# ashawkey/torch-ngp

Measured on AMD Instinct MI355X. Metric: training samples/s (rays x steps), lego-shaped synthetic, fp16 autocast, full step incl. Adam, higher is better.
Workload: dtype f16

## Files before the change

include/ngp_hip.h:

```cpp
#ifndef NGP_HIP_H
#define NGP_HIP_H

#include <stddef.h>
#include <stdint.h>

#ifdef __cplusplus
extern "C" {
#endif

typedef void* ngp_stream_t;

enum {
    NGP_OK = 0,
    NGP_ERR_INVALID = 1,
    NGP_ERR_LAUNCH = 2,
    NGP_ERR_DEVICE = 3
};

enum { NGP_F32 = 0, NGP_F16 = 1, NGP_F64 = 2 };

#define NGP_MAX_LEVELS 32

const char* ngp_last_error(void);
int ngp_abi_version(void);
// ... 133 lines not shown
    float lr, beta1, beta2, eps;
} ngp_table_adam_t;
uint32_t ngp_grid_table_adam_prefix(const int32_t* offsets_host, uint32_t B, uint32_t D, uint32_t C, uint32_t L, float S, uint32_t H,
                                    uint32_t gridtype, int align_corners, int dtype);
typedef struct ngp_slab_sets {
    const void* slabs_a; uint32_t n_slabs_a, n_params_a; void* grad_weights_a;
    const void* slabs_b; uint32_t n_slabs_b, n_params_b; void* grad_weights_b;
    const float* ray_err; uint32_t n_rays; float* loss;
    uint32_t overwrite_table;
    const ngp_table_adam_t* table_adam;
} ngp_slab_sets_t;
int ngp_grid_encode_backward_checked_slabs(const void* grad, const float* inputs, const void* embeddings, const int32_t* offsets,
                                           void* grad_embeddings, uint32_t B, uint32_t D, uint32_t C, uint32_t L, float S, uint32_t H,
                                           const void* dy_dx, void* grad_inputs, uint32_t gridtype, int align_corners, uint32_t interp,
                                           int dtype, float bound, const int32_t* offsets_host, void* workspace, size_t workspace_bytes,
                                           float* found_inf, const ngp_slab_sets_t* slab_sets, ngp_stream_t stream);
int ngp_grid_encode_backward_ws(const void* grad, const float* inputs, const void* embeddings, const int32_t* offsets,
                                void* grad_embeddings, uint32_t B, uint32_t D, uint32_t C, uint32_t L, float S, uint32_t H,
                                const void* dy_dx, void* grad_inputs, uint32_t gridtype, int align_corners, uint32_t interp,
                                int dtype, float bound, const int32_t* offsets_host, void* workspace, size_t workspace_bytes,
                                ngp_stream_t stream);

size_t ngp_density_grid_update_workspace_bytes(uint32_t n_cells);
int ngp_density_grid_update(const float* sigmas, const int64_t* cells, uint32_t n, float density_scale, float decay, float* density_grid,
                            uint32_t n_cells, float* scratch, float density_thresh, float* mean_out, uint8_t* bitfield, void* workspace,
                            ngp_stream_t stream);

#define NGP_FF_INPUT_PLANAR 1u
#define NGP_FF_DX_PLANAR 2u
#define NGP_FF_LAYERED 4u
#define NGP_FF_SINGLE_WAVE 8u
#define NGP_FF_DEFER_REDUCE 16u
#define NGP_FF_RECOMPUTE 32u
int ngp_ffmlp_forward_ex(const void* inputs, const void* weights, uint32_t B, uint32_t input_dim, uint32_t output_dim,
                         uint32_t hidden_dim, uint32_t num_layers, uint32_t activation, uint32_t output_activation,
                         void* forward_buffer, void* outputs, uint32_t flags, ngp_stream_t stream);
int ngp_ffmlp_inference_ex(const void* inputs, const void* weights, uint32_t B, uint32_t input_dim,
                           uint32_t output_dim, uint32_t hidden_dim, uint32_t num_layers, uint32_t activation,
                           uint32_t output_activation, void* inference_buffer, void* outputs, uint32_t flags,
                           ngp_stream_t stream);
int ngp_ffmlp_backward_ex(const void* grad, const void* inputs, const void* weights, const void* forward_buffer,
                          uint32_t B, uint32_t input_dim, uint32_t output_dim, uint32_t hidden_dim, uint32_t num_layers,
                          uint32_t activation, uint32_t output_activation, int calc_grad_inputs, void* backward_buffer,
                          void* grad_inputs, void* grad_weights, uint32_t flags, ngp_stream_t stream);

size_t ngp_ffmlp_backward_workspace_bytes(uint32_t B, uint32_t input_dim, uint32_t hidden_dim, uint32_t num_layers);
int ngp_ffmlp_backward_ws(const void* grad, const void* inputs, const void* weights, const void* forward_buffer, uint32_t B,
                          uint32_t input_dim, uint32_t output_dim, uint32_t hidden_dim, uint32_t num_layers, uint32_t activation,
                          uint32_t output_activation, int calc_grad_inputs, void* backward_buffer, void* grad_inputs, void* grad_weights,
                          uint32_t flags, void* workspace, size_t workspace_bytes, ngp_stream_t stream);

int ngp_network_forward(const void* enc, const float* dirs, uint32_t M, uint32_t M_valid, const void* w_sigma, const void* w_color,
                        uint32_t num_layers_sigma, uint32_t num_layers_color, float density_scale, int training,
                        void* forward_buffer_sigma, void* h16, float* sigma, void* color_in, void* forward_buffer_color, float* rgb,
                        uint32_t flags, ngp_stream_t stream);

int ngp_network_forward_rows(const void* enc, const float* dirs, uint32_t M, uint32_t M_valid, const void* w_sigma, const void* w_color,
                             uint32_t num_layers_sigma, uint32_t num_layers_color, float density_scale, int training,
                             void* forward_buffer_sigma, void* h16, float* sigma, void* color_in, void* forward_buffer_color, float* rgb,
                             uint32_t flags, const uint32_t* rows_dev, ngp_stream_t stream);

int ngp_network_backward_color(const void* grad_out16, const void* color_in, const void* w_color, const void* forward_buffer_color, uint32_t M,
                               uint32_t num_layers_color, void* backward_buffer, const float* grad_sigma, const void* h16,
                               float density_scale, void* grad_h16, void* grad_w_color, uint32_t flags, ngp_stream_t stream);
uint32_t ngp_ffmlp_backward_slab_count(uint32_t B, uint32_t input_dim, uint32_t hidden_dim, uint32_t num_layers);
int ngp_ffmlp_reduce_slabs_pair(const void* slabs_a, uint32_t n_slabs_a, uint32_t n_params_a, void* grad_weights_a, const void* slabs_b,
                                uint32_t n_slabs_b, uint32_t n_params_b, void* grad_weights_b, float* found_inf, ngp_stream_t stream);

int ngp_pipeline_mid_forward(const void* h16, const float* dirs, float* sigma, void* color_in, uint32_t M, uint32_t M_valid,
                             float density_scale, ngp_stream_t stream);
int ngp_pipeline_rgb_forward(const void* out16, float* rgb, uint32_t M, ngp_stream_t stream);
int ngp_pipeline_rgb_backward(const float* grad_rgb, const float* rgb, void* grad_out16, uint32_t M, ngp_stream_t stream);
int ngp_pipeline_mid_backward(const float* grad_sigma, const void* h16, const void* grad_color_in, void* grad_h16, uint32_t M,
                              float density_scale, ngp_stream_t stream);

int ngp_pipeline_mse_loss(const float* image, const float* target, uint32_t n, const float* loss_scale, float* loss,
                          float* grad_image, ngp_stream_t stream);
// ... 73 lines not shown
                                         float T_thresh, float* grad_sigmas, float* grad_rgbs, int bg_mode, float bg_scalar,
                                         const float* bg, const uint32_t* rows_used, ngp_stream_t stream);

int ngp_composite_train_loss_backward(const float* sigmas, const float* rgbs, const float* deltas, const int32_t* rays, uint32_t M,
                                      uint32_t N, float T_thresh, int bg_mode, float bg_scalar, const float* bg, const float* nears,
                                      const float* fars, const float* target, const float* loss_scale, float* weights_sum,
                                      float* image_out, float* depth_out, float* loss, float* ray_err, float* grad_sigmas,
                                      void* grad_out16, void* march_workspace, size_t march_workspace_bytes, ngp_stream_t stream);

int ngp_freq_encode_forward(const float* inputs, uint32_t B, uint32_t D, uint32_t deg, uint32_t C, float* outputs,
                            ngp_stream_t stream);
int ngp_freq_encode_backward(const float* grad, const float* outputs, uint32_t B, uint32_t D, uint32_t deg, uint32_t C,
                             float* grad_inputs, ngp_stream_t stream);

int ngp_optim_adam_step(int count, const uint64_t* n, float* const* params, float* const* exp_avg, float* const* exp_avg_sq,
                        void* const* grads, void* const* params_fp16, const int* grad_is_half, const float* lr, float beta1,
                        float beta2, float eps, float grad_mult, float growth_factor, float backoff_factor, float growth_interval,
                        float* state, ngp_stream_t stream);

#define NGP_OPT_PHASE_CHECK 1u
#define NGP_OPT_PHASE_UPDATE 2u
#define NGP_OPT_PHASE_COMMIT 4u
#define NGP_OPT_PHASE_FLIP 8u
int ngp_optim_adam_step_ex(int count, const uint64_t* n, float* const* params, float* const* exp_avg, float* const* exp_avg_sq,
                           void* const* grads, void* const* params_fp16, const int* grad_is_half, const float* lr, float beta1,
                           float beta2, float eps, float grad_mult, float growth_factor, float backoff_factor, float growth_interval,
                           float* state, float* const* ema, float ema_one_minus_decay, uint32_t phases, ngp_stream_t stream);
struct ngp_table_adam;
int ngp_optim_adam_small_commit(int count, const uint64_t* n, float* const* params, float* const* exp_avg, float* const* exp_avg_sq,
                                void* const* grads, void* const* params_fp16, const int* grad_is_half, const float* lr, float beta1,
                                float beta2, float eps, float grad_mult, float growth_factor, float backoff_factor, float growth_interval,
                                float* state, int flip_parity, const struct ngp_table_adam* table, const void* table_grad_fp16,
                                uint64_t table_prefix_params, ngp_stream_t stream);
int ngp_optim_poison_shards(void* flat_grad_fp16, uint32_t shards, uint64_t payload, const float* state, ngp_stream_t stream);
int ngp_optim_shard_verdict(const void* shard_grad_fp16, float* state, void* flat_grad_fp16, uint32_t shards, uint64_t payload,
                            ngp_stream_t stream);
int ngp_optim_ema_update(int count, const uint64_t* n, float* const* params, float* const* ema, float one_minus_decay, ngp_stream_t stream);

#ifdef __cplusplus
}
#endif
#endif
```

torch-ngp_amd/_ngp_capi.py:

```python
import ctypes
import os

import torch

_HERE = os.path.dirname(os.path.abspath(__file__))
LIB_PATH = os.environ.get('NGP_HIP_LIBRARY') or os.path.join(_HERE, 'libngp_hip.so')

NGP_F32, NGP_F16, NGP_F64 = 0, 1, 2
NGP_FF_INPUT_PLANAR, NGP_FF_DX_PLANAR, NGP_FF_LAYERED, NGP_FF_SINGLE_WAVE, NGP_FF_DEFER_REDUCE, NGP_FF_RECOMPUTE = 1, 2, 4, 8, 16, 32
NGP_MARCH_RESET_COUNTER, NGP_MARCH_ZERO_TAIL, NGP_MARCH_NOISE_FROM_SEED, NGP_MARCH_SCAN_LAUNCH = 1, 2, 4, 8
NGP_OPT_PHASE_CHECK, NGP_OPT_PHASE_UPDATE, NGP_OPT_PHASE_COMMIT, NGP_OPT_PHASE_FLIP = 1, 2, 4, 8
ABI_VERSION = 11

if not os.path.exists(LIB_PATH):
    raise ImportError(
        f"{LIB_PATH} is missing: build the HIP extension first (python __graft_entry__.py, or "
        f"make -C {os.path.join(_HERE, 'csrc')}).  There is no CPU fallback for these operators.")

lib = ctypes.CDLL(LIB_PATH)

_vp, _u32, _f32, _i32, _sz = ctypes.c_void_p, ctypes.c_uint32, ctypes.c_float, ctypes.c_int, ctypes.c_size_t

_SIGNATURES = {
    'ngp_grid_encode_forward': [_vp, _vp, _vp, _vp, _u32, _u32, _u32, _u32, _f32, _u32, _vp, _u32, _i32, _u32, _i32, _vp],
    'ngp_grid_encode_backward': [_vp, _vp, _vp, _vp, _vp, _u32, _u32, _u32, _u32, _f32, _u32, _vp, _vp, _u32, _i32, _u32, _i32, _vp],
    'ngp_grad_total_variation': [_vp, _vp, _vp, _vp, _f32, _u32, _u32, _u32, _u32, _f32, _u32, _u32, _i32, _i32, _vp],
    'ngp_grid_corner_indices': [_vp, _vp, _vp, _u32, _u32, _u32, _f32, _u32, _u32, _i32, _vp],
    'ngp_grid_level_table': [_u32, _f32, _u32, _vp, _vp],
    'ngp_grid_encode_backward_backward': [_vp, _vp, _vp, _vp, _vp, _vp, _vp, _vp, _u32, _u32, _u32, _u32, _f32, _u32, _u32, _i32, _u32, _i32, _vp,
                                          _sz, _vp],
    'ngp_sh_encode_forward': [_vp, _vp, _u32, _u32, _u32, _vp, _i32, _vp],
    'ngp_sh_encode_backward': [_vp, _vp, _u32, _u32, _u32, _vp, _vp, _i32, _vp],
    'ngp_freq_encode_forward': [_vp, _u32, _u32, _u32, _u32, _vp, _vp],
    'ngp_freq_encode_backward': [_vp, _vp, _u32, _u32, _u32, _u32, _vp, _vp],
    'ngp_near_far_from_aabb': [_vp, _vp, _vp, _u32, _f32, _vp, _vp, _vp],
    'ngp_sph_from_ray': [_vp, _vp, _f32, _u32, _vp, _vp],
    'ngp_morton3D': [_vp, _u32, _vp, _vp],
    'ngp_morton3D_invert': [_vp, _u32, _vp, _vp],
    'ngp_packbits': [_vp, _u32, _f32, _vp, _vp],
    'ngp_packbits_ex': [_vp, _u32, _f32, _vp, _vp, _vp],
    'ngp_march_rays_train': [_vp, _vp, _vp, _f32, _f32, _u32, _u32, _u32, _u32, _u32, _vp, _vp, _vp, _vp, _vp, _vp, _vp, _vp, _vp, _vp],
    'ngp_composite_rays_train_forward': [_vp, _vp, _vp, _vp, _u32, _u32, _f32, _vp, _vp, _vp, _vp],
# ... 24 lines not shown
    'ngp_grid_encode_backward_ws': [_vp, _vp, _vp, _vp, _vp, _u32, _u32, _u32, _u32, _f32, _u32, _vp, _vp, _u32, _i32, _u32, _i32, _f32, _vp, _vp,
                                    _sz, _vp],
    'ngp_grid_encode_backward_checked': [_vp, _vp, _vp, _vp, _vp, _u32, _u32, _u32, _u32, _f32, _u32, _vp, _vp, _u32, _i32, _u32, _i32, _f32, _vp,
                                         _vp, _sz, _vp, _vp],
    'ngp_grid_encode_backward_checked_slabs': [_vp, _vp, _vp, _vp, _vp, _u32, _u32, _u32, _u32, _f32, _u32, _vp, _vp, _u32, _i32, _u32, _i32, _f32,
                                               _vp, _vp, _sz, _vp, _vp, _vp],
    'ngp_density_grid_update': [_vp, _vp, _u32, _f32, _f32, _vp, _u32, _vp, _f32, _vp, _vp, _vp, _vp],
    'ngp_ffmlp_forward_ex': [_vp, _vp, _u32, _u32, _u32, _u32, _u32, _u32, _u32, _vp, _vp, _u32, _vp],
    'ngp_ffmlp_inference_ex': [_vp, _vp, _u32, _u32, _u32, _u32, _u32, _u32, _u32, _vp, _vp, _u32, _vp],
    'ngp_ffmlp_backward_ex': [_vp, _vp, _vp, _vp, _u32, _u32, _u32, _u32, _u32, _u32, _u32, _i32, _vp, _vp, _vp, _u32, _vp],
    'ngp_ffmlp_backward_ws': [_vp, _vp, _vp, _vp, _u32, _u32, _u32, _u32, _u32, _u32, _u32, _i32, _vp, _vp, _vp, _u32, _vp, _sz, _vp],
    'ngp_network_forward': [_vp, _vp, _u32, _u32, _vp, _vp, _u32, _u32, _f32, _i32, _vp, _vp, _vp, _vp, _vp, _vp, _u32, _vp],
    'ngp_network_forward_rows': [_vp, _vp, _u32, _u32, _vp, _vp, _u32, _u32, _f32, _i32, _vp, _vp, _vp, _vp, _vp, _vp, _u32, _vp, _vp],
    'ngp_march_rays_dev_rows': [_vp, _u32, _u32, _u32, _vp, _vp, _vp, _vp, _f32, _f32, _u32, _u32, _u32, _vp, _vp, _vp, _vp, _vp, _vp, _vp, _u32, _vp, _vp],
    'ngp_pipeline_mid_forward': [_vp, _vp, _vp, _vp, _u32, _u32, _f32, _vp],
    'ngp_pipeline_rgb_forward': [_vp, _vp, _u32, _vp],
    'ngp_pipeline_rgb_backward': [_vp, _vp, _vp, _u32, _vp],
    'ngp_pipeline_mid_backward': [_vp, _vp, _vp, _vp, _u32, _f32, _vp],
    'ngp_pipeline_mse_loss': [_vp, _vp, _u32, _vp, _vp, _vp, _vp],
    'ngp_rays_from_pixels': [_vp, _u32, _f32, _f32, _f32, _f32, _u32, _vp, _u32, _u32, _vp, _vp, _vp],
    'ngp_march_rays_train_ex': [_vp, _vp, _vp, _f32, _f32, _u32, _u32, _u32, _u32, _u32, _vp, _vp, _vp, _vp, _vp, _vp, _vp, _vp, _vp, _u32, _vp],
    'ngp_march_rays_train_aabb': [_vp, _vp, _vp, _f32, _f32, _u32, _u32, _u32, _u32, _u32, _vp, _f32, _vp, _vp, _vp, _vp, _vp, _vp, _vp, _vp, _vp, _u32,
                                  _vp],
    'ngp_composite_rays_train_forward_ex': [_vp, _vp, _vp, _vp, _u32, _u32, _f32, _vp, _vp, _vp, _i32, _f32, _vp, _vp, _vp, _vp, _vp, _vp],
    'ngp_composite_rays_train_backward_ex': [_vp, _vp, _vp, _vp, _vp, _vp, _vp, _vp, _u32, _u32, _f32, _vp, _vp, _i32, _f32, _vp, _vp, _vp],
    'ngp_composite_train_loss_backward': [_vp, _vp, _vp, _vp, _u32, _u32, _f32, _i32, _f32, _vp, _vp, _vp, _vp, _vp, _vp, _vp, _vp, _vp, _vp, _vp,
                                          _vp, _vp, _sz, _vp],
    'ngp_network_backward_color': [_vp, _vp, _vp, _vp, _u32, _u32, _vp, _vp, _vp, _f32, _vp, _vp, _u32, _vp],
    'ngp_ffmlp_reduce_slabs_pair': [_vp, _u32, _u32, _vp, _vp, _u32, _u32, _vp, _vp, _vp],
    'ngp_optim_adam_step': [_i32, _vp, _vp, _vp, _vp, _vp, _vp, _vp, _vp, _f32, _f32, _f32, _f32, _f32, _f32, _f32, _vp, _vp],
    'ngp_optim_adam_step_ex': [_i32, _vp, _vp, _vp, _vp, _vp, _vp, _vp, _vp, _f32, _f32, _f32, _f32, _f32, _f32, _f32, _vp, _vp, _f32, _u32, _vp],
    'ngp_optim_adam_small_commit': [_i32, _vp, _vp, _vp, _vp, _vp, _vp, _vp, _vp, _f32, _f32, _f32, _f32, _f32, _f32, _f32, _vp, _i32, _vp, _vp,
                                    ctypes.c_uint64, _vp],
    'ngp_optim_ema_update': [_i32, _vp, _vp, _vp, _f32, _vp],
    'ngp_optim_poison_shards': [_vp, _u32, ctypes.c_uint64, _vp, _vp],
    'ngp_optim_shard_verdict': [_vp, _vp, _vp, _u32, ctypes.c_uint64, _vp],
    'ngp_linear_stack_pack': [_vp, _u32, _u32, _u32, _u32, _i32, _vp, _vp],
    'ngp_linear_stack_unpack_grad': [_vp, _u32, _u32, _u32, _u32, _i32, _vp, _vp],
    'ngp_pad_2d_fp16': [_vp, _u32, _u32, _u32, _vp, _u32, _u32, _vp],
    'ngp_allocate_splitk': [_sz],
    'ngp_free_splitk': [],
}
for _name, _args in _SIGNATURES.items():
    _fn = getattr(lib, _name)
    _fn.argtypes = _args
    _fn.restype = ctypes.c_int
lib.ngp_last_error.restype = ctypes.c_char_p
lib.ngp_target_arch.restype = ctypes.c_char_p
lib.ngp_abi_version.restype = ctypes.c_int
lib.ngp_ffmlp_backward_slab_count.argtypes = [_u32, _u32, _u32, _u32]
lib.ngp_ffmlp_backward_slab_count.restype = _u32
lib.ngp_march_rays_train_workspace_bytes.argtypes = [_u32]
lib.ngp_march_rays_train_workspace_bytes.restype = _sz
lib.ngp_compact_rays_workspace_bytes.argtypes = [_u32]
lib.ngp_ffmlp_backward_workspace_bytes.argtypes = [_u32, _u32, _u32, _u32]
lib.ngp_ffmlp_backward_workspace_bytes.restype = _sz
lib.ngp_grid_backward_workspace_bytes.argtypes = [_vp, _u32, _u32, _u32, _u32, _f32, _u32, _u32, _i32, _i32]
lib.ngp_grid_backward_workspace_bytes.restype = _sz
lib.ngp_grid_backward_backward_workspace_bytes.argtypes = [_vp, _u32, _u32, _u32, _u32, _i32]
lib.ngp_grid_backward_backward_workspace_bytes.restype = _sz
lib.ngp_compact_rays_workspace_bytes.restype = _sz
lib.ngp_grid_table_adam_prefix.argtypes = [_vp, _u32, _u32, _u32, _u32, _f32, _u32, _u32, _i32, _i32]
lib.ngp_grid_table_adam_prefix.restype = _u32
lib.ngp_coarse_occupancy_bytes.argtypes = [_u32, _u32]
lib.ngp_coarse_occupancy_bytes.restype = _sz
lib.ngp_grid_forward_work_lists.argtypes = [_u32, _u32, _vp, _vp, _vp, _vp]
lib.ngp_grid_forward_work_lists.restype = _u32
lib.ngp_density_grid_update_workspace_bytes.argtypes = [_u32]
lib.ngp_linear_stack_flat_size.argtypes = [_u32, _u32, _u32, _u32, _i32]
lib.ngp_linear_stack_flat_size.restype = _u32
lib.ngp_density_grid_update_workspace_bytes.restype = _sz

if lib.ngp_abi_version() != ABI_VERSION:
    raise ImportError(f"{LIB_PATH}: ABI version {lib.ngp_abi_version()} != expected {ABI_VERSION}; rebuild the extension")

EXPORTED = sorted(list(_SIGNATURES) + ['ngp_last_error', 'ngp_target_arch', 'ngp_abi_version',
                                       'ngp_march_rays_train_workspace_bytes', 'ngp_compact_rays_workspace_bytes',
                                       'ngp_grid_backward_workspace_bytes', 'ngp_ffmlp_backward_workspace_bytes',
                                       'ngp_ffmlp_backward_slab_count', 'ngp_density_grid_update_workspace_bytes', 'ngp_grid_forward_work_lists', 'ngp_coarse_occupancy_bytes',
                                       'ngp_grid_table_adam_prefix', 'ngp_linear_stack_flat_size',
                                       'ngp_grid_backward_backward_workspace_bytes'])


def check(rc):
    if rc != 0:
        raise RuntimeError(lib.ngp_last_error().decode('utf-8', 'replace'))


class SlabSets(ctypes.Structure):
    _fields_ = [('slabs_a', ctypes.c_void_p), ('n_slabs_a', ctypes.c_uint32), ('n_params_a', ctypes.c_uint32), ('grad_weights_a', ctypes.c_void_p),
                ('slabs_b', ctypes.c_void_p), ('n_slabs_b', ctypes.c_uint32), ('n_params_b', ctypes.c_uint32), ('grad_weights_b', ctypes.c_void_p),
                ('ray_err', ctypes.c_void_p), ('n_rays', ctypes.c_uint32), ('loss', ctypes.c_void_p), ('overwrite_table', ctypes.c_uint32),
                ('table_adam', ctypes.c_void_p)]


class RenderLoop(ctypes.Structure):
    _fields_ = ([('state', ctypes.c_void_p), ('alive', ctypes.c_void_p * 2)] +
                [(n, ctypes.c_void_p) for n in ('rays_t', 'rays_o', 'rays_d', 'nears', 'fars', 'grid', 'noises', 'xyzs', 'dirs', 'deltas', 'enc', 'sigmas',
                                                'rgbs', 'embeddings', 'offsets', 'level_cost_host', 'w_sigma', 'w_color', 'weights_sum', 'depth', 'image',
                                                'compact_workspace', 'rows_used')] +
                [(n, ctypes.c_uint32) for n in ('lanes', 'rows', 'n_total', 'n_step_cap', 'max_steps', 'cascade', 'grid_size', 'L', 'H', 'gridtype',
                                                'interp', 'num_layers_sigma', 'num_layers_color')] +
                [('align_corners', ctypes.c_int32)] + [(n, ctypes.c_float) for n in ('bound', 'dt_gamma', 'T_thresh', 'S', 'density_scale')])


class TableAdam(ctypes.Structure):
    _fields_ = [('param', ctypes.c_void_p * 2), ('exp_avg', ctypes.c_void_p * 2), ('exp_avg_sq', ctypes.c_void_p * 2), ('param_fp16', ctypes.c_void_p * 2),
                ('state', ctypes.c_void_p), ('lr', ctypes.c_float), ('beta1', ctypes.c_float), ('beta2', ctypes.c_float), ('eps', ctypes.c_float)]


def ptr(t):
    return None if t is None else t.data_ptr()


def stream():
    return torch.cuda.current_stream().cuda_stream


def require_device(t, name):
    if not t.is_cuda:
        raise RuntimeError(f"{name} must be a CUDA tensor")


def require_contiguous(t, name):
    if not t.is_contiguous():
        raise RuntimeError(f"{name} must be a contiguous tensor")


def require_int32(t, name):
    if t.dtype != torch.int32:
        raise RuntimeError(f"{name} must be an int tensor")


def float_code(t, name):
    if t.dtype == torch.float16:
        return NGP_F16
    if t.dtype == torch.float32:
        return NGP_F32
    if t.dtype == torch.float64:
        return NGP_F64
    raise RuntimeError(f"{name} must be a floating tensor")
# ... 60 lines not shown
```

torch-ngp_amd/csrc/ffmlp.hip:

```cpp
#include "common.h"
#include "sh_poly.inc"

namespace ngp {

constexpr int FF_WAVES = 4;
constexpr int FF_THREADS = FF_WAVES * 64;
constexpr int FF_TILE = 32;

enum Act : uint32_t { ACT_RELU = 0, ACT_EXP = 1, ACT_SINE = 2, ACT_SIGMOID = 3, ACT_SQUAREPLUS = 4, ACT_SOFTPLUS = 5, ACT_NONE = 6 };
constexpr float K_ACT = 10.0f;

__device__ __forceinline__ float act_forward(uint32_t a, float x) {
    switch (a) {
        case ACT_RELU: return x > 0.0f ? x : 0.0f;
        case ACT_EXP: return __expf(x);
        case ACT_SINE: return __sinf(x);
        case ACT_SIGMOID: return 1.0f / (1.0f + __expf(-x));
        case ACT_SQUAREPLUS: { const float s = x * K_ACT; return 0.5f * (s + sqrtf(s * s + 4.0f)) / K_ACT; }
        case ACT_SOFTPLUS: return __logf(__expf(x * K_ACT) + 1.0f) / K_ACT;
        default: return x;
    }
}
__device__ __forceinline__ float act_backward_factor(uint32_t a, float y) {
    switch (a) {
        case ACT_RELU: return y > 0.0f ? 1.0f : 0.0f;
        case ACT_EXP: return y;
        case ACT_SIGMOID: return y * (1.0f - y);
        case ACT_SQUAREPLUS: { const float s = y * K_ACT; return s * s / (s * s + 1.0f); }
        case ACT_SOFTPLUS: return 1.0f - __expf(-y * K_ACT);
        default: return 1.0f;
    }
}

// ... 115 lines not shown
__device__ void build_forward_image(half8_t* img, const half_t* __restrict__ w, uint32_t in_dim, uint32_t num_layers, uint32_t first_frag = 0,
                                    uint32_t n_frags = 0xFFFFFFFFu) {
    if (first_frag == 0u && n_frags == 0xFFFFFFFFu && (in_dim & 15u) == 0u) {
        build_forward_image_coalesced<WIDTH>(img, w, in_dim, num_layers);
        return;
    }
    const uint32_t all = fwd_frag_count<WIDTH>(in_dim, num_layers);
    const uint32_t total = (n_frags == 0xFFFFFFFFu ? all : n_frags) * 64;
    const uint32_t shift = first_frag * 64;
    for (uint32_t e0 = threadIdx.x; e0 < total; e0 += IMG_BATCH * blockDim.x) {
        half4_t lo[IMG_BATCH], hi[IMG_BATCH];
        bool real[IMG_BATCH];
#pragma unroll
        for (int b = 0; b < IMG_BATCH; b++) {
            const uint32_t e = e0 + b * blockDim.x;
            const half_t *pl = nullptr, *ph = nullptr;
            if (e < total) forward_fragment_source<WIDTH>(e + shift, w, in_dim, num_layers, pl, ph);
            real[b] = pl != nullptr;
            lo[b] = *reinterpret_cast<const half4_t*>(pl ? pl : w);
            hi[b] = *reinterpret_cast<const half4_t*>(ph ? ph : w);
        }
#pragma unroll
        for (int b = 0; b < IMG_BATCH; b++) {
            const uint32_t e = e0 + b * blockDim.x;
            if (e < total) {
                const half4_t z = {(half_t)0.0f, (half_t)0.0f, (half_t)0.0f, (half_t)0.0f};
                const half4_t l4 = real[b] ? lo[b] : z, h4 = real[b] ? hi[b] : z;
                img[e] = half8_t{l4.x, l4.y, l4.z, l4.w, h4.x, h4.y, h4.z, h4.w};
            }
        }
    }
}

template <int WIDTH>
__device__ __forceinline__ void pack_hidden(const float16_t (&acc)[Shape<WIDTH>::NIB], half8_t (&frag)[Shape<WIDTH>::NKB]) {
#pragma unroll
    for (int kb = 0; kb < Shape<WIDTH>::NKB; kb++) {
#pragma unroll
        for (int j = 0; j < 8; j++) frag[kb][j] = (half_t)acc[kb >> 1][(kb & 1) * 8 + j];
    }
}

__device__ __forceinline__ uint32_t relu_pack2(float a, float b) {
    typedef float f32x2 __attribute__((ext_vector_type(2)));
    typedef short i16x2 __attribute__((ext_vector_type(2)));
    const half2_t hv = __builtin_convertvector(f32x2{a, b}, half2_t);
    return __builtin_bit_cast(uint32_t, __builtin_elementwise_max(__builtin_bit_cast(i16x2, hv), i16x2{0, 0}));
}
template <int WIDTH>
__device__ __forceinline__ void pack_hidden_relu(const float16_t (&acc)[Shape<WIDTH>::NIB], half8_t (&frag)[Shape<WIDTH>::NKB]) {
    typedef uint32_t u32x4 __attribute__((ext_vector_type(4)));
#pragma unroll
    for (int kb = 0; kb < Shape<WIDTH>::NKB; kb++) {
        u32x4 w;
#pragma unroll
        for (int q = 0; q < 4; q++) w[q] = relu_pack2(acc[kb >> 1][(kb & 1) * 8 + 2 * q], acc[kb >> 1][(kb & 1) * 8 + 2 * q + 1]);
        frag[kb] = __builtin_bit_cast(half8_t, w);
    }
}


__device__ __forceinline__ half8_t load_features8(const half_t* __restrict__ inputs, bool planar, size_t rows, size_t s, uint32_t in_dim,
                                                  uint32_t f0) {
    if (!planar) return *reinterpret_cast<const half8_t*>(inputs + s * in_dim + f0);
    half8_t v;
#pragma unroll
    for (int q = 0; q < 4; q++) {
        const half2_t t = *reinterpret_cast<const half2_t*>(inputs + ((size_t)(f0 / 2 + q) * rows + s) * 2);
        v[2 * q] = t.x;
        v[2 * q + 1] = t.y;
    }
    return v;
}

template <typename V>
__device__ __forceinline__ void stream_store(V* dst, V v) {
    __builtin_nontemporal_store(v, dst);
}

template <int WIDTH, bool TRAIN, bool PLAIN >
__device__ __forceinline__ void ffmlp_forward_body(const half_t* __restrict__ inputs, const half_t* __restrict__ weights,
                                                   half_t* __restrict__ forward_buffer, half_t* __restrict__ outputs, uint32_t n_tiles,
                                                   uint32_t in_dim, uint32_t num_layers, uint32_t act, uint32_t out_act, bool in_planar) {
    constexpr int NIB = Shape<WIDTH>::NIB, NKB = Shape<WIDTH>::NKB;
    extern __shared__ __attribute__((aligned(16))) unsigned char smem[];
    half8_t* img = reinterpret_cast<half8_t*>(smem);
    build_forward_image<WIDTH>(img, weights, in_dim, num_layers);
    const size_t rows = (size_t)n_tiles * FF_TILE;
    __syncthreads();

    const int lane = threadIdx.x & 63, wid = threadIdx.x >> 6;
    const int n = lane & 31, h = lane >> 5;
    const uint32_t in_kb = in_dim / 16;
    const half8_t* img_l0 = img + lane;
    const half8_t* img_hid = img_l0 + (size_t)NIB * in_kb * 64;
    const half8_t* img_out = img_hid + (size_t)(num_layers - 1) * NIB * NKB * 64;
    const size_t layer_stride = (size_t)n_tiles * NKB * 64;

    for (uint32_t tile = blockIdx.x * FF_WAVES + wid; tile < n_tiles; tile += gridDim.x * FF_WAVES) {
        const size_t srow = (size_t)tile * FF_TILE + n;
        float16_t acc[NIB];
#pragma unroll
        for (int ib = 0; ib < NIB; ib++) acc[ib] = zero16();
        for (uint32_t kb = 0; kb < in_kb; kb++) {
            const half8_t x = load_features8(inputs, in_planar, rows, srow, in_dim, 16 * kb + 8 * h);
#pragma unroll
            for (int ib = 0; ib < NIB; ib++) acc[ib] = mfma(img_l0[(ib * in_kb + kb) * 64], x, acc[ib]);
        }
        half8_t hid[NKB];
        for (uint32_t l = 0;; l++) {
            if (PLAIN || act == ACT_RELU) {
                pack_hidden_relu<WIDTH>(acc, hid);
            } else {
                if (act != ACT_NONE) {
#pragma unroll
                    for (int ib = 0; ib < NIB; ib++)
#pragma unroll
                        for (int r = 0; r < 16; r++) acc[ib][r] = act_forward(act, acc[ib][r]);
                }
                pack_hidden<WIDTH>(acc, hid);
            }
            if (TRAIN) {
                half8_t* dst = reinterpret_cast<half8_t*>(forward_buffer) + l * layer_stride + (size_t)tile * NKB * 64 + lane;
#pragma unroll
                for (int kb = 0; kb < NKB; kb++) stream_store(dst + kb * 64, hid[kb]);
            }
            if (l + 1 == num_layers) break;
            const half8_t* wl = img_hid + (size_t)l * NIB * NKB * 64;
#pragma unroll
            for (int ib = 0; ib < NIB; ib++) {
                acc[ib] = zero16();
#pragma unroll
                for (int kb = 0; kb < NKB; kb++) acc[ib] = mfma(wl[(ib * NKB + kb) * 64], hid[kb], acc[ib]);
            }
        }
        float16_t o = zero16();
#pragma unroll
        for (int kb = 0; kb < NKB; kb++) o = mfma(img_out[kb * 64], hid[kb], o);
        half4_t lo, hi;
#pragma unroll
        for (int c = 0; c < 4; c++) {
            lo[c] = (half_t)(PLAIN ? o[c] : act_forward(out_act, o[c]));
            hi[c] = (half_t)(PLAIN ? o[4 + c] : act_forward(out_act, o[4 + c]));
        }
        half_t* orow = outputs + ((size_t)tile * FF_TILE + n) * 16 + 4 * h;
        *reinterpret_cast<half4_t*>(orow) = lo;
        *reinterpret_cast<half4_t*>(orow + 8) = hi;
    }
}

template <int WIDTH, bool TRAIN, bool PLAIN>
__global__ __launch_bounds__(FF_THREADS) __attribute__((amdgpu_waves_per_eu(4, 4))) void k_ffmlp_forward(
    const half_t* __restrict__ inputs, const half_t* __restrict__ weights, half_t* __restrict__ forward_buffer, half_t* __restrict__ outputs,
    uint32_t n_tiles, uint32_t in_dim, uint32_t num_layers, uint32_t act, uint32_t out_act, bool in_planar) {
    ffmlp_forward_body<WIDTH, TRAIN, PLAIN>(inputs, weights, forward_buffer, outputs, n_tiles, in_dim, num_layers, act, out_act, in_planar);
}
template <int WIDTH, bool TRAIN, bool PLAIN>
__global__ __launch_bounds__(FF_THREADS) __attribute__((amdgpu_waves_per_eu(2, 2))) void k_ffmlp_forward_wide(
    const half_t* __restrict__ inputs, const half_t* __restrict__ weights, half_t* __restrict__ forward_buffer, half_t* __restrict__ outputs,
    uint32_t n_tiles, uint32_t in_dim, uint32_t num_layers, uint32_t act, uint32_t out_act, bool in_planar) {
    ffmlp_forward_body<WIDTH, TRAIN, PLAIN>(inputs, weights, forward_buffer, outputs, n_tiles, in_dim, num_layers, act, out_act, in_planar);
}


template <bool TRAIN, int NT>
__device__ __forceinline__ void relu_network_tail(float16_t (&acc)[NT][2], float16_t (&o)[NT], const half8_t* __restrict__ hid_img,
                                                  const half8_t* __restrict__ out_img, uint32_t nl, half_t* __restrict__ fb, size_t layer_stride,
                                                  const uint32_t (&tile)[NT], const bool (&live)[NT], int lane) {
    constexpr int WIDTH = 64, NIB = 2, NKB = 4;
    half8_t hid[NT][NKB];
    for (uint32_t l = 0;; l++) {
#pragma unroll
        for (int t = 0; t < NT; t++) {
            pack_hidden_relu<WIDTH>(acc[t], hid[t]);
            if (TRAIN && fb && live[t]) {
                half8_t* dst = reinterpret_cast<half8_t*>(fb) + l * layer_stride + (size_t)tile[t] * NKB * 64 + lane;
#pragma unroll
                for (int kb = 0; kb < NKB; kb++) stream_store(dst + kb * 64, hid[t][kb]);
            }
        }
        if (l + 1 == nl) break;
        const half8_t* wl = hid_img + (size_t)l * NIB * NKB * 64;
#pragma unroll
        for (int ib = 0; ib < NIB; ib++) {
#pragma unroll
            for (int t = 0; t < NT; t++) acc[t][ib] = zero16();
#pragma unroll
            for (int kb = 0; kb < NKB; kb++) {
                const half8_t a = wl[(ib * NKB + kb) * 64];
#pragma unroll
                for (int t = 0; t < NT; t++) acc[t][ib] = mfma(a, hid[t][kb], acc[t][ib]);
            }
        }
    }
#pragma unroll
    for (int t = 0; t < NT; t++) o[t] = zero16();
#pragma unroll
    for (int kb = 0; kb < NKB; kb++) {
        const half8_t a = out_img[kb * 64];
#pragma unroll
        for (int t = 0; t < NT; t++) o[t] = mfma(a, hid[t][kb], o[t]);
    }
}

template <bool TRAIN, int WAVES , int NT >
__global__ __launch_bounds__(WAVES * 64) __attribute__((amdgpu_waves_per_eu(NT == 1 ? 4 : 2, NT == 1 ? 4 : 3))) void k_network_forward(
    const half_t* __restrict__ enc, bool enc_planar, const float* __restrict__ dirs, uint32_t M_valid, const half_t* __restrict__ w_sigma,
    const half_t* __restrict__ w_color, half_t* __restrict__ fb_s, half_t* __restrict__ h16, float* __restrict__ sigma,
    half_t* __restrict__ color_in, half_t* __restrict__ fb_c, float* __restrict__ rgb, uint32_t n_tiles_cap, uint32_t nl_s, uint32_t nl_c,
    float density_scale, const uint32_t* __restrict__ rows_dev) {
    constexpr int WIDTH = 64, NIB = 2, NKB = 4;
    constexpr uint32_t in_kb = 2;
    const uint32_t n_tiles = rows_dev ? min(n_tiles_cap, (rows_dev[0] + (uint32_t)FF_TILE - 1u) / (uint32_t)FF_TILE) : n_tiles_cap;
    extern __shared__ __attribute__((aligned(16))) unsigned char smem[];
    half8_t* img_s = reinterpret_cast<half8_t*>(smem);
    const uint32_t frags_s = NIB * in_kb + (nl_s - 1) * NIB * NKB + NKB;
    half8_t* img_c = img_s + (size_t)frags_s * 64;
    const size_t rows = (size_t)n_tiles_cap * FF_TILE;
    const int lane = threadIdx.x & 63, wid = threadIdx.x >> 6;
    const int n = lane & 31, h = lane >> 5;
    const uint32_t n_groups = (n_tiles + NT - 1) / NT;
    half8_t x_next[NT][in_kb];
    float dir_next[NT][3];
#pragma unroll
    for (int t = 0; t < NT; t++) dir_next[t][0] = dir_next[t][1] = dir_next[t][2] = 0.0f;
    auto request = [&](uint32_t group) {
        if (group < n_groups) {
#pragma unroll
            for (int t = 0; t < NT; t++) {
                const uint32_t tl = group * NT + t < n_tiles ? group * NT + t : n_tiles - 1;
                const size_t srow = (size_t)tl * FF_TILE + n;
#pragma unroll
                for (uint32_t kb = 0; kb < in_kb; kb++) x_next[t][kb] = load_features8(enc, enc_planar, rows, srow, 32, 16 * kb + 8 * h);
                dir_next[t][0] = dir_next[t][1] = dir_next[t][2] = 0.0f;
                if (srow < M_valid) { dir_next[t][0] = dirs[srow * 3]; dir_next[t][1] = dirs[srow * 3 + 1]; dir_next[t][2] = dirs[srow * 3 + 2]; }
            }
        }
    };
    request(blockIdx.x * WAVES + wid);
    build_forward_image<WIDTH>(img_s, w_sigma, 32, nl_s);
    build_forward_image<WIDTH>(img_c, w_color, 32, nl_c);
    __syncthreads();

    const size_t layer_stride = (size_t)n_tiles_cap * NKB * 64;
    const half8_t* s_l0 = img_s + lane;
    const half8_t* s_hid = s_l0 + (size_t)NIB * in_kb * 64;
    const half8_t* s_out = s_hid + (size_t)(nl_s - 1) * NIB * NKB * 64;
    const half8_t* c_l0 = img_c + lane;
    const half8_t* c_hid = c_l0 + (size_t)NIB * in_kb * 64;
    const half8_t* c_out = c_hid + (size_t)(nl_c - 1) * NIB * NKB * 64;

    for (uint32_t group = blockIdx.x * WAVES + wid; group < n_groups; group += gridDim.x * WAVES) {
        uint32_t tile[NT];
        bool live[NT];
        size_t srow[NT];
        half8_t x_cur[NT][in_kb];
        float dir_x[NT], dir_y[NT], dir_z[NT];
#pragma unroll
        for (int t = 0; t < NT; t++) {
            live[t] = NT == 1 || group * NT + t < n_tiles;
            tile[t] = live[t] ? group * NT + t : n_tiles - 1;
            srow[t] = (size_t)tile[t] * FF_TILE + n;
#pragma unroll
            for (uint32_t kb = 0; kb < in_kb; kb++) x_cur[t][kb] = x_next[t][kb];
            dir_x[t] = dir_next[t][0]; dir_y[t] = dir_next[t][1]; dir_z[t] = dir_next[t][2];
        }
        request(group + gridDim.x * WAVES);
        float16_t acc[NT][NIB], o[NT];
#pragma unroll
        for (int t = 0; t < NT; t++)
#pragma unroll
            for (int ib = 0; ib < NIB; ib++) acc[t][ib] = zero16();
#pragma unroll
        for (uint32_t kb = 0; kb < in_kb; kb++)
// ... 254 lines not shown
        for (int kb = 0; kb < NKB; kb++) { dma16(frag + l * layer_stride + kb * 64, buf + (size_t)(1 + l * NKB + kb) * 1024); issued++; }
    unsigned char* xb = buf + (size_t)(1 + num_layers * NKB) * 1024;
    const uint32_t in_kb = in_dim / 16;
    if (!in_planar) {
        for (uint32_t kb = 0; kb < in_kb; kb++) { dma16(inputs + srow * in_dim + 16 * kb + 8 * h, xb + (size_t)kb * 1024); issued++; }
    } else {
        for (uint32_t kb = 0; kb < in_kb; kb++)
#pragma unroll
            for (int q = 0; q < 4; q++) {
                dma4(inputs + ((size_t)((16 * kb + 8 * h) / 2 + q) * rows + srow) * 2, xb + (size_t)kb * 1024 + q * 256);
                issued++;
            }
    }
    return issued;
}

__device__ __forceinline__ half8_t tile_x(const unsigned char* xb, uint32_t kb, bool in_planar, int lane) {
    if (!in_planar) return *reinterpret_cast<const half8_t*>(xb + (size_t)kb * 1024 + lane * 16);
    half8_t v;
#pragma unroll
    for (int q = 0; q < 4; q++) {
        const half2_t t = *reinterpret_cast<const half2_t*>(xb + (size_t)kb * 1024 + q * 256 + lane * 4);
        v[2 * q] = t.x;
        v[2 * q + 1] = t.y;
    }
    return v;
}

template <int WIDTH, int IN_JB , int NHM , bool RELU >
__global__ __launch_bounds__(FF_THREADS) void k_ffmlp_backward(const half_t* __restrict__ grad, const half_t* __restrict__ inputs,
                                                               const half_t* __restrict__ weights, const half_t* __restrict__ forward_buffer,
                                                               uint32_t n_tiles, uint32_t in_dim, uint32_t num_layers, uint32_t act,
                                                               bool with_dx, half_t* __restrict__ grad_inputs, float* __restrict__ slabs,
                                                               half_t* __restrict__ grad_weights_direct, bool in_planar, bool dx_planar, uint32_t pf_depth) {
    constexpr int NIB = Shape<WIDTH>::NIB, NKB = Shape<WIDTH>::NKB;
    extern __shared__ __attribute__((aligned(16))) unsigned char smem[];
    half8_t* img = reinterpret_cast<half8_t*>(smem);
    const uint32_t nfrag = bwd_frag_count<WIDTH>(in_dim, num_layers, with_dx);
    build_backward_image<WIDTH>(img, weights, in_dim, num_layers, with_dx);
    const int lane = threadIdx.x & 63, wid = threadIdx.x >> 6;
    const int n = lane & 31, h = lane >> 5;
    (void)nfrag;
    const Selectors sel = make_selectors(n, h);
    __syncthreads();

    const uint32_t in_kb = in_dim / 16;
    const half8_t* img_out = img + lane;
    const half8_t* img_hid = img_out + (size_t)NIB * 64;
    const half8_t* img_in = img_hid + (size_t)(num_layers - 1) * NIB * NKB * 64;
    const size_t layer_stride = (size_t)n_tiles * NKB * 64;
    const half8_t* fb = reinterpret_cast<const half8_t*>(forward_buffer);
    const size_t rows = (size_t)n_tiles * FF_TILE;

    float16_t gw_out[NIB];
    float16_t gw_in[NIB][IN_JB];
#pragma unroll
    for (int jb = 0; jb < NIB; jb++) gw_out[jb] = zero16();
#pragma unroll
    for (int ib = 0; ib < NIB; ib++)
#pragma unroll
        for (int jb = 0; jb < IN_JB; jb++) gw_in[ib][jb] = zero16();
    float16_t gw_hid[NHM][NIB][NIB];
#pragma unroll
    for (int l = 0; l < NHM; l++)
#pragma unroll
        for (int ib = 0; ib < NIB; ib++)
#pragma unroll
            for (int jb = 0; jb < NIB; jb++) gw_hid[l][ib][jb] = zero16();

    const uint32_t tile_frags = 1 + num_layers * NKB + in_dim / 16;
    unsigned char* pf_base = smem + (size_t)nfrag * 1024 + (size_t)wid * pf_depth * tile_frags * 1024;
    const uint32_t tile_step = gridDim.x * FF_WAVES;
// ... 169 lines not shown
    for (int ib = 0; ib < NIB; ib++) acc[ib] = zero16();
    for (uint32_t kb = 0; kb < in_kb; kb++) {
        const half8_t x = tile_x(xb, kb, in_planar, lane);
#pragma unroll
        for (int ib = 0; ib < NIB; ib++) acc[ib] = mfma(fimg_lane[(ib * in_kb + kb) * 64], x, acc[ib]);
    }
    const half8_t* fhid = fimg_lane + (size_t)NIB * in_kb * 64;
    half8_t hid[NKB];
#pragma unroll
    for (int l = 0; l <= NHM; l++) {
        pack_hidden_relu<WIDTH>(acc, hid);
        sink(l, hid);
        if (l == NHM) break;
        const half8_t* wl = fhid + (size_t)l * NIB * NKB * 64;
#pragma unroll
        for (int ib = 0; ib < NIB; ib++) {
            acc[ib] = zero16();
#pragma unroll
            for (int kb = 0; kb < NKB; kb++) acc[ib] = mfma(wl[(ib * NKB + kb) * 64], hid[kb], acc[ib]);
        }
    }
}

template <int N>
__device__ __forceinline__ void wait_vmcnt() {
    asm volatile("s_waitcnt vmcnt(%0)" ::"n"(N) : "memory");
}

template <int WIDTH, int IN_JB, int NHM , bool RELU, bool RECOMP = false>
__global__ __launch_bounds__(FP_THREADS) __attribute__((amdgpu_waves_per_eu(2, 2)))
void k_ffmlp_backward_paired(const half_t* __restrict__ grad, const half_t* __restrict__ inputs, const half_t* __restrict__ weights,
                             const half_t* __restrict__ forward_buffer, uint32_t n_tiles, uint32_t in_dim, uint32_t num_layers, uint32_t act,
                             bool with_dx, half_t* __restrict__ grad_inputs, float* __restrict__ slabs,
                             half_t* __restrict__ grad_weights_direct, bool in_planar, bool dx_planar, uint32_t pf_depth, MidEpilogue mid) {
    static_assert(NHM == 1 || NHM == 2, "the paired backward covers 2- and 3-layer networks");
    constexpr int NIB = Shape<WIDTH>::NIB, NKB = Shape<WIDTH>::NKB;
    extern __shared__ __attribute__((aligned(16))) unsigned char smem[];
    half8_t* img = reinterpret_cast<half8_t*>(smem);
    const uint32_t nfrag = bwd_frag_count<WIDTH>(in_dim, num_layers, with_dx);
    const uint32_t in_kb = in_dim / 16;
    const uint32_t ffrag = RECOMP ? NIB * in_kb + (num_layers - 1) * NIB * NKB : 0u;
    const int lane = threadIdx.x & 63, wid = threadIdx.x >> 6;
    const int n = lane & 31, h = lane >> 5;
    const int pair = wid & (FP_PAIRS - 1), role = wid / FP_PAIRS;
    const size_t layer_stride = (size_t)n_tiles * NKB * 64;
    const half8_t* fb = reinterpret_cast<const half8_t*>(forward_buffer);
    const size_t rows = (size_t)n_tiles * FF_TILE;
    const uint32_t act_layers = RECOMP ? 0u : num_layers;
    const uint32_t tile_frags = 1 + act_layers * NKB + in_kb;
    unsigned char* pf_base = smem + (size_t)(nfrag + ffrag) * 1024 + (size_t)pair * pf_depth * tile_frags * 1024;
    half8_t* scratch = reinterpret_cast<half8_t*>(smem + (size_t)(nfrag + ffrag) * 1024 + (size_t)FP_PAIRS * pf_depth * tile_frags * 1024 +
                                                  (size_t)pair * NHM * NKB * 1024) + lane;
    const uint32_t base_step = gridDim.x * FP_PAIRS;
    uint32_t cur = 0;
    const uint32_t tile_loads = tile_dma_count<WIDTH>(act_layers, in_dim, in_planar);
    auto prefetch = [&](uint32_t buffer, uint32_t tile) {
        const uint32_t issued = prefetch_tile<WIDTH>(pf_base + (size_t)buffer * tile_frags * 1024, tile, grad, fb, inputs, act_layers, layer_stride,
                                                     rows, in_dim, in_planar, lane, n, h);
        NGP_BOUNDS(issued == tile_loads);
        (void)issued;
    };
    if (role == 0) {
        for (uint32_t d = 0; d + 1 < (pf_depth > 1 ? pf_depth : 2u); d++)
            if (blockIdx.x * FP_PAIRS + d * base_step + pair < n_tiles) prefetch(d, blockIdx.x * FP_PAIRS + d * base_step + pair);
    }
    build_backward_image<WIDTH>(img, weights, in_dim, num_layers, with_dx);
    if (RECOMP) build_forward_image<WIDTH>(img + (size_t)nfrag * 64, weights, in_dim, num_layers, 0, ffrag);
    const Selectors sel = make_selectors(n, h);
    __syncthreads();

    const half8_t* img_out = img + lane;
    const half8_t* img_hid = img_out + (size_t)NIB * 64;
    const half8_t* img_in = img_hid + (size_t)(num_layers - 1) * NIB * NKB * 64;
    const half8_t* fimg = img + (size_t)nfrag * 64 + lane;
    static_assert(tile_dma_count<64>(0, 32, false) == 3u && tile_dma_count<64>(0, 32, true) == 9u && tile_dma_count<64>(2, 32, false) == 11u &&
                  tile_dma_count<64>(2, 32, true) == 17u, "the enumerated vmcnt immediates below are the DMA counts of the three-deep shapes");
    const bool deep = pf_depth == 3 && (tile_loads == 3u || tile_loads == 9u || tile_loads == 11u || tile_loads == 17u);
    auto next_tile_buffer = [&](uint32_t base) -> const unsigned char* {
        if (role == 0) {
            if (deep && base + base_step + pair < n_tiles) {
                switch (tile_loads) {
                    case 3u: wait_vmcnt<3>(); break;
                    case 9u: wait_vmcnt<9>(); break;
                    case 11u: wait_vmcnt<11>(); break;
                    default: wait_vmcnt<17>(); break;
                }
            } else {
                wait_vmcnt<0>();
            }
        }
        __syncthreads();
        const unsigned char* tb = pf_base + (size_t)cur * tile_frags * 1024;
        if (pf_depth > 1) {
            const uint32_t ahead = pf_depth - 1;
            const uint32_t fill = cur == 0 ? pf_depth - 1 : cur - 1;
            cur = cur + 1 == pf_depth ? 0u : cur + 1;
            if (role == 0 && base + ahead * base_step + pair < n_tiles) prefetch(fill, base + ahead * base_step + pair);
        }
        return tb;
    };
// ... 542 lines not shown
    slab_reduce_block(sets, blockIdx.x, part, found_inf);
}

struct DeviceInfo {
    int cus = 0;
    bool ok = false;
};
static DeviceInfo device_info() {
    static thread_local DeviceInfo info;
    if (!info.ok) {
        int dev = 0;
        if (hipGetDevice(&dev) == hipSuccess) {
            hipDeviceProp_t p;
            if (hipGetDeviceProperties(&p, dev) == hipSuccess) {
                info.cus = p.multiProcessorCount;
                info.ok = true;
            }
        }
        if (!info.ok) info.cus = 256;
    }
    return info;
}

static int check_ff_args(const char* fn, uint32_t B, uint32_t in_dim, uint32_t out_dim, uint32_t hidden, uint32_t num_layers) {
    NGP_REQUIRE(hidden == 16 || hidden == 32 || hidden == 64 || hidden == 128 || hidden == 256, NGP_ERR_INVALID,
                "%s: hidden_dim should in [16, 32, 64, 128, 256], but got %u", fn, hidden);
    NGP_REQUIRE(in_dim > 0 && in_dim % 16 == 0, NGP_ERR_INVALID, "%s: input_dim should be 16 * m (m > 0), but got %u", fn, in_dim);
    NGP_REQUIRE(out_dim == 16, NGP_ERR_INVALID, "%s: output_dim must be padded to 16 by the caller (got %u)", fn, out_dim);
    NGP_REQUIRE(num_layers >= 2, NGP_ERR_INVALID, "%s: num_layers should be larger than 2 (3 matmuls), but got %u", fn, num_layers);
    NGP_REQUIRE(B % 128 == 0, NGP_ERR_INVALID, "%s: batch size must be 128 * m, but got %u", fn, B);
    return NGP_OK;
}

static int raise_lds(const void* kern, size_t lds, const char* what) {
    if (lds > 64 * 1024) {
        hipError_t e = hipFuncSetAttribute(kern, hipFuncAttributeMaxDynamicSharedMemorySize, (int)lds);
        NGP_REQUIRE(e == hipSuccess, NGP_ERR_LAUNCH, "%s: cannot raise the dynamic LDS limit: %s", what, hipGetErrorString(e));
    }
    return NGP_OK;
}

template <int WIDTH>
static size_t forward_image_bytes(uint32_t in_dim, uint32_t num_layers) {
    constexpr int NIB = Shape<WIDTH>::NIB, NKB = Shape<WIDTH>::NKB;
    return (size_t)(NIB * (in_dim / 16) + (num_layers - 1) * NIB * NKB + NKB) * 1024;
}

template <int WIDTH, bool TRAIN>
static int launch_forward_layered(const void* inputs, const void* weights, uint32_t B, uint32_t in_dim, uint32_t num_layers, uint32_t act,
                                  uint32_t out_act, void* buffer, void* outputs, uint32_t flags, hipStream_t st) {
    constexpr int NIB = Shape<WIDTH>::NIB, NKB = Shape<WIDTH>::NKB;
    const uint32_t n_tiles = B / FF_TILE;
    uint32_t frags = NIB * (in_dim / 16);
    if (frags < (uint32_t)(NIB * NKB)) frags = NIB * NKB;
    const size_t lds = (size_t)frags * 1024;
    NGP_REQUIRE(lds <= 152 * 1024, NGP_ERR_INVALID, "ffmlp: one %u x %u layer (%zu B) exceeds the LDS of a CU", (unsigned)WIDTH, in_dim, lds);
    NGP_REQUIRE(buffer, NGP_ERR_INVALID, "ffmlp: this network shape needs the %s the reference passes", TRAIN ? "forward_buffer" : "inference_buffer [B, hidden]");
    auto kern = k_ffmlp_forward_layered<WIDTH, TRAIN>;
    int rc = raise_lds(reinterpret_cast<const void*>(kern), lds, "ffmlp");
    if (rc) return rc;
    const uint32_t per_cu = (uint32_t)((160 * 1024) / (lds + 1024));
    uint32_t blocks = (uint32_t)device_info().cus * (per_cu < 1 ? 1 : (per_cu > 2 ? 2 : per_cu));
    const uint32_t need = cdiv(n_tiles, FF_WAVES);
    if (blocks > need) blocks = need;
    hipLaunchKernelGGL(kern, dim3(blocks), dim3(FF_THREADS), lds, st, (const half_t*)inputs, (const half_t*)weights, (half_t*)buffer,
                       (half_t*)outputs, n_tiles, in_dim, num_layers, act, out_act, (flags & NGP_FF_INPUT_PLANAR) != 0);
    return check_launch(TRAIN ? "ffmlp_forward(layered)" : "ffmlp_inference(layered)");
}

template <int WIDTH, bool TRAIN>
static int launch_forward(const void* inputs, const void* weights, uint32_t B, uint32_t in_dim, uint32_t num_layers, uint32_t act,
                          uint32_t out_act, void* fwd, void* outputs, uint32_t flags, hipStream_t st) {
    const uint32_t n_tiles = B / FF_TILE;
    const size_t lds = forward_image_bytes<WIDTH>(in_dim, num_layers);
    if (WIDTH > 128 || lds > 152 * 1024 || (flags & NGP_FF_LAYERED))
        return launch_forward_layered<WIDTH, TRAIN>(inputs, weights, B, in_dim, num_layers, act, out_act, fwd, outputs, flags, st);
    if constexpr (WIDTH > 128) {
        return NGP_ERR_INVALID;
    } else {
    const bool plain = act == ACT_RELU && out_act == ACT_NONE;
    const void* kern;
    if constexpr (WIDTH > 64) kern = plain ? reinterpret_cast<const void*>(k_ffmlp_forward_wide<WIDTH, TRAIN, true>)
                                           : reinterpret_cast<const void*>(k_ffmlp_forward_wide<WIDTH, TRAIN, false>);
    else kern = plain ? reinterpret_cast<const void*>(k_ffmlp_forward<WIDTH, TRAIN, true>) : reinterpret_cast<const void*>(k_ffmlp_forward<WIDTH, TRAIN, false>);
    int rc = raise_lds(kern, lds, "ffmlp");
    if (rc) return rc;
    const uint32_t per_cu = (uint32_t)((160 * 1024) / (lds + 1024));
    uint32_t blocks = (uint32_t)device_info().cus * (per_cu < 1 ? 1 : (per_cu > 4 ? 4 : per_cu));
    const uint32_t need = cdiv(n_tiles, FF_WAVES);
    if (blocks > need) blocks = need;
    const half_t* a0 = (const half_t*)inputs;
    const half_t* a1 = (const half_t*)weights;
    half_t* a2 = (half_t*)fwd;
    half_t* a3 = (half_t*)outputs;
    uint32_t a4 = n_tiles, a5 = in_dim, a6 = num_layers, a7 = act, a8 = out_act;
    bool a9 = (flags & NGP_FF_INPUT_PLANAR) != 0;
    void* args[] = {&a0, &a1, &a2, &a3, &a4, &a5, &a6, &a7, &a8, &a9};
    hipError_t e = hipLaunchKernel(kern, dim3(blocks), dim3(FF_THREADS), args, lds, st);
    NGP_REQUIRE(e == hipSuccess, NGP_ERR_LAUNCH, "ffmlp: kernel launch failed: %s", hipGetErrorString(e));
    return check_launch(TRAIN ? "ffmlp_forward" : "ffmlp_inference");
    }
}

constexpr uint32_t WG_MAX_CHUNKS = 64;

template <int WIDTH>
static int launch_backward_layered(const void* grad, const void* inputs, const void* weights, const void* fwd, uint32_t B, uint32_t in_dim,
                                   uint32_t num_layers, uint32_t act, bool with_dx, void* backward_buffer, void* grad_inputs,
                                   void* grad_weights, uint32_t flags, void* workspace, size_t workspace_bytes, hipStream_t st) {
    constexpr int NIB = Shape<WIDTH>::NIB, NKB = Shape<WIDTH>::NKB;
    const bool in_planar = (flags & NGP_FF_INPUT_PLANAR) != 0, dx_planar = (flags & NGP_FF_DX_PLANAR) != 0;
    const uint32_t n_tiles = B / FF_TILE;
    const uint32_t in_jb = (in_dim + 31) / 32;
    uint32_t frags = NIB * NKB;
    if (with_dx && frags < in_jb * NKB) frags = in_jb * NKB;
    const size_t lds = (size_t)frags * 1024;
    NGP_REQUIRE(lds <= 152 * 1024, NGP_ERR_INVALID, "ffmlp_backward: one %u x %u layer (%zu B) exceeds the LDS of a CU", (unsigned)WIDTH, in_dim, lds);
    const void* dk = act == ACT_RELU ? reinterpret_cast<const void*>(k_ffmlp_dgrad_layered<WIDTH, true>)
                                     : reinterpret_cast<const void*>(k_ffmlp_dgrad_layered<WIDTH, false>);
    int rc = raise_lds(dk, lds, "ffmlp_backward");
    if (rc) return rc;
    const uint32_t per_cu = (uint32_t)((160 * 1024) / (lds + 1024));
    uint32_t blocks = (uint32_t)device_info().cus * (per_cu < 1 ? 1 : (per_cu > 2 ? 2 : per_cu));
    const uint32_t need = cdiv(n_tiles, FF_WAVES);
    if (blocks > need) blocks = need;
    if (act == ACT_RELU)
        hipLaunchKernelGGL((k_ffmlp_dgrad_layered<WIDTH, true>), dim3(blocks), dim3(FF_THREADS), lds, st, (const half_t*)grad, (const half_t*)weights,
                           (const half_t*)fwd, (half_t*)backward_buffer, n_tiles, in_dim, num_layers, act, with_dx, (half_t*)grad_inputs, dx_planar);
    else
        hipLaunchKernelGGL((k_ffmlp_dgrad_layered<WIDTH, false>), dim3(blocks), dim3(FF_THREADS), lds, st, (const half_t*)grad, (const half_t*)weights,
// ... 12 lines not shown
        if (chunks > by_tiles) chunks = by_tiles;
        if (chunks < 1) chunks = 1;
    }
    const uint32_t tiles_per_chunk = cdiv(n_tiles, chunks);
    chunks = cdiv(n_tiles, tiles_per_chunk);
    const bool direct = chunks == 1;
    hipLaunchKernelGGL(k_ffmlp_wgrad<WIDTH>, dim3(chunks, jobs), dim3(FF_THREADS), 0, st, (const half_t*)grad, (const half_t*)inputs, (const half_t*)fwd,
                       (const half_t*)backward_buffer, n_tiles, in_dim, num_layers, in_planar, tiles_per_chunk, direct ? (float*)nullptr : (float*)workspace,
                       direct ? (half_t*)grad_weights : (half_t*)nullptr);
    rc = check_launch("ffmlp_backward(wgrad)");
    if (rc || direct) return rc;
    hipLaunchKernelGGL(k_ffmlp_reduce_slabs, dim3(cdiv(n_params, RS_PARAMS)), dim3(RS_PARAMS * RS_GROUPS), 0, st, (const float*)workspace, chunks,
                       n_params, (half_t*)grad_weights);
    return check_launch("ffmlp_backward(reduce)");
}

template <int WIDTH>
static uint32_t backward_slab_count(uint32_t B, uint32_t in_dim, uint32_t num_layers) {
    const uint32_t n_params = ff_param_count(in_dim, WIDTH, num_layers);
    const size_t buf_bytes = (size_t)num_layers * B * WIDTH * sizeof(half_t);
    uint32_t blocks = (uint32_t)device_info().cus;
    const uint32_t need = cdiv(B / FF_TILE, FF_WAVES);
    if (blocks > need) blocks = need;
    const size_t fit = buf_bytes / ((size_t)n_params * 4);
    if (blocks > fit) blocks = (uint32_t)fit;
    return blocks;
}

template <int WIDTH, int IN_JB, int NHM, bool RELU>
static int launch_backward_t(const void* grad, const void* inputs, const void* weights, const void* fwd, uint32_t B, uint32_t in_dim,
                           uint32_t num_layers, uint32_t act, bool with_dx, void* backward_buffer, void* grad_inputs,
                           void* grad_weights, uint32_t flags, hipStream_t st, const MidEpilogue* mid_in) {
    const bool in_planar = (flags & NGP_FF_INPUT_PLANAR) != 0, dx_planar = (flags & NGP_FF_DX_PLANAR) != 0;
    const bool defer = (flags & NGP_FF_DEFER_REDUCE) != 0;
    const MidEpilogue mid = mid_in ? *mid_in : MidEpilogue{nullptr, nullptr, nullptr, 0.0f};
    constexpr int NIB = Shape<WIDTH>::NIB, NKB = Shape<WIDTH>::NKB;
    const uint32_t n_tiles = B / FF_TILE;
    const uint32_t nfrag = NIB + (num_layers - 1) * NIB * NKB + (with_dx ? ((in_dim + 31) / 32) * NKB : 0);
    const uint32_t n_params = ff_param_count(in_dim, WIDTH, num_layers);
    const size_t tile_bytes = (size_t)(1 + num_layers * NKB + in_dim / 16) * 1024;
    uint32_t pf_depth = 2;
    if ((size_t)nfrag * 1024 + 2 * FF_WAVES * tile_bytes > 160 * 1024) pf_depth = 1;
    size_t lds = (size_t)nfrag * 1024 + (size_t)pf_depth * FF_WAVES * tile_bytes;
    if (lds < (size_t)n_params * 4) lds = (size_t)n_params * 4;
    NGP_REQUIRE(lds <= 160 * 1024, NGP_ERR_INVALID, "ffmlp_backward: LDS need (%zu B) exceeds 160 KiB", lds);
    const uint32_t blocks = backward_slab_count<WIDTH>(B, in_dim, num_layers);
    if (flags & NGP_FF_RECOMPUTE) {
        if constexpr (WIDTH == 64 && IN_JB == 1 && RELU && (NHM == 1 || NHM == 2)) {
            NGP_REQUIRE(in_dim == 32 && !(flags & NGP_FF_SINGLE_WAVE), NGP_ERR_INVALID, "ffmlp_backward: NGP_FF_RECOMPUTE needs input_dim 32 and the paired kernel");
            const uint32_t ffrag = NIB * (in_dim / 16) + (num_layers - 1) * NIB * NKB;
            const size_t tile_b = (size_t)(1 + in_dim / 16) * 1024;
            const uint32_t depth = 3;
            size_t lds_r = (size_t)(nfrag + ffrag) * 1024 + (size_t)depth * FP_PAIRS * tile_b + (size_t)FP_PAIRS * NHM * NKB * 1024;
            if (lds_r < (size_t)n_params * 4) lds_r = (size_t)n_params * 4;
            auto pk = k_ffmlp_backward_paired<WIDTH, IN_JB, NHM, RELU, true>;
            if (lds_r > 64 * 1024) {
                hipError_t e = hipFuncSetAttribute(reinterpret_cast<const void*>(pk), hipFuncAttributeMaxDynamicSharedMemorySize, (int)lds_r);
                NGP_REQUIRE(e == hipSuccess, NGP_ERR_LAUNCH, "ffmlp_backward: cannot raise the dynamic LDS limit: %s", hipGetErrorString(e));
            }
            const bool direct = blocks <= 1;
            hipLaunchKernelGGL(pk, dim3(direct ? 1 : blocks), dim3(FP_THREADS), lds_r, st, (const half_t*)grad, (const half_t*)inputs,
                               (const half_t*)weights, (const half_t*)nullptr, n_tiles, in_dim, num_layers, act, with_dx, (half_t*)grad_inputs,
                               direct ? (float*)nullptr : (float*)backward_buffer, direct ? (half_t*)grad_weights : (half_t*)nullptr, in_planar,
                               dx_planar, depth, mid);
            int rc = check_launch("ffmlp_backward");
            if (rc || direct || defer) return rc;
            hipLaunchKernelGGL(k_ffmlp_reduce_slabs, dim3(cdiv(n_params, RS_PARAMS)), dim3(RS_PARAMS * RS_GROUPS), 0, st,
                               (const float*)backward_buffer, blocks, n_params, (half_t*)grad_weights);
            return check_launch("ffmlp_backward(reduce)");
        } else {
            NGP_REQUIRE(false, NGP_ERR_INVALID, "ffmlp_backward: NGP_FF_RECOMPUTE serves 64-wide ReLU networks with 32 inputs and 2 or 3 layers");
        }
    }
    if constexpr (NHM == 1 || NHM == 2) {
        if (!(flags & NGP_FF_SINGLE_WAVE)) {
            auto pk = k_ffmlp_backward_paired<WIDTH, IN_JB, NHM, RELU>;
            if (lds > 64 * 1024) {
                hipError_t e = hipFuncSetAttribute(reinterpret_cast<const void*>(pk), hipFuncAttributeMaxDynamicSharedMemorySize, (int)lds);
                NGP_REQUIRE(e == hipSuccess, NGP_ERR_LAUNCH, "ffmlp_backward: cannot raise the dynamic LDS limit: %s", hipGetErrorString(e));
            }
            const bool direct = blocks <= 1;
            hipLaunchKernelGGL(pk, dim3(direct ? 1 : blocks), dim3(FP_THREADS), lds, st, (const half_t*)grad, (const half_t*)inputs,
                               (const half_t*)weights, (const half_t*)fwd, n_tiles, in_dim, num_layers, act, with_dx, (half_t*)grad_inputs,
                               direct ? (float*)nullptr : (float*)backward_buffer, direct ? (half_t*)grad_weights : (half_t*)nullptr, in_planar,
                               dx_planar, pf_depth, mid);
            int rc = check_launch("ffmlp_backward");
            if (rc || direct || defer) return rc;
            hipLaunchKernelGGL(k_ffmlp_reduce_slabs, dim3(cdiv(n_params, RS_PARAMS)), dim3(RS_PARAMS * RS_GROUPS), 0, st,
                               (const float*)backward_buffer, blocks, n_params, (half_t*)grad_weights);
            return check_launch("ffmlp_backward(reduce)");
        }
    }
    NGP_REQUIRE(!mid.grad_sigma && !defer, NGP_ERR_INVALID, "ffmlp_backward: this extension needs the paired kernel (2 or 3 layers)");
    auto kern = k_ffmlp_backward<WIDTH, IN_JB, NHM, RELU>;
    if (lds > 64 * 1024) {
        hipError_t e = hipFuncSetAttribute(reinterpret_cast<const void*>(kern), hipFuncAttributeMaxDynamicSharedMemorySize, (int)lds);
        NGP_REQUIRE(e == hipSuccess, NGP_ERR_LAUNCH, "ffmlp_backward: cannot raise the dynamic LDS limit: %s", hipGetErrorString(e));
    }
    if (blocks <= 1) {
        hipLaunchKernelGGL(kern, dim3(1), dim3(FF_THREADS), lds, st, (const half_t*)grad, (const half_t*)inputs, (const half_t*)weights,
                           (const half_t*)fwd, n_tiles, in_dim, num_layers, act, with_dx, (half_t*)grad_inputs, (float*)nullptr,
                           (half_t*)grad_weights, in_planar, dx_planar, pf_depth);
        return check_launch("ffmlp_backward");
    }
    hipLaunchKernelGGL(kern, dim3(blocks), dim3(FF_THREADS), lds, st, (const half_t*)grad, (const half_t*)inputs, (const half_t*)weights,
                       (const half_t*)fwd, n_tiles, in_dim, num_layers, act, with_dx, (half_t*)grad_inputs, (float*)backward_buffer,
                       (half_t*)nullptr, in_planar, dx_planar, pf_depth);
    int rc = check_launch("ffmlp_backward");
    if (rc) return rc;
    hipLaunchKernelGGL(k_ffmlp_reduce_slabs, dim3(cdiv(n_params, RS_PARAMS)), dim3(RS_PARAMS * RS_GROUPS), 0, st, (const float*)backward_buffer, blocks, n_params,
                       (half_t*)grad_weights);
    return check_launch("ffmlp_backward(reduce)");
}

template <int WIDTH, int IN_JB, int NHM>
static int launch_backward(const void* grad, const void* inputs, const void* weights, const void* fwd, uint32_t B, uint32_t in_dim,
                           uint32_t num_layers, uint32_t act, bool with_dx, void* backward_buffer, void* grad_inputs,
                           void* grad_weights, uint32_t flags, hipStream_t st, const MidEpilogue* mid = nullptr) {
    if (act == ACT_RELU)
        return launch_backward_t<WIDTH, IN_JB, NHM, true>(grad, inputs, weights, fwd, B, in_dim, num_layers, act, with_dx, backward_buffer,
                                                          grad_inputs, grad_weights, flags, st, mid);
    return launch_backward_t<WIDTH, IN_JB, NHM, false>(grad, inputs, weights, fwd, B, in_dim, num_layers, act, with_dx, backward_buffer,
                                                       grad_inputs, grad_weights, flags, st, mid);
}

}

using namespace ngp;

#define FF_WIDTHS(CALL)                  \
    switch (hidden_dim) {                \
        case 16: return CALL(16);        \
        case 32: return CALL(32);        \
        case 64: return CALL(64);        \
        case 128: return CALL(128);      \
        default: return CALL(256);       \
    }

extern "C" int ngp_ffmlp_forward_ex(const void* inputs, const void* weights, uint32_t B, uint32_t input_dim, uint32_t output_dim,
                                    uint32_t hidden_dim, uint32_t num_layers, uint32_t activation, uint32_t output_activation,
                                    void* forward_buffer, void* outputs, uint32_t flags, ngp_stream_t stream) {
    int rc = check_ff_args("ffmlp_forward", B, input_dim, output_dim, hidden_dim, num_layers);
    if (rc) return rc;
    if (B == 0) return NGP_OK;
    NGP_REQUIRE(inputs && weights && forward_buffer && outputs, NGP_ERR_INVALID, "ffmlp_forward: NULL tensor");
    hipStream_t st = as_stream(stream);
#define FF_FWD(W) launch_forward<W, true>(inputs, weights, B, input_dim, num_layers, activation, output_activation, forward_buffer, outputs, flags, st)
    FF_WIDTHS(FF_FWD)
#undef FF_FWD
}

extern "C" int ngp_ffmlp_inference_ex(const void* inputs, const void* weights, uint32_t B, uint32_t input_dim, uint32_t output_dim,
                                      uint32_t hidden_dim, uint32_t num_layers, uint32_t activation, uint32_t output_activation,
                                      void* inference_buffer, void* outputs, uint32_t flags, ngp_stream_t stream) {
    int rc = check_ff_args("ffmlp_inference", B, input_dim, output_dim, hidden_dim, num_layers);
    if (rc) return rc;
    if (B == 0) return NGP_OK;
    NGP_REQUIRE(inputs && weights && outputs, NGP_ERR_INVALID, "ffmlp_inference: NULL tensor");
    hipStream_t st = as_stream(stream);
#define FF_INF(W) launch_forward<W, false>(inputs, weights, B, input_dim, num_layers, activation, output_activation, inference_buffer, outputs, flags, st)
    FF_WIDTHS(FF_INF)
#undef FF_INF
}

extern "C" size_t ngp_ffmlp_backward_workspace_bytes(uint32_t B, uint32_t input_dim, uint32_t hidden_dim, uint32_t num_layers) {
    const bool fast = (hidden_dim == 32 || hidden_dim == 64) && num_layers <= 4 && input_dim <= 64;
    if (fast || B == 0) return 0;
    return (size_t)WG_MAX_CHUNKS * ff_param_count(input_dim, hidden_dim, num_layers) * sizeof(float);
}

extern "C" int ngp_ffmlp_backward_ws(const void* grad, const void* inputs, const void* weights, const void* forward_buffer, uint32_t B,
                                     uint32_t input_dim, uint32_t output_dim, uint32_t hidden_dim, uint32_t num_layers, uint32_t activation,
                                     uint32_t output_activation, int calc_grad_inputs, void* backward_buffer, void* grad_inputs,
                                     void* grad_weights, uint32_t flags, void* workspace, size_t workspace_bytes, ngp_stream_t stream) {
    (void)output_activation;
    int rc = check_ff_args("ffmlp_backward", B, input_dim, output_dim, hidden_dim, num_layers);
    if (rc) return rc;
    if (B == 0) {
        if (grad_weights && !(flags & NGP_FF_DEFER_REDUCE)) {
            const size_t n_w = (size_t)hidden_dim * ((size_t)input_dim + (size_t)hidden_dim * (num_layers - 1) + (size_t)output_dim);
            hipError_t e = hipMemsetAsync(grad_weights, 0, n_w * sizeof(half_t), as_stream(stream));
            NGP_REQUIRE(e == hipSuccess, NGP_ERR_LAUNCH, "ffmlp_backward: hipMemsetAsync failed: %s", hipGetErrorString(e));
        }
        return NGP_OK;
    }
    NGP_REQUIRE(grad && inputs && weights && (forward_buffer || (flags & NGP_FF_RECOMPUTE)) && backward_buffer && grad_weights, NGP_ERR_INVALID,
                "ffmlp_backward: NULL tensor");
    NGP_REQUIRE(!calc_grad_inputs || grad_inputs, NGP_ERR_INVALID, "ffmlp_backward: grad_inputs is NULL but calc_grad_inputs is set");
    hipStream_t st = as_stream(stream);
    const bool dx = calc_grad_inputs != 0;
    const bool fast = (hidden_dim == 32 || hidden_dim == 64) && num_layers <= 4 && input_dim <= 64 && !(flags & NGP_FF_LAYERED);
    NGP_REQUIRE(fast || !(flags & NGP_FF_RECOMPUTE), NGP_ERR_INVALID, "ffmlp_backward: NGP_FF_RECOMPUTE serves 64-wide ReLU networks with 32 inputs and 2 or 3 layers");
    NGP_REQUIRE(fast || !(flags & NGP_FF_DEFER_REDUCE), NGP_ERR_INVALID, "ffmlp_backward: NGP_FF_DEFER_REDUCE needs a 2- or 3-layer network of width 32 / 64");
    if (!fast) {
#define FF_LAY(W) launch_backward_layered<W>(grad, inputs, weights, forward_buffer, B, input_dim, num_layers, activation, dx, backward_buffer, grad_inputs, grad_weights, flags, workspace, workspace_bytes, st)
        FF_WIDTHS(FF_LAY)
#undef FF_LAY
    }
    const uint32_t in_jb = (input_dim + 31) / 32;
#define FF_BWD(W, J, N) \
    return launch_backward<W, J, N>(grad, inputs, weights, forward_buffer, B, input_dim, num_layers, activation, dx, backward_buffer, grad_inputs, grad_weights, flags, st)
#define FF_BWD_N(W, J)                      \
    switch (num_layers - 1) {               \
        case 1: FF_BWD(W, J, 1);            \
        case 2: FF_BWD(W, J, 2);            \
        default: FF_BWD(W, J, 3);           \
    }
    if (hidden_dim == 64) {
        if (in_jb == 1) { FF_BWD_N(64, 1) }
        FF_BWD_N(64, 2)
    }
    if (in_jb == 1) { FF_BWD_N(32, 1) }
    FF_BWD_N(32, 2)
#undef FF_BWD_N
#undef FF_BWD
}

extern "C" int ngp_ffmlp_backward_ex(const void* grad, const void* inputs, const void* weights, const void* forward_buffer, uint32_t B,
                                     uint32_t input_dim, uint32_t output_dim, uint32_t hidden_dim, uint32_t num_layers, uint32_t activation,
                                     uint32_t output_activation, int calc_grad_inputs, void* backward_buffer, void* grad_inputs,
                                     void* grad_weights, uint32_t flags, ngp_stream_t stream) {
    return ngp_ffmlp_backward_ws(grad, inputs, weights, forward_buffer, B, input_dim, output_dim, hidden_dim, num_layers, activation,
                                 output_activation, calc_grad_inputs, backward_buffer, grad_inputs, grad_weights, flags, nullptr, 0, stream);
}


extern "C" uint32_t ngp_ffmlp_backward_slab_count(uint32_t B, uint32_t input_dim, uint32_t hidden_dim, uint32_t num_layers) {
    if ((hidden_dim != 32 && hidden_dim != 64) || num_layers < 2 || num_layers > 3 || input_dim > 64 || B == 0) return 0;
    const uint32_t blocks = hidden_dim == 64 ? backward_slab_count<64>(B, input_dim, num_layers) : backward_slab_count<32>(B, input_dim, num_layers);
    return blocks <= 1 ? 0u : blocks;
}

extern "C" int ngp_ffmlp_reduce_slabs_pair(const void* slabs_a, uint32_t n_slabs_a, uint32_t n_params_a, void* grad_weights_a,
                                           const void* slabs_b, uint32_t n_slabs_b, uint32_t n_params_b, void* grad_weights_b,
                                           float* found_inf, ngp_stream_t stream) {
    const uint32_t blocks_a = (n_slabs_a || found_inf) && n_params_a ? cdiv(n_params_a, RS_PARAMS) : 0u;
    const uint32_t blocks_b = (n_slabs_b || found_inf) && n_params_b ? cdiv(n_params_b, RS_PARAMS) : 0u;
    if (blocks_a + blocks_b == 0) return NGP_OK;
    NGP_REQUIRE((!blocks_a || ((slabs_a || !n_slabs_a) && grad_weights_a)) && (!blocks_b || ((slabs_b || !n_slabs_b) && grad_weights_b)),
                NGP_ERR_INVALID, "ffmlp_reduce_slabs_pair: NULL tensor");
    SlabSets sets;
    sets.slabs[0] = (const float*)slabs_a; sets.n_slabs[0] = n_slabs_a; sets.n_params[0] = n_params_a; sets.grad_weights[0] = (half_t*)grad_weights_a;
    sets.slabs[1] = (const float*)slabs_b; sets.n_slabs[1] = n_slabs_b; sets.n_params[1] = n_params_b; sets.grad_weights[1] = (half_t*)grad_weights_b;
    sets.blocks[0] = blocks_a; sets.blocks[1] = blocks_b;
    hipLaunchKernelGGL(k_ffmlp_reduce_slabs_pair, dim3(blocks_a + blocks_b), dim3(RS_PARAMS * RS_GROUPS), 0, as_stream(stream), sets, found_inf);
    return check_launch("ffmlp_reduce_slabs_pair");
}

extern "C" int ngp_network_backward_color(const void* grad_out16, const void* color_in, const void* w_color, const void* forward_buffer_color,
                                          uint32_t M, uint32_t num_layers_color, void* backward_buffer, const float* grad_sigma,
                                          const void* h16, float density_scale, void* grad_h16, void* grad_w_color, uint32_t flags,
                                          ngp_stream_t stream) {
    NGP_REQUIRE(num_layers_color == 2 || num_layers_color == 3, NGP_ERR_INVALID,
                "network_backward_color: 2 or 3 layers (got %u); use ngp_ffmlp_backward_ex + ngp_pipeline_mid_backward", num_layers_color);
    NGP_REQUIRE(!(flags & ~(NGP_FF_DEFER_REDUCE | NGP_FF_RECOMPUTE)), NGP_ERR_INVALID,
                "network_backward_color: only NGP_FF_DEFER_REDUCE and NGP_FF_RECOMPUTE are accepted");
    int rc = check_ff_args("network_backward_color", M, 32, 16, 64, num_layers_color);
    if (rc) return rc;
    if (M == 0) return NGP_OK;
    NGP_REQUIRE(grad_out16 && color_in && w_color && (forward_buffer_color || (flags & NGP_FF_RECOMPUTE)) && backward_buffer && grad_sigma && h16 &&
                    grad_h16 && grad_w_color,
                NGP_ERR_INVALID, "network_backward_color: NULL tensor");
    const MidEpilogue mid{grad_sigma, (const half_t*)h16, (half_t*)grad_h16, density_scale};
    if (num_layers_color == 2)
        return launch_backward<64, 1, 1>(grad_out16, color_in, w_color, forward_buffer_color, M, 32, 2, ACT_RELU, true, backward_buffer, nullptr,
                                         grad_w_color, flags, as_stream(stream), &mid);
    return launch_backward<64, 1, 2>(grad_out16, color_in, w_color, forward_buffer_color, M, 32, 3, ACT_RELU, true, backward_buffer, nullptr,
                                     grad_w_color, flags, as_stream(stream), &mid);
}

extern "C" int ngp_network_forward(const void* enc, const float* dirs, uint32_t M, uint32_t M_valid, const void* w_sigma, const void* w_color,
                                   uint32_t num_layers_sigma, uint32_t num_layers_color, float density_scale, int training,
                                   void* forward_buffer_sigma, void* h16, float* sigma, void* color_in, void* forward_buffer_color,
                                   float* rgb, uint32_t flags, ngp_stream_t stream) {
    return ngp_network_forward_rows(enc, dirs, M, M_valid, w_sigma, w_color, num_layers_sigma, num_layers_color, density_scale, training,
                                    forward_buffer_sigma, h16, sigma, color_in, forward_buffer_color, rgb, flags, nullptr, stream);
}

extern "C" int ngp_network_forward_rows(const void* enc, const float* dirs, uint32_t M, uint32_t M_valid, const void* w_sigma, const void* w_color,
                                        uint32_t num_layers_sigma, uint32_t num_layers_color, float density_scale, int training,
                                        void* forward_buffer_sigma, void* h16, float* sigma, void* color_in, void* forward_buffer_color,
                                        float* rgb, uint32_t flags, const uint32_t* rows_dev, ngp_stream_t stream) {
    NGP_REQUIRE(M % 128 == 0, NGP_ERR_INVALID, "network_forward: sample count must be 128 * m, but got %u", M);
    NGP_REQUIRE(num_layers_sigma >= 2 && num_layers_color >= 2, NGP_ERR_INVALID, "network_forward: num_layers should be larger than 2");
    if (M == 0) return NGP_OK;
    NGP_REQUIRE(enc && dirs && w_sigma && w_color && sigma && rgb, NGP_ERR_INVALID, "network_forward: NULL tensor");
    NGP_REQUIRE(!training || (h16 && color_in && (forward_buffer_sigma != nullptr) == (forward_buffer_color != nullptr)), NGP_ERR_INVALID,
                "network_forward: the training variant needs h16 and color_in, and both forward buffers or (NGP_FF_RECOMPUTE backward) neither");
    const size_t lds = forward_image_bytes<64>(32, num_layers_sigma) + forward_image_bytes<64>(32, num_layers_color);
    NGP_REQUIRE(lds <= 152 * 1024, NGP_ERR_INVALID, "network_forward: weights (%zu B) exceed the LDS of a CU", lds);
#ifndef NGP_NETFWD_TRAIN_WAVES
#define NGP_NETFWD_TRAIN_WAVES 4
#endif
#ifndef NGP_NETFWD_INFER_WAVES
#define NGP_NETFWD_INFER_WAVES 4
#endif
#ifndef NGP_NETFWD_TRAIN_TILES
#define NGP_NETFWD_TRAIN_TILES 1
#endif
#ifndef NGP_NETFWD_INFER_TILES
#define NGP_NETFWD_INFER_TILES 1
#endif
    constexpr int TW = NGP_NETFWD_TRAIN_WAVES, IW = NGP_NETFWD_INFER_WAVES, TT = NGP_NETFWD_TRAIN_TILES, IT = NGP_NETFWD_INFER_TILES;
    const void* kern = training ? reinterpret_cast<const void*>(k_network_forward<true, TW, TT>) : reinterpret_cast<const void*>(k_network_forward<false, IW, IT>);
    int rc = raise_lds(kern, lds, "network_forward");
    if (rc) return rc;
    const uint32_t n_tiles = M / FF_TILE;
    const uint32_t waves = training ? TW : IW, nt = training ? TT : IT;
    const uint32_t by_lds = (uint32_t)((160 * 1024) / (lds + 1024)), by_waves = (nt == 1 ? 16u : 12u) / waves;
#ifndef NGP_NETFWD_PER_CU
#define NGP_NETFWD_PER_CU 4u
#endif
    uint32_t per_cu = by_lds < by_waves ? by_lds : by_waves;
    per_cu = per_cu < 1 ? 1 : (per_cu > NGP_NETFWD_PER_CU ? NGP_NETFWD_PER_CU : per_cu);
    uint32_t blocks = (uint32_t)device_info().cus * per_cu;
    const uint32_t need = cdiv(cdiv(n_tiles, nt), waves);
    if (blocks > need) blocks = need;
    hipStream_t st = as_stream(stream);
    const bool planar = (flags & NGP_FF_INPUT_PLANAR) != 0;
    if (training)
        hipLaunchKernelGGL((k_network_forward<true, TW, TT>), dim3(blocks), dim3(TW * 64), lds, st, (const half_t*)enc, planar, dirs, M_valid, (const half_t*)w_sigma,
                           (const half_t*)w_color, (half_t*)forward_buffer_sigma, (half_t*)h16, sigma, (half_t*)color_in, (half_t*)forward_buffer_color, rgb,
                           n_tiles, num_layers_sigma, num_layers_color, density_scale, rows_dev);
    else
        hipLaunchKernelGGL((k_network_forward<false, IW, IT>), dim3(blocks), dim3(IW * 64), lds, st, (const half_t*)enc, planar, dirs, M_valid, (const half_t*)w_sigma,
                           (const half_t*)w_color, (half_t*)nullptr, (half_t*)nullptr, sigma, (half_t*)nullptr, (half_t*)nullptr, rgb, n_tiles,
                           num_layers_sigma, num_layers_color, density_scale, rows_dev);
    return check_launch("network_forward");
}

extern "C" int ngp_ffmlp_forward(const void* inputs, const void* weights, uint32_t B, uint32_t input_dim, uint32_t output_dim,
                                 uint32_t hidden_dim, uint32_t num_layers, uint32_t activation, uint32_t output_activation,
                                 void* forward_buffer, void* outputs, ngp_stream_t stream) {
    return ngp_ffmlp_forward_ex(inputs, weights, B, input_dim, output_dim, hidden_dim, num_layers, activation, output_activation,
                                forward_buffer, outputs, 0u, stream);
}
extern "C" int ngp_ffmlp_inference(const void* inputs, const void* weights, uint32_t B, uint32_t input_dim, uint32_t output_dim,
                                   uint32_t hidden_dim, uint32_t num_layers, uint32_t activation, uint32_t output_activation,
                                   void* inference_buffer, void* outputs, ngp_stream_t stream) {
    return ngp_ffmlp_inference_ex(inputs, weights, B, input_dim, output_dim, hidden_dim, num_layers, activation, output_activation,
                                  inference_buffer, outputs, 0u, stream);
}
extern "C" int ngp_ffmlp_backward(const void* grad, const void* inputs, const void* weights, const void* forward_buffer, uint32_t B,
                                  uint32_t input_dim, uint32_t output_dim, uint32_t hidden_dim, uint32_t num_layers, uint32_t activation,
                                  uint32_t output_activation, int calc_grad_inputs, void* backward_buffer, void* grad_inputs,
                                  void* grad_weights, ngp_stream_t stream) {
    return ngp_ffmlp_backward_ex(grad, inputs, weights, forward_buffer, B, input_dim, output_dim, hidden_dim, num_layers, activation,
                                 output_activation, calc_grad_inputs, backward_buffer, grad_inputs, grad_weights, 0u, stream);
}

static size_t g_splitk_request = 0;
extern "C" int ngp_allocate_splitk(size_t size) {
    g_splitk_request = size;
    return NGP_OK;
}
extern "C" int ngp_free_splitk(void) {
    g_splitk_request = 0;
    return NGP_OK;
}
```

torch-ngp_amd/csrc/optim.hip:

```cpp
#include "common.h"
#include <math.h>
#include <stdlib.h>

namespace ngp {

#define NGP_ADAM_EL(G, M, V, P)                                                    \
    {                                                                              \
        float m_ = (M), v_ = (V), p_ = (P);                                        \
        adam_element((G), m_, v_, p_, beta1, beta2, eps, step_size, bc2_sqrt);     \
        (M) = m_; (V) = v_; (P) = p_;                                              \
    }

constexpr int OPT_THREADS = 256;
constexpr int OPT_MAX_TENSORS = 8;

struct OptTensors {
    int count;
    uint64_t n[OPT_MAX_TENSORS];
    float* p[OPT_MAX_TENSORS];
    float* m[OPT_MAX_TENSORS];
    float* v[OPT_MAX_TENSORS];
    void* g[OPT_MAX_TENSORS];
    half_t* p16[OPT_MAX_TENSORS];
    int g_is_half[OPT_MAX_TENSORS];
    float lr[OPT_MAX_TENSORS];
    float* ema[OPT_MAX_TENSORS];
};

__global__ __launch_bounds__(OPT_THREADS) void k_check_finite(OptTensors ts, float* __restrict__ state) {
    bool bad = false;
    for (int k = 0; k < ts.count; k++) {
        const uint64_t n = ts.n[k];
        if (ts.g_is_half[k] & 1) {
// ... 152 lines not shown
    }
}

__device__ __forceinline__ void update_scale(float* state, float growth, float backoff, float growth_interval, bool flip_parity = false) {
    float4_t a = *reinterpret_cast<const float4_t*>(state), b = *reinterpret_cast<const float4_t*>(state + 4);
    float scale = a.x, tracker = a.y, t = a.w, parity = b.y, dead = b.w;
    const bool scale_dead = !__builtin_isfinite(1.0f / scale);
    if (a.z != 0.0f || scale_dead) {
        if (scale_dead) dead = 1.0f;
        scale *= backoff;
        tracker = 0.0f;
    } else {
        t += 1.0f;
        const float tr = tracker + 1.0f;
        if (tr >= growth_interval) {
            const float grown = scale * growth;
            if (__builtin_isfinite(grown)) scale = grown;
            tracker = 0.0f;
        } else {
            tracker = tr;
        }
        if (flip_parity) parity = parity != 0.0f ? 0.0f : 1.0f;
    }
    *reinterpret_cast<float4_t*>(state) = float4_t{scale, tracker, 0.0f, t};
    state[5] = parity;
    state[7] = dead;
}
__global__ void k_update_scale(float* __restrict__ state, float growth, float backoff, float growth_interval, int flip_parity) {
    if (threadIdx.x != 0 || blockIdx.x != 0) return;
    update_scale(state, growth, backoff, growth_interval, flip_parity != 0);
}

constexpr int OPT_SMALL_THREADS = 1024;
__global__ __launch_bounds__(OPT_SMALL_THREADS) void k_adam_small_commit(OptTensors ts, float* __restrict__ state, float beta1, float beta2, float eps,
                                                                        float grad_mult, float growth, float backoff, float growth_interval,
                                                                        int flip_parity, TableAdam ta, const half_t* __restrict__ tgrad,
                                                                        uint64_t tprefix, uint32_t prefix_blocks) {
    const AdamConsts ac = adam_consts(state, beta1, beta2, grad_mult);
    const float bc2_sqrt = ac.bc2_sqrt;
    const float beta1_s = beta1, beta2_s = beta2, eps_s = eps;
    const bool prefix_role = blockIdx.x < prefix_blocks;
    const uint32_t role_blocks = prefix_role ? prefix_blocks : gridDim.x - prefix_blocks;
    const uint64_t gtid = (uint64_t)(prefix_role ? blockIdx.x : blockIdx.x - prefix_blocks) * OPT_SMALL_THREADS + threadIdx.x;
    const uint64_t gstride = (uint64_t)role_blocks * OPT_SMALL_THREADS;
    if (prefix_role && tprefix && !ac.skip) {
        const uint32_t src = state[5] != 0.0f ? 1u : 0u, dst = src ^ 1u;
        const float step_size = ta.lr * ac.lr_mult / ac.bc1;
        beta1 = ta.beta1; beta2 = ta.beta2; eps = ta.eps;
        const float4_t* __restrict__ p_in = reinterpret_cast<const float4_t*>(ta.p[src]);
        const float4_t* __restrict__ m_in = reinterpret_cast<const float4_t*>(ta.m[src]);
        const float4_t* __restrict__ v_in = reinterpret_cast<const float4_t*>(ta.v[src]);
        float4_t* __restrict__ p_out = reinterpret_cast<float4_t*>(ta.p[dst]);
        float4_t* __restrict__ m_out = reinterpret_cast<float4_t*>(ta.m[dst]);
        float4_t* __restrict__ v_out = reinterpret_cast<float4_t*>(ta.v[dst]);
        half4_t* __restrict__ h_out = reinterpret_cast<half4_t*>(ta.p16[dst]);
        const half4_t* __restrict__ g4 = reinterpret_cast<const half4_t*>(tgrad);
        const uint64_t n4 = tprefix / 4;
        for (uint64_t i = gtid; i < n4; i += 2 * gstride) {
            const uint64_t j = i + gstride;
            const bool two = j < n4;
            const uint64_t jj = two ? j : i;
            const half4_t x0 = g4[i], x1 = g4[jj];
            float4_t pm0 = m_in[i], pv0 = v_in[i], pp0 = p_in[i];
            float4_t pm1 = m_in[jj], pv1 = v_in[jj], pp1 = p_in[jj];
            half4_t ph0, ph1;
#pragma unroll
            for (int c = 0; c < 4; c++) {
                const float g0 = (float)x0[c] * ac.inv_scale, g1 = (float)x1[c] * ac.inv_scale;
                NGP_ADAM_EL(g0, pm0[c], pv0[c], pp0[c]);
                ph0[c] = (half_t)pp0[c];
                NGP_ADAM_EL(g1, pm1[c], pv1[c], pp1[c]);
                ph1[c] = (half_t)pp1[c];
            }
            m_out[i] = pm0; v_out[i] = pv0; p_out[i] = pp0; h_out[i] = ph0;
            if (two) { m_out[j] = pm1; v_out[j] = pv1; p_out[j] = pp1; h_out[j] = ph1; }
        }
    }
    for (int k = 0; !prefix_role && k < ts.count; k++) {
        const uint64_t n = ts.n[k];
        const float step_size = ts.lr[k] * ac.lr_mult / ac.bc1;
        float* __restrict__ p = ts.p[k];
        float* __restrict__ m = ts.m[k];
        float* __restrict__ v = ts.v[k];
        half_t* __restrict__ p16 = ts.p16[k];
        const bool gh = (ts.g_is_half[k] & 1) != 0, keep = (ts.g_is_half[k] & 2) != 0;
        half_t* g16 = reinterpret_cast<half_t*>(ts.g[k]);
        float* g32 = reinterpret_cast<float*>(ts.g[k]);
        for (uint64_t i = gtid; i < n; i += gstride) {
            float g = gh ? (float)g16[i] : g32[i];
            if (!keep) { if (gh) g16[i] = (half_t)0.0f; else g32[i] = 0.0f; }
            if (ac.skip) continue;
            g *= ac.inv_scale;
            float nm = m[i], nv = v[i], np_ = p[i];
            adam_element(g, nm, nv, np_, beta1_s, beta2_s, eps_s, step_size, bc2_sqrt);
            m[i] = nm; v[i] = nv; p[i] = np_;
            if (p16) p16[i] = (half_t)np_;
        }
    }
    __syncthreads();
    if (threadIdx.x == 0) {
        const float old = __hip_atomic_fetch_add(&state[6], 1.0f, __ATOMIC_RELAXED, __HIP_MEMORY_SCOPE_AGENT);
        if (old == (float)(gridDim.x - 1u)) {
            update_scale(state, growth, backoff, growth_interval, flip_parity != 0);
            __hip_atomic_store(&state[6], 0.0f, __ATOMIC_RELAXED, __HIP_MEMORY_SCOPE_AGENT);
        }
    }
}

__global__ void k_poison_shards(half_t* __restrict__ grad, uint32_t shards, uint64_t payload, const float* __restrict__ state) {
    if (state[2] == 0.0f) return;
    for (uint32_t r = threadIdx.x; r < shards; r += blockDim.x) grad[(uint64_t)r * payload] = (half_t)__builtin_nanf("");
}
__global__ void k_shard_verdict(const half_t* __restrict__ shard, float* __restrict__ state, half_t* __restrict__ flat, uint32_t shards,
                                uint64_t payload) {
    if (threadIdx.x == 0 && !__builtin_isfinite((float)shard[0])) state[2] = 1.0f;
    if (flat)
        for (uint32_t r = threadIdx.x; r < shards; r += blockDim.x)
            if (!__builtin_isfinite((float)flat[(uint64_t)r * payload])) flat[(uint64_t)r * payload] = (half_t)0.0f;
}

__global__ __launch_bounds__(OPT_THREADS) void k_ema(OptTensors ts, float omd) {
    for (int k = 0; k < ts.count; k++) {
        const uint64_t n = ts.n[k];
        const float* __restrict__ p = ts.p[k];
        float* __restrict__ e = ts.ema[k];
        for (uint64_t i = (uint64_t)blockIdx.x * OPT_THREADS + threadIdx.x; i < n; i += (uint64_t)gridDim.x * OPT_THREADS) e[i] -= omd * (e[i] - p[i]);
    }
}

}

using namespace ngp;

static uint32_t opt_blocks(uint64_t total) {
    uint32_t blocks = (uint32_t)cdiv64(total / 2 + 1, OPT_THREADS * 4);
#ifndef NGP_ADAM_MAX_BLOCKS
#define NGP_ADAM_MAX_BLOCKS 768u
#endif
    if (blocks > NGP_ADAM_MAX_BLOCKS) blocks = NGP_ADAM_MAX_BLOCKS;
// ... 38 lines not shown
            hipLaunchKernelGGL(k_check_finite, dim3(blocks), dim3(OPT_THREADS), 0, st, ts, state);
            const int rc = check_launch("optim_adam_step(check)");
            if (rc) return rc;
        }
        if (phases & NGP_OPT_PHASE_UPDATE) {
            hipLaunchKernelGGL(k_adam, dim3(blocks), dim3(OPT_THREADS), 0, st, ts, (const float*)state, beta1, beta2, eps, grad_mult,
                               ema_one_minus_decay > 0.0f ? ema_one_minus_decay : 0.0f);
            const int rc = check_launch("optim_adam_step(adam)");
            if (rc) return rc;
        }
    }
    if (phases & NGP_OPT_PHASE_COMMIT) {
        hipLaunchKernelGGL(k_update_scale, dim3(1), dim3(64), 0, st, state, growth_factor, backoff_factor, growth_interval,
                           (phases & NGP_OPT_PHASE_FLIP) ? 1 : 0);
        return check_launch("optim_adam_step(scale)");
    }
    return NGP_OK;
}

extern "C" int ngp_optim_adam_step(int count, const uint64_t* n, float* const* params, float* const* exp_avg, float* const* exp_avg_sq,
                                   void* const* grads, void* const* params_fp16, const int* grad_is_half, const float* lr, float beta1,
                                   float beta2, float eps, float grad_mult, float growth_factor, float backoff_factor, float growth_interval,
                                   float* state, ngp_stream_t stream) {
    const uint32_t phases = NGP_OPT_PHASE_CHECK | NGP_OPT_PHASE_UPDATE | (growth_interval < 0.0f ? 0u : NGP_OPT_PHASE_COMMIT);
    return ngp_optim_adam_step_ex(count, n, params, exp_avg, exp_avg_sq, grads, params_fp16, grad_is_half, lr, beta1, beta2, eps, grad_mult,
                                  growth_factor, backoff_factor, growth_interval, state, nullptr, 0.0f, phases, stream);
}

extern "C" int ngp_optim_adam_small_commit(int count, const uint64_t* n, float* const* params, float* const* exp_avg, float* const* exp_avg_sq,
                                           void* const* grads, void* const* params_fp16, const int* grad_is_half, const float* lr, float beta1,
                                           float beta2, float eps, float grad_mult, float growth_factor, float backoff_factor,
                                           float growth_interval, float* state, int flip_parity, const ngp_table_adam_t* table,
                                           const void* table_grad_fp16, uint64_t table_prefix_params, ngp_stream_t stream) {
    NGP_REQUIRE(state, NGP_ERR_INVALID, "optim_adam_small_commit: NULL state");
    NGP_REQUIRE((reinterpret_cast<uintptr_t>(state) & 15u) == 0, NGP_ERR_INVALID, "optim_adam_small_commit: state (8 floats) must be 16-byte aligned");
    NGP_REQUIRE(count >= 0 && count <= OPT_MAX_TENSORS, NGP_ERR_INVALID, "optim_adam_small_commit: at most %d tensors per call (got %d)", OPT_MAX_TENSORS,
                count);
    NGP_REQUIRE(count == 0 || (n && params && exp_avg && exp_avg_sq && grads && grad_is_half && lr), NGP_ERR_INVALID,
                "optim_adam_small_commit: NULL argument");
    OptTensors ts = {};
    ts.count = count;
    uint64_t total = 0;
    for (int k = 0; k < count; k++) {
        NGP_REQUIRE(grads[k] && params[k] && exp_avg[k] && exp_avg_sq[k], NGP_ERR_INVALID, "optim_adam_small_commit: NULL tensor %d", k);
        ts.n[k] = n[k];
        ts.p[k] = params[k];
        ts.m[k] = exp_avg[k];
        ts.v[k] = exp_avg_sq[k];
        ts.g[k] = grads[k];
        ts.p16[k] = params_fp16 ? reinterpret_cast<half_t*>(params_fp16[k]) : nullptr;
        ts.g_is_half[k] = grad_is_half[k];
        ts.lr[k] = lr[k];
        total += n[k];
    }
    TableAdam ta = {};
    if (table_prefix_params) {
        NGP_REQUIRE(table && table_grad_fp16 && table->state == state, NGP_ERR_INVALID,
                    "optim_adam_small_commit: a table prefix needs the table's buffer sets (on the same state) and its stored fp16 gradient");
        NGP_REQUIRE((table_prefix_params & 3u) == 0, NGP_ERR_INVALID, "optim_adam_small_commit: table_prefix_params must be a multiple of 4");
        for (int k = 0; k < 2; k++) {
            NGP_REQUIRE(table->param[k] && table->exp_avg[k] && table->exp_avg_sq[k] && table->param_fp16[k], NGP_ERR_INVALID,
                        "optim_adam_small_commit: NULL buffer in table set %d", k);
            ta.p[k] = table->param[k]; ta.m[k] = table->exp_avg[k]; ta.v[k] = table->exp_avg_sq[k];
            ta.p16[k] = reinterpret_cast<_Float16*>(table->param_fp16[k]);
        }
        ta.state = state;
        ta.lr = table->lr; ta.beta1 = table->beta1; ta.beta2 = table->beta2; ta.eps = table->eps;
        total += table_prefix_params;
    }
    NGP_REQUIRE(total <= (1u << 22), NGP_ERR_INVALID, "optim_adam_small_commit: %llu parameters -- this entry serves small tensors (<= 4 M); use "
                "ngp_optim_adam_step_ex", (unsigned long long)total);
    uint32_t prefix_blocks = (uint32_t)cdiv64(table_prefix_params, (uint64_t)OPT_SMALL_THREADS * 8);
    if (prefix_blocks > 192u) prefix_blocks = 192u;
    uint32_t small_blocks = (uint32_t)cdiv64(total - table_prefix_params, (uint64_t)OPT_SMALL_THREADS);
    small_blocks = small_blocks < 1u ? 1u : (small_blocks > 32u ? 32u : small_blocks);
    hipLaunchKernelGGL(k_adam_small_commit, dim3(prefix_blocks + small_blocks), dim3(OPT_SMALL_THREADS), 0, as_stream(stream), ts, state, beta1, beta2, eps,
                       grad_mult, growth_factor, backoff_factor, growth_interval, flip_parity, ta, reinterpret_cast<const half_t*>(table_grad_fp16),
                       table_prefix_params, prefix_blocks);
    return check_launch("optim_adam_small_commit");
}

extern "C" int ngp_optim_poison_shards(void* flat_grad_fp16, uint32_t shards, uint64_t payload, const float* state, ngp_stream_t stream) {
    NGP_REQUIRE(flat_grad_fp16 && state && shards >= 1 && payload >= 1, NGP_ERR_INVALID, "optim_poison_shards: NULL / empty argument");
    hipLaunchKernelGGL(k_poison_shards, dim3(1), dim3(64), 0, as_stream(stream), reinterpret_cast<half_t*>(flat_grad_fp16), shards, payload, state);
    return check_launch("optim_poison_shards");
}

extern "C" int ngp_optim_shard_verdict(const void* shard_grad_fp16, float* state, void* flat_grad_fp16, uint32_t shards, uint64_t payload,
                                       ngp_stream_t stream) {
    NGP_REQUIRE(shard_grad_fp16 && state, NGP_ERR_INVALID, "optim_shard_verdict: NULL argument");
    NGP_REQUIRE(!flat_grad_fp16 || (shards >= 1 && payload >= 1), NGP_ERR_INVALID, "optim_shard_verdict: empty shard layout");
    hipLaunchKernelGGL(k_shard_verdict, dim3(1), dim3(64), 0, as_stream(stream), reinterpret_cast<const half_t*>(shard_grad_fp16), state,
                       reinterpret_cast<half_t*>(flat_grad_fp16), shards, payload);
    return check_launch("optim_shard_verdict");
}

extern "C" int ngp_optim_ema_update(int count, const uint64_t* n, float* const* params, float* const* ema, float one_minus_decay,
                                    ngp_stream_t stream) {
    NGP_REQUIRE(count >= 1 && count <= OPT_MAX_TENSORS, NGP_ERR_INVALID, "optim_ema_update: between 1 and %d tensors per call (got %d)",
                OPT_MAX_TENSORS, count);
    NGP_REQUIRE(n && params && ema, NGP_ERR_INVALID, "optim_ema_update: NULL argument");
    OptTensors ts = {};
    ts.count = count;
    uint64_t total = 0;
    for (int k = 0; k < count; k++) {
        NGP_REQUIRE(params[k] && ema[k], NGP_ERR_INVALID, "optim_ema_update: NULL tensor %d", k);
        ts.n[k] = n[k];
        ts.p[k] = params[k];
        ts.ema[k] = ema[k];
        total += n[k];
    }
// ... 4 lines not shown
```

torch-ngp_amd/ffmlp/ffmlp.py:

```python
import math

import torch
import torch.nn as nn
from torch.autograd import Function
from torch.amp import custom_bwd, custom_fwd

try:
    import os as _os
    if _os.environ.get('NGP_HIP_LIBRARY'):
        raise ImportError('NGP_HIP_LIBRARY is set')
    import _ffmlp as _backend
except ImportError:
    from .backend import _backend

ACTIVATION_IDS = {'relu': 0, 'exponential': 1, 'sine': 2, 'sigmoid': 3, 'squareplus': 4, 'softplus': 5}


def convert_activation(act):
    return ACTIVATION_IDS.get(act, 6)


class _ffmlp_forward(Function):
    @staticmethod
    @custom_fwd(device_type='cuda', cast_inputs=torch.half)
# ... 21 lines not shown
        input_dim, output_dim, hidden_dim, num_layers, activation, output_activation, calc_grad_inputs = ctx.net
        grad = grad.contiguous()
        batch = grad.shape[0]
        grad_inputs = torch.empty_like(inputs) if calc_grad_inputs else torch.empty(1, device=grad.device, dtype=grad.dtype)
        grad_weights = torch.empty_like(weights)
        backward_buffer = torch.empty(num_layers, batch, hidden_dim, device=grad.device, dtype=grad.dtype)
        _backend.ffmlp_backward(grad, inputs, weights, forward_buffer, batch, input_dim, output_dim, hidden_dim, num_layers,
                                activation, output_activation, calc_grad_inputs, backward_buffer, grad_inputs, grad_weights)
        return (grad_inputs if calc_grad_inputs else None), grad_weights, None, None, None, None, None, None, None, None


ffmlp_forward = _ffmlp_forward.apply


class FFMLP(nn.Module):
    def __init__(self, input_dim, output_dim, hidden_dim, num_layers, activation='relu'):
        super().__init__()
        assert hidden_dim in [16, 32, 64, 128, 256], f"FFMLP only support hidden_dim in [16, 32, 64, 128, 256], but got {hidden_dim}"
        assert input_dim > 0 and input_dim % 16 == 0, f"FFMLP input_dim should be 16 * m (m  > 0), but got {input_dim}"
        assert output_dim <= 16, f"FFMLP current only supports output dim <= 16, but got {output_dim}"
        assert num_layers >= 2, f"FFMLP num_layers should be larger than 2 (3 matmuls), but got {num_layers}"

        self.input_dim = input_dim
        self.output_dim = output_dim
        self.hidden_dim = hidden_dim
        self.num_layers = num_layers
        self.activation = convert_activation(activation)
        self.output_activation = convert_activation('none')
        self.tensorcore_width = 16
        self.padded_output_dim = int(math.ceil(output_dim / 16)) * 16

        self.num_parameters = hidden_dim * (input_dim + hidden_dim * (num_layers - 1) + self.padded_output_dim)
        self.weights = nn.Parameter(torch.zeros(self.num_parameters))
        self.reset_parameters()
        _backend.allocate_splitk(self.num_layers + 1)

    def cleanup(self):
        _backend.free_splitk()

    def __repr__(self):
        return (f"FFMLP: input_dim={self.input_dim} output_dim={self.output_dim} hidden_dim={self.hidden_dim} "
                f"num_layers={self.num_layers} activation={self.activation}")

    def reset_parameters(self):
        torch.manual_seed(42)
        bound = math.sqrt(3 / self.hidden_dim)
        self.weights.data.uniform_(-bound, bound)

    def forward(self, inputs):
        batch, width = inputs.shape
        pad = 128 - (batch % 128)
        padded = torch.cat([inputs, torch.zeros(pad, width, dtype=inputs.dtype, device=inputs.device)], dim=0)
        out = ffmlp_forward(padded, self.weights, self.input_dim, self.padded_output_dim, self.hidden_dim, self.num_layers,
                            self.activation, self.output_activation, not self.training, padded.requires_grad)
        return out[:batch, :self.output_dim]
```

torch-ngp_amd/fused.py:

```python
import ctypes
import os
from collections import namedtuple

import numpy as np
import torch
from torch.autograd import Function

import _ngp_capi as capi
from optim import announce_overwrite, clean_deposits, resync_stale_shadows

_PLANAR_IN = capi.NGP_FF_INPUT_PLANAR
_PLANAR_DX = capi.NGP_FF_DX_PLANAR

NetCfg = namedtuple('NetCfg', 'bound L S H gridtype align interp nl_sigma nl_color training')
RenderCfg = namedtuple('RenderCfg', 'cascade grid_size min_near capacity perturb dt_gamma max_steps T_thresh density_scale bg_scalar')
Marched = namedtuple('Marched', 'xyzs dirs deltas rays nears fars ws')
Saved = namedtuple('Saved', 'xyzs offsets enc ws16 wc16 fb_s fb_c h16 color_in rgb sigma deltas rays weights_sum image_raw bg march_ws')
Bufs = namedtuple('Bufs', 'emb16 ws16 wc16 g_emb g_ws g_wc')


def _grid_forward(x, emb16, offsets, enc, M, L, S, H, gridtype, align, interp, bound, costs, st):
    sel = getattr(emb16, '_ngp_sel', None)
    if sel is not None:
        capi.check(capi.lib.ngp_grid_encode_forward_sel(x.data_ptr(), emb16.data_ptr(), sel[0].data_ptr(), sel[1].data_ptr(), None, offsets.data_ptr(),
                                                         enc.data_ptr(), M, 3, 2, L, S, H, gridtype, align, interp, capi.NGP_F16, float(bound), costs, st))
    else:
        capi.check(capi.lib.ngp_grid_encode_forward_sched(x.data_ptr(), emb16.data_ptr(), offsets.data_ptr(), enc.data_ptr(), M, 3, 2, L, S, H,
                                                           None, gridtype, align, interp, capi.NGP_F16, float(bound), costs, st))


class _fused_ngp(Function):
    @staticmethod
    def forward(ctx, x, d, embeddings, w_sigma, w_color, offsets, cfg, bufs, density_scale=1.0):
        M = x.shape[0]
        dev = x.device
        st = capi.stream()
        x = x.contiguous()
        d = d.contiguous()
        half = dict(device=dev, dtype=torch.half)

        enc = torch.empty(cfg.L, M, 2, **half)
        costs = capi.ray_level_costs(cfg.L, cfg.S, cfg.H, 3.0 ** 0.5 / (1024.0 * max(float(cfg.bound), 1e-6))) if USE_BALANCED_FORWARD else None
        _grid_forward(x, bufs.emb16, offsets, enc, M, cfg.L, cfg.S, cfg.H, cfg.gridtype, cfg.align, cfg.interp, cfg.bound, costs, st)
        h16 = torch.empty(M, 16, **half)
        color_in = torch.empty(M, 32, **half)
        out16 = torch.empty(M, 16, **half)
        sigma = torch.empty(M, device=dev, dtype=torch.float32)
        rgb = torch.empty(M, 3, device=dev, dtype=torch.float32)
        d_valid = d.shape[0]
        if cfg.training:
            fb_s = torch.empty(cfg.nl_sigma, M, 64, **half)
            fb_c = torch.empty(cfg.nl_color, M, 64, **half)
        else:
            fb_s = fb_c = None
        assert not cfg.training or density_scale == 1.0, 'the backward of _fused_ngp knows no density scale (the fused training render folds it itself)'
        _network_forward(enc, d, d_valid, bufs.ws16, bufs.wc16, cfg.nl_sigma, cfg.nl_color, float(density_scale), cfg.training, fb_s, h16, sigma,
                         color_in, fb_c, out16, rgb, M, st)
        if cfg.training:
            ctx.save_for_backward(x, offsets, enc, bufs.ws16, bufs.wc16, fb_s, fb_c, h16, color_in, rgb)
            ctx.cfg = cfg
            ctx.n_emb = embeddings.shape[0]
            ctx.bufs = bufs
        return sigma, rgb

    @staticmethod
    def backward(ctx, grad_sigma, grad_rgb):
        x, offsets, enc, ws16, wc16, fb_s, fb_c, h16, color_in, rgb = ctx.saved_tensors
        cfg = ctx.cfg
        nl_sigma, nl_color = cfg.nl_sigma, cfg.nl_color
        M = x.shape[0]
        dev = x.device
        st = capi.stream()
        half = dict(device=dev, dtype=torch.half)
        grad_sigma = torch.zeros(M, device=dev) if grad_sigma is None else grad_sigma.contiguous().float()
        grad_rgb = torch.zeros(M, 3, device=dev) if grad_rgb is None else grad_rgb.contiguous().float()

        g_out16 = torch.empty(M, 16, **half)
        capi.check(capi.lib.ngp_pipeline_rgb_backward(grad_rgb.data_ptr(), rgb.data_ptr(), g_out16.data_ptr(), M, st))
        g_color_in = torch.empty(M, 32, **half)
        g_emb, g_ws, g_wc, deposited = _grad_targets(ctx.bufs, ctx.n_emb, dev)
        scratch_c = torch.empty(nl_color, M, 64, **half)
        capi.check(capi.lib.ngp_ffmlp_backward_ex(g_out16.data_ptr(), color_in.data_ptr(), wc16.data_ptr(), fb_c.data_ptr(), M, 32, 16, 64,
                                                   nl_color, 0, 6, 1, scratch_c.data_ptr(), g_color_in.data_ptr(), g_wc.data_ptr(), 0, st))
        g_h16 = g_out16
        capi.check(capi.lib.ngp_pipeline_mid_backward(grad_sigma.data_ptr(), h16.data_ptr(), g_color_in.data_ptr(), g_h16.data_ptr(), M, 1.0, st))
        g_enc = torch.empty(cfg.L, M, 2, **half)
        scratch_s = scratch_c[:nl_sigma]
        capi.check(capi.lib.ngp_ffmlp_backward_ex(g_h16.data_ptr(), enc.data_ptr(), ws16.data_ptr(), fb_s.data_ptr(), M, 32, 16, 64, nl_sigma,
                                                   0, 6, 1, scratch_s.data_ptr(), g_enc.data_ptr(), g_ws.data_ptr(), _PLANAR_IN | _PLANAR_DX, st))
        _grid_backward(g_enc, x, offsets, g_emb, M, cfg.L, cfg.S, cfg.H, cfg.gridtype, cfg.align, cfg.interp, cfg.bound, st)
        if deposited:
            return None, None, None, None, None, None, None, None, None
        return None, None, g_emb, g_ws, g_wc, None, None, None, None


USE_FUSED_NETWORK = True


def _network_forward(enc, dirs, d_valid, ws16, wc16, nl_sigma, nl_color, density_scale, training, fb_s, h16, sigma, color_in, fb_c, out16, rgb, M, st):
    if USE_FUSED_NETWORK:
        capi.check(capi.lib.ngp_network_forward(enc.data_ptr(), dirs.data_ptr(), M, d_valid, ws16.data_ptr(), wc16.data_ptr(), nl_sigma, nl_color,
                                                 float(density_scale), 1 if training else 0, capi.ptr(fb_s), capi.ptr(h16) if training else None,
                                                 sigma.data_ptr(), capi.ptr(color_in) if training else None, capi.ptr(fb_c), rgb.data_ptr(), _PLANAR_IN, st))
        return
    if training:
        capi.check(capi.lib.ngp_ffmlp_forward_ex(enc.data_ptr(), ws16.data_ptr(), M, 32, 16, 64, nl_sigma, 0, 6, fb_s.data_ptr(), h16.data_ptr(),
                                                  _PLANAR_IN, st))
    else:
        capi.check(capi.lib.ngp_ffmlp_inference_ex(enc.data_ptr(), ws16.data_ptr(), M, 32, 16, 64, nl_sigma, 0, 6, None, h16.data_ptr(), _PLANAR_IN, st))
    capi.check(capi.lib.ngp_pipeline_mid_forward(h16.data_ptr(), dirs.data_ptr(), sigma.data_ptr(), color_in.data_ptr(), M, d_valid, float(density_scale), st))
    if training:
        capi.check(capi.lib.ngp_ffmlp_forward_ex(color_in.data_ptr(), wc16.data_ptr(), M, 32, 16, 64, nl_color, 0, 6, fb_c.data_ptr(), out16.data_ptr(), 0, st))
    else:
        capi.check(capi.lib.ngp_ffmlp_inference_ex(color_in.data_ptr(), wc16.data_ptr(), M, 32, 16, 64, nl_color, 0, 6, None, out16.data_ptr(), 0, st))
    capi.check(capi.lib.ngp_pipeline_rgb_forward(out16.data_ptr(), rgb.data_ptr(), M, st))


def _grid_backward(g_enc, x, offsets, g_emb, M, L, S, H, gridtype, align, interp, bound, st, found_inf=None, slabs=None, overwrite=False,
                   table_adam=None):
    arr, ws, nbytes = capi.grid_backward_workspace(offsets, M, 3, 2, L, S, H, gridtype, align, capi.NGP_F16)
    if overwrite:
        slabs = slabs if slabs is not None else capi.SlabSets()
        slabs.overwrite_table = 1
    if table_adam is not None:
        if not overwrite:
            raise RuntimeError('fused: table_adam needs overwrite_table')
        slabs.table_adam = ctypes.cast(ctypes.pointer(table_adam), ctypes.c_void_p)
    if found_inf is not None and arr is None:
        raise RuntimeError('fused: the in-kernel non-finite sweep needs the host copy of the encoder offsets (call iteration_checks_gradients '
                           'outside stream capture first)')
    capi.check(capi.lib.ngp_grid_encode_backward_checked_slabs(g_enc.data_ptr(), x.data_ptr(), None, offsets.data_ptr(), capi.ptr(g_emb), M, 3, 2, L, S,
                                                                 H, None, None, gridtype, align, interp, capi.NGP_F16, float(bound),
                                                                 None if arr is None else ctypes.cast(arr, ctypes.c_void_p), capi.ptr(ws), nbytes,
                                                                 capi.ptr(found_inf), None if slabs is None else ctypes.cast(ctypes.pointer(slabs), ctypes.c_void_p),
                                                                 st))

# ... 28 lines not shown
    cfg = network_cfg(encoder, sigma_net, color_net, bound, training)
    params = (encoder.embeddings, sigma_net.weights, color_net.weights)
    return _fused_ngp.apply(x, d, *params, encoder.offsets, cfg, _operands(params, deposit=training), density_scale)


def _render_train_march(rays_o, rays_d, bitfield, aabb, counter, cfg, rcfg, noise_seed=None, into=None):
    N = rays_o.shape[0]
    M = rcfg.capacity
    dev = rays_o.device
    st = capi.stream()
    f32 = dict(device=dev, dtype=torch.float32)
    if into is not None:
        (xyzs, dirs, deltas, rays, nears, fars, ws) = into
    else:
        nears = torch.empty(N, **f32)
        fars = torch.empty(N, **f32)
        xyzs = torch.empty(M, 3, **f32)
        dirs = torch.empty(M, 3, **f32)
        deltas = torch.empty(M, 2, **f32)
        rays = torch.empty(N, 3, device=dev, dtype=torch.int32)
        ws = torch.empty(capi.lib.ngp_march_rays_train_workspace_bytes(N), dtype=torch.uint8, device=dev)
    march_flags = capi.NGP_MARCH_RESET_COUNTER | capi.NGP_MARCH_ZERO_TAIL | (0 if USE_FUSED_SCAN else capi.NGP_MARCH_SCAN_LAUNCH)
    if rcfg.perturb and noise_seed is not None:
        noises, march_flags = noise_seed, march_flags | capi.NGP_MARCH_NOISE_FROM_SEED
    else:
        noises = torch.rand(N, **f32) if rcfg.perturb else torch.zeros(N, **f32)
    capi.check(capi.lib.ngp_march_rays_train_aabb(rays_o.data_ptr(), rays_d.data_ptr(), bitfield.data_ptr(), float(cfg.bound), float(rcfg.dt_gamma),
                                                   rcfg.max_steps, N, rcfg.cascade, rcfg.grid_size, M, aabb.data_ptr(), float(rcfg.min_near),
                                                   nears.data_ptr(), fars.data_ptr(), xyzs.data_ptr(), dirs.data_ptr(), deltas.data_ptr(),
                                                   rays.data_ptr(), counter.data_ptr(), noises.data_ptr(), ws.data_ptr(), march_flags, st))
    return Marched(xyzs, dirs, deltas, rays, nears, fars, ws)


def _render_train_network(marched, bufs, bg, offsets, cfg, rcfg, composite=True):
    xyzs, rays = marched.xyzs, marched.rays
    nl_sigma, nl_color = cfg.nl_sigma, cfg.nl_color
    N, M = rays.shape[0], rcfg.capacity
    dev = xyzs.device
    st = capi.stream()
    f32 = dict(device=dev, dtype=torch.float32)
    half = dict(device=dev, dtype=torch.half)
    enc = torch.empty(cfg.L, M, 2, **half)
    costs = capi.ray_level_costs(cfg.L, cfg.S, cfg.H, 3.0 ** 0.5 / (rcfg.max_steps * max(float(cfg.bound), 1e-6))) if USE_BALANCED_FORWARD else None
    _grid_forward(xyzs, bufs.emb16, offsets, enc, M, cfg.L, cfg.S, cfg.H, cfg.gridtype, cfg.align, cfg.interp, cfg.bound, costs, st)
    h16 = torch.empty(M, 16, **half)
    color_in = torch.empty(M, 32, **half)
    out16 = torch.empty(M, 16, **half)
    sigma = torch.empty(M, **f32)
    rgb = torch.empty(M, 3, **f32)
    if _recompute(nl_sigma, nl_color):
        fb_s = fb_c = None
    else:
        fb_s = torch.empty(nl_sigma, M, 64, **half)
        fb_c = torch.empty(nl_color, M, 64, **half)
    _network_forward(enc, marched.dirs, M, bufs.ws16, bufs.wc16, nl_sigma, nl_color, float(rcfg.density_scale), True, fb_s, h16, sigma, color_in, fb_c,
                     out16, rgb, M, st)
    saved = Saved(xyzs, offsets, enc, bufs.ws16, bufs.wc16, fb_s, fb_c, h16, color_in, rgb, sigma, marched.deltas, rays, weights_sum=None,
                  image_raw=None, bg=bg, march_ws=marched.ws)
    if not composite:
        return saved
    weights_sum = torch.empty(N, **f32)
    depth_raw = torch.empty(N, **f32)
    image_raw = torch.empty(N, 3, **f32)
    image = torch.empty(N, 3, **f32)
    depth = torch.empty(N, **f32)
    bg_mode = 2 if bg is not None else 1
    capi.check(capi.lib.ngp_composite_rays_train_forward_ex(sigma.data_ptr(), rgb.data_ptr(), marched.deltas.data_ptr(), rays.data_ptr(), M, N,
                                                             float(rcfg.T_thresh), weights_sum.data_ptr(), depth_raw.data_ptr(), image_raw.data_ptr(),
                                                             bg_mode, float(rcfg.bg_scalar), capi.ptr(bg), marched.nears.data_ptr(),
                                                             marched.fars.data_ptr(), image.data_ptr(), depth.data_ptr(), st))
    return image, depth, weights_sum, saved._replace(weights_sum=weights_sum, image_raw=image_raw)


def _render_train_backward(saved, cfg, rcfg, grad_image, grad_ws, g_emb, g_ws, g_wc, found_inf=None, overwrite=False):
    s = saved
    M, N = s.xyzs.shape[0], s.rays.shape[0]
    dev = s.xyzs.device
    st = capi.stream()
    g_sigma = torch.empty(M, device=dev)
    g_rgb = torch.empty(M, 3, device=dev)
    bg_mode = 2 if s.bg is not None else 1
    capi.check(capi.lib.ngp_composite_rays_train_backward_ex(capi.ptr(grad_ws), grad_image.data_ptr(), s.sigma.data_ptr(), s.rgb.data_ptr(),
                                                              s.deltas.data_ptr(), s.rays.data_ptr(), s.weights_sum.data_ptr(),
                                                              s.image_raw.data_ptr(), M, N, float(rcfg.T_thresh), g_sigma.data_ptr(),
                                                              g_rgb.data_ptr(), bg_mode, float(rcfg.bg_scalar), capi.ptr(s.bg),
                                                              s.march_ws.data_ptr(), st))
    g_out16 = torch.empty(M, 16, device=dev, dtype=torch.half)
    capi.check(capi.lib.ngp_pipeline_rgb_backward(g_rgb.data_ptr(), s.rgb.data_ptr(), g_out16.data_ptr(), M, st))
    _network_backward(saved, cfg, rcfg, g_sigma, g_out16, g_emb, g_ws, g_wc, found_inf, None, overwrite)


def _network_backward(saved, cfg, rcfg, g_sigma, g_out16, g_emb, g_ws, g_wc, found_inf=None, loss_job=None, overwrite=False, table_adam=None):
    s = saved
    nl_sigma, nl_color, density_scale = cfg.nl_sigma, cfg.nl_color, rcfg.density_scale
    grid = (cfg.L, cfg.S, cfg.H, cfg.gridtype, cfg.align, cfg.interp, cfg.bound)
    M = s.xyzs.shape[0]
    st = capi.stream()
    half = dict(device=s.xyzs.device, dtype=torch.half)
    g_enc = torch.empty(cfg.L, M, 2, **half)
    if USE_FUSED_MID and nl_color in (2, 3) and nl_sigma in (2, 3):
        scratch_c = torch.empty(nl_color, M, 64, **half)
        scratch_s = torch.empty(nl_sigma, M, 64, **half)
        g_h16 = torch.empty(M, 16, **half)
        rc = capi.NGP_FF_RECOMPUTE if s.fb_c is None else 0
        capi.check(capi.lib.ngp_network_backward_color(g_out16.data_ptr(), s.color_in.data_ptr(), s.wc16.data_ptr(), capi.ptr(s.fb_c), M, nl_color,
                                                        scratch_c.data_ptr(), g_sigma.data_ptr(), s.h16.data_ptr(), float(density_scale),
                                                        g_h16.data_ptr(), g_wc.data_ptr(), capi.NGP_FF_DEFER_REDUCE | rc, st))
        capi.check(capi.lib.ngp_ffmlp_backward_ex(g_h16.data_ptr(), s.enc.data_ptr(), s.ws16.data_ptr(), capi.ptr(s.fb_s), M, 32, 16, 64, nl_sigma,
                                                   0, 6, 1, scratch_s.data_ptr(), g_enc.data_ptr(), g_ws.data_ptr(),
                                                   _PLANAR_IN | _PLANAR_DX | capi.NGP_FF_DEFER_REDUCE | rc, st))
        n_c, n_s = capi.lib.ngp_ffmlp_backward_slab_count(M, 32, 64, nl_color), capi.lib.ngp_ffmlp_backward_slab_count(M, 32, 64, nl_sigma)
        if USE_SLABS_IN_ACCUMULATE:
            err, loss = loss_job if loss_job is not None else (None, None)
            slabs = capi.SlabSets(scratch_c.data_ptr(), n_c, g_wc.numel(), g_wc.data_ptr(), scratch_s.data_ptr(), n_s, g_ws.numel(), g_ws.data_ptr(),
                                  capi.ptr(err), 0 if err is None else err.numel(), capi.ptr(loss))
            _grid_backward(g_enc, s.xyzs, s.offsets, g_emb, M, *grid, st, found_inf, slabs, overwrite, table_adam)
            return
        if loss_job is not None:
            raise RuntimeError('fused: a deferred loss sum needs the carried reductions (_carries_reductions)')
        capi.check(capi.lib.ngp_ffmlp_reduce_slabs_pair(scratch_c.data_ptr(), n_c, g_wc.numel(), g_wc.data_ptr(), scratch_s.data_ptr(), n_s, g_ws.numel(),
                                                         g_ws.data_ptr(), capi.ptr(found_inf), st))
    else:
        if found_inf is not None:
            raise RuntimeError('fused: found_inf needs the fused colour-head / slab-reduction path (see iteration_checks_gradients)')
        if loss_job is not None:
            raise RuntimeError('fused: a deferred loss sum needs the carried reductions (_carries_reductions)')
        g_color_in = torch.empty(M, 32, **half)
        scratch = torch.empty(max(nl_color, nl_sigma), M, 64, **half)
        capi.check(capi.lib.ngp_ffmlp_backward_ex(g_out16.data_ptr(), s.color_in.data_ptr(), s.wc16.data_ptr(), s.fb_c.data_ptr(), M, 32, 16, 64,
                                                   nl_color, 0, 6, 1, scratch.data_ptr(), g_color_in.data_ptr(), g_wc.data_ptr(), 0, st))
        g_h16 = g_out16
        capi.check(capi.lib.ngp_pipeline_mid_backward(g_sigma.data_ptr(), s.h16.data_ptr(), g_color_in.data_ptr(), g_h16.data_ptr(), M,
                                                       float(density_scale), st))
        capi.check(capi.lib.ngp_ffmlp_backward_ex(g_h16.data_ptr(), s.enc.data_ptr(), s.ws16.data_ptr(), s.fb_s.data_ptr(), M, 32, 16, 64, nl_sigma,
                                                   0, 6, 1, scratch[:nl_sigma].data_ptr(), g_enc.data_ptr(), g_ws.data_ptr(),
                                                   _PLANAR_IN | _PLANAR_DX, st))
    _grid_backward(g_enc, s.xyzs, s.offsets, g_emb, M, *grid, st, found_inf, None, overwrite, table_adam)


class _fused_render_train(Function):
    @staticmethod
    def forward(ctx, rays_o, rays_d, embeddings, w_sigma, w_color, bg, offsets, bitfield, aabb, counter, cfg, rcfg, bufs):
        marched = _render_train_march(rays_o, rays_d, bitfield, aabb, counter, cfg, rcfg)
        image, depth, weights_sum, saved = _render_train_network(marched, bufs, bg, offsets, cfg, rcfg)
        ctx.save_for_backward(*saved)
        ctx.cfg, ctx.rcfg, ctx.n_emb, ctx.bufs = cfg, rcfg, embeddings.shape[0], bufs
        ctx.mark_non_differentiable(depth)
        return image, depth, weights_sum

    @staticmethod
    def backward(ctx, grad_image, grad_depth, grad_ws):
        saved = Saved(*ctx.saved_tensors)
        dev = saved.xyzs.device
        N = saved.rays.shape[0]
        grad_image = torch.zeros(N, 3, device=dev) if grad_image is None else grad_image.contiguous().float()
        grad_ws = None if grad_ws is None else grad_ws.contiguous().float()
        g_emb, g_ws, g_wc, deposited = _grad_targets(ctx.bufs, ctx.n_emb, dev)
        _render_train_backward(saved, ctx.cfg, ctx.rcfg, grad_image, grad_ws, g_emb, g_ws, g_wc)
        if deposited:
            return (None,) * 13
        return None, None, g_emb, g_ws, g_wc, None, None, None, None, None, None, None, None


def network_cfg(encoder, sigma_net, color_net, bound, training):
    return NetCfg(float(bound), int(encoder.num_levels), float(np.log2(encoder.per_level_scale)), int(encoder.base_resolution),
                  int(encoder.gridtype_id), int(bool(encoder.align_corners)), int(encoder.interp_id), int(sigma_net.num_layers),
                  int(color_net.num_layers), bool(training))


# ... 16 lines not shown
def fused_train_iteration(model, rays_o, rays_d, target, box, counter, capacity, loss_scale, bg_color=1, perturb=False, dt_gamma=0,
                          max_steps=1024, T_thresh=1e-4, noise_seed=None, found_inf=None, overwrite_table=False, table_adam=None):
    march, rest = fused_train_iteration_split(model, rays_o, rays_d, target, box, counter, capacity, loss_scale, bg_color, perturb, dt_gamma,
                                              max_steps, T_thresh, noise_seed, found_inf, overwrite_table, table_adam)
    march()
    return rest()


def _table_adam_prefix(model, cfg, M):
    arr = capi.host_offsets(model.encoder.offsets)
    prefix = int(capi.lib.ngp_grid_table_adam_prefix(ctypes.cast(arr, ctypes.c_void_p), int(M), 3, 2, cfg.L, cfg.S, cfg.H, cfg.gridtype, cfg.align,
                                                     capi.NGP_F16))
    if prefix == 0xffffffff:
        raise RuntimeError('fused: table_adam: this batch / table shape cannot carry the sweep (ngp_grid_table_adam_prefix)')
    return prefix


def _table_adam_of(optimizer, model):
    if optimizer is None:
        return None
    if getattr(optimizer, 'fused_table', None) is not model.encoder.embeddings:
        raise RuntimeError('fused: table_adam: call optimizer.enable_table_fusion(model.encoder.embeddings) first')
    return optimizer.table_adam()


USE_BALANCED_FORWARD = True
USE_FUSED_CHECK = True
USE_FUSED_SCAN = True
USE_FUSED_MID = True
USE_FUSED_COMPOSITE = True
USE_OVERWRITE_TABLE = os.environ.get('NGP_FUSED_OVERWRITE_TABLE', '1') != '0'
USE_SLABS_IN_ACCUMULATE = os.environ.get('NGP_FUSED_SLABS_IN_ACCUMULATE', '1') != '0'
USE_RECOMPUTE = os.environ.get('NGP_FUSED_RECOMPUTE', '0') == '1'


def _carries_reductions(nl_sigma, nl_color):
    return bool(USE_SLABS_IN_ACCUMULATE and USE_FUSED_MID and nl_color in (2, 3) and nl_sigma in (2, 3))


def _recompute(nl_sigma, nl_color):
    return bool(USE_RECOMPUTE and USE_FUSED_NETWORK and USE_FUSED_MID and nl_color in (2, 3) and nl_sigma in (2, 3))


def iteration_checks_gradients(model):
    nl = (int(model.sigma_net.num_layers), int(model.color_net.num_layers))
    return bool(USE_FUSED_CHECK and USE_FUSED_MID and all(n in (2, 3) for n in nl) and capi.host_offsets(model.encoder.offsets) is not None)


def _train_iteration_rest(marched, bufs, bg_t, offsets, target, loss_scale, cfg, rcfg, found_inf=None, overwrite=False, table_adam=None):
    if table_adam is not None and not (USE_FUSED_COMPOSITE and found_inf is not None and overwrite):
        raise RuntimeError('fused: table_adam needs the fused compositor, the in-kernel non-finite sweep (found_inf) and overwrite_table')
    g_emb, g_ws, g_wc = bufs.g_emb, bufs.g_ws.view(-1), bufs.g_wc.view(-1)
    if not USE_FUSED_COMPOSITE:
        image, depth, weights_sum, saved = _render_train_network(marched, bufs, bg_t, offsets, cfg, rcfg)
        loss = torch.empty(1, device=image.device, dtype=torch.float32)
        grad_image = torch.empty_like(image)
        capi.check(capi.lib.ngp_pipeline_mse_loss(image.data_ptr(), target.data_ptr(), image.numel(), capi.ptr(loss_scale), loss.data_ptr(),
                                                   grad_image.data_ptr(), capi.stream()))
        _render_train_backward(saved, cfg, rcfg, grad_image, None, g_emb, g_ws, g_wc, found_inf, overwrite)
        return loss, image, depth, weights_sum
    s = _render_train_network(marched, bufs, bg_t, offsets, cfg, rcfg, composite=False)
    N, M, dev = s.rays.shape[0], s.xyzs.shape[0], s.xyzs.device
    f32 = dict(device=dev, dtype=torch.float32)
    weights_sum, image, depth = torch.empty(N, **f32), torch.empty(N, 3, **f32), torch.empty(N, **f32)
    loss, ray_err = torch.empty(1, **f32), torch.empty(N, **f32)
    g_sigma = torch.empty(M, **f32)
    g_out16 = torch.empty(M, 16, device=dev, dtype=torch.half)
    defer = _carries_reductions(cfg.nl_sigma, cfg.nl_color)
    capi.check(capi.lib.ngp_composite_train_loss_backward(s.sigma.data_ptr(), s.rgb.data_ptr(), s.deltas.data_ptr(), s.rays.data_ptr(), M, N,
                                                           float(rcfg.T_thresh), 2 if s.bg is not None else 1, float(rcfg.bg_scalar), capi.ptr(s.bg),
                                                           marched.nears.data_ptr(), marched.fars.data_ptr(), target.data_ptr(),
                                                           capi.ptr(loss_scale), weights_sum.data_ptr(), image.data_ptr(), depth.data_ptr(),
                                                           None if defer else loss.data_ptr(), ray_err.data_ptr(), g_sigma.data_ptr(),
                                                           g_out16.data_ptr(), s.march_ws.data_ptr(),
                                                           s.march_ws.numel() * s.march_ws.element_size(), capi.stream()))
    _network_backward(s, cfg, rcfg, g_sigma, g_out16, g_emb, g_ws, g_wc, found_inf, loss_job=(ray_err, loss) if defer else None,
                      overwrite=overwrite, table_adam=table_adam)
    return loss, image, depth, weights_sum


@torch.no_grad()
def fused_train_iteration_split(model, rays_o, rays_d, target, box, counter, capacity, loss_scale, bg_color=1, perturb=False, dt_gamma=0,
                                max_steps=1024, T_thresh=1e-4, noise_seed=None, found_inf=None, overwrite_table=False, table_adam=None):
    cfg = network_cfg(model.encoder, model.sigma_net, model.color_net, model.bound, True)
    bg_t, rcfg = _render_cfg(model, capacity, bg_color, perturb, dt_gamma, max_steps, T_thresh)
    bufs = _operands((model.encoder.embeddings, model.sigma_net.weights, model.color_net.weights), True, overwrite_table)
    if bufs.g_emb is None:
        raise RuntimeError('fused_train_iteration: the parameters are not managed by optim.NGPAdam(deposit=True)')
    rays_o = rays_o.contiguous().view(-1, 3)
    rays_d = rays_d.contiguous().view(-1, 3)
    target = target.contiguous().view(-1, 3)
    if target.shape[0] != rays_o.shape[0] or target.dtype != torch.float32:
        raise RuntimeError('fused_train_iteration: target must be [N,3] float32')
    box_ = {}

    def march():
        box_['m'] = _render_train_march(rays_o, rays_d, model.density_bitfield, box, counter, cfg, rcfg, noise_seed, into=box_.get('m'))

    def rest():
        ta = _table_adam_of(table_adam, model)
        out = _train_iteration_rest(box_['m'], bufs, bg_t, model.encoder.offsets, target, loss_scale, cfg, rcfg, found_inf, overwrite_table, ta)
        if overwrite_table:
            announce_overwrite(model.encoder.embeddings, None if ta is None else _table_adam_prefix(model, cfg, capacity))
        return out
    return march, rest


density_point_spacing = None


@torch.no_grad()
def fused_density(x, encoder, sigma_net, bound):
    M = x.shape[0]
    dev = x.device
    st = capi.stream()
    emb16, w16 = _half_weights((encoder.embeddings, sigma_net.weights))
    L = int(encoder.num_levels)
    enc = torch.empty(L, M, 2, device=dev, dtype=torch.half)
    S, H = float(np.log2(encoder.per_level_scale)), int(encoder.base_resolution)
    costs = None if density_point_spacing is None else capi.ray_level_costs(L, S, H, float(density_point_spacing))
    _grid_forward(x.contiguous(), emb16, encoder.offsets, enc, M, L, S, H, int(encoder.gridtype_id), int(bool(encoder.align_corners)),
                  int(encoder.interp_id), bound, costs, st)
    h16 = torch.empty(M, 16, device=dev, dtype=torch.half)
    capi.check(capi.lib.ngp_ffmlp_inference_ex(enc.data_ptr(), w16.data_ptr(), M, 32, 16, 64, int(sigma_net.num_layers), 0, 6, None, h16.data_ptr(),
                                                _PLANAR_IN, st))
    return torch.exp(h16[:, 0].float()), h16[:, 1:]


def inference_weights(model, x):
    enc, sn, cn = getattr(model, 'encoder', None), getattr(model, 'sigma_net', None), getattr(model, 'color_net', None)
    if enc is None or sn is None or cn is None or torch.is_grad_enabled():
        return None
    probe = torch.empty(128, 3, device=x.device, dtype=torch.float32)
    if not getattr(model, '_fused_ok', lambda *_: False)(probe, probe):
        return None
    emb16, ws16, wc16 = _half_weights((enc.embeddings, sn.weights, cn.weights), cast=False)
    if emb16 is None or ws16 is None or wc16 is None or getattr(emb16, '_ngp_sel', None) is not None:
        return None
    return emb16, ws16, wc16, network_cfg(enc, sn, cn, model.bound, False)


class pinned_half_weights:

    def __init__(self, model):
        enc, sn, cn = getattr(model, 'encoder', None), getattr(model, 'sigma_net', None), getattr(model, 'color_net', None)
        self.params = [getattr(enc, 'embeddings', None), getattr(sn, 'weights', None), getattr(cn, 'weights', None)]

    def __enter__(self):
        if all(p is not None and p.is_cuda for p in self.params) and not torch.is_grad_enabled():
            for p in self.params:
                fn = getattr(p, '_ngp_materialize', None)
                if fn is not None:
                    fn()
                buf = getattr(p, '_ngp_fp16_pinbuf', None)
                if buf is None or buf.shape != p.shape or buf.device != p.device:
                    buf = torch.empty_like(p, dtype=torch.half)
                    p._ngp_fp16_pinbuf = buf
                buf.copy_(p.detach())
                p._ngp_fp16_pin = buf
        return self

    def __exit__(self, *exc):
        for p in self.params:
            if p is not None and hasattr(p, '_ngp_fp16_pin'):
                del p._ngp_fp16_pin
        return False
```

torch-ngp_amd/optim.py:

```python
import ctypes

import torch
import torch.distributed as dist

import _ngp_capi as capi

_MAX = 8


def announce_overwrite(p, table_adam_prefix=None):
    p._ngp_deposit_overwritten = True
    if table_adam_prefix is not None:
        p._ngp_table_adam_prefix = int(table_adam_prefix)
        p._ngp_table_adam_done = True


def _consumed(p, kept):
    p._ngp_deposit_overwritten = False
    p._ngp_grad16_stale = kept


def replayed_kept_deposits(params):
    for p in params:
        if getattr(p, '_ngp_grad16', None) is not None:
            p._ngp_grad16_stale = True


def replayed_fused_table_step(optimizer):
    if getattr(optimizer, 'fused_table', None) is not None:
        optimizer._maybe_flipped = True


SMALL_COMMIT_MAX_PARAMS = 1 << 22


def table_fusion_fits(prefix_entries, level_dim, rest_params):
    return int(prefix_entries) * int(level_dim) + int(rest_params) <= SMALL_COMMIT_MAX_PARAMS


def clean_deposits(params):
    for p in params:
        if getattr(p, '_ngp_grad16_stale', False):
            p._ngp_grad16.zero_()
            p._ngp_grad16_stale = False


def refresh_shadow(p):
    p._ngp_fp16.copy_(p.detach())
    p._ngp_version = p._version


def resync_stale_shadows(params):
    for p in params:
        if getattr(p, '_ngp_fp16', None) is not None and getattr(p, '_ngp_version', None) != p._version:
            with torch.no_grad():
                refresh_shadow(p)


class NGPAdam:
    _require_cuda = True

    def __init__(self, params, lr=1e-2, betas=(0.9, 0.99), eps=1e-15, init_scale=65536.0, growth_factor=2.0, backoff_factor=0.5,
                 growth_interval=2000, world_size=1, deposit=True, shard=False, rank=None, process_group=None, verdict='poison'):
        groups = list(params)
        if groups and not isinstance(groups[0], dict):
            groups = [{'params': groups}]
        self.param_groups = []
        for g in groups:
            ps = [p for p in g['params'] if p.requires_grad]
            self.param_groups.append({'params': ps, 'lr': float(g.get('lr', lr))})
        self.betas, self.eps = (float(betas[0]), float(betas[1])), float(eps)
        self.growth_factor, self.backoff_factor, self.growth_interval = float(growth_factor), float(backoff_factor), float(growth_interval)
        self.world_size = int(world_size)
        self.group = process_group
        self.shard = bool(shard) and (self.world_size > 1 or shard == 'force')
        if verdict not in ('poison', 'allreduce'):
            raise ValueError("NGPAdam: verdict must be 'poison' or 'allreduce'")
        self.verdict = verdict
        if self.shard and not deposit:
            raise RuntimeError('NGPAdam: shard=True needs deposit=True (the flat fp16 gradient buffer is what gets reduce-scattered)')
        self.rank = (dist.get_rank(process_group) if rank is None else int(rank)) if self.shard else 0
        self.check_mixed_gradients = False
        self.state = {}
        dev = None
        flat_params = [p for g in self.param_groups for p in g['params']]
        for p in flat_params:
            if not ((p.is_cuda or not self._require_cuda) and p.dtype == torch.float32 and p.is_contiguous()):
                raise RuntimeError('NGPAdam: parameters must be contiguous float32 CUDA tensors')
            dev = p.device
        self.flat_params = flat_params
        self.offsets, total = [], 0
        for p in flat_params:
            self.offsets.append(total)
            total += (p.numel() + 7) // 8 * 8
        self.payload = total
        if self.shard:
            self.payload = ((total + self.world_size - 1) // self.world_size + 7) // 8 * 8
            total = self.payload * self.world_size
        self.total = total
        self.flat_grad16 = self.flat_p16 = self.flat_master = None
        if deposit:
            self.flat_grad16 = torch.zeros(total, dtype=torch.half, device=dev)
            self.flat_p16 = torch.zeros(total, dtype=torch.half, device=dev)
        if self.shard:
            self.flat_master = torch.zeros(total, dtype=torch.float32, device=dev)
            self.shard_grad = torch.zeros(self.payload, dtype=torch.half, device=dev)
            self.exp_avg = torch.zeros(self.payload, dtype=torch.float32, device=dev)
            self.exp_avg_sq = torch.zeros(self.payload, dtype=torch.float32, device=dev)
            self.shard_range = (self.rank * self.payload, (self.rank + 1) * self.payload)
        for p, off in zip(flat_params, self.offsets):
            n = p.numel()
            st = {}
            if self.shard:
                self.flat_master[off:off + n].copy_(p.detach().reshape(-1))
                p.data = self.flat_master[off:off + n].view_as(p)
            else:
                st.update(exp_avg=torch.zeros_like(p), exp_avg_sq=torch.zeros_like(p))
            if deposit:
                st['fp16'] = self.flat_p16[off:off + n].view_as(p)
                st['fp16'].copy_(p.detach())
                st['grad16'] = self.flat_grad16[off:off + n].view_as(p)
                p._ngp_fp16, p._ngp_grad16, p._ngp_version = st['fp16'], st['grad16'], p._version
            self.state[p] = st
        self.scalars = torch.tensor([init_scale, 0.0, 0.0, 0.0, 1.0, 0.0, 0.0, 0.0], dtype=torch.float32, device=dev)
        self._scale_view = self.scalars[0]
        self._keep = []
        self._comm_stream = None
        self._shadows_ready = None
        self.fused_table = None
        self._table_alt = None
        self._maybe_flipped = False

    def enable_table_fusion(self, param):
        if self.shard or self.world_size > 1:
            raise RuntimeError('NGPAdam.enable_table_fusion: the sharded / data-parallel update exchanges the gradient first (not available)')
        st = self.state.get(param)
        if st is None or 'fp16' not in st or 'exp_avg' not in st:
            raise RuntimeError('NGPAdam.enable_table_fusion: the parameter is not a deposit-managed parameter of this optimizer')
        if self.fused_table is param:
            return
        if self.fused_table is not None:
            raise RuntimeError('NGPAdam.enable_table_fusion: one table per optimizer')
        self._table_alt = {'p': torch.empty_like(param.data), 'm': torch.empty_like(st['exp_avg']), 'v': torch.empty_like(st['exp_avg_sq']),
                           'p16': torch.empty_like(st['fp16'])}
        for t in self._table_alt.values():
            t.zero_()
        self.fused_table = param
        self.scalars[5:6].zero_()
        st['fp16']._ngp_sel = (self._table_alt['p16'], self.scalars[5:6])
        param._ngp_materialize = self.materialize

    def table_adam(self):
        if self.fused_table is None:
# ... 223 lines not shown
                    continue
                entries.append((p, st, grad, is_half, g['lr']))
        return entries

    clean_deposits = staticmethod(clean_deposits)

    def _deposit_used(self, st):
        if torch.cuda.is_current_stream_capturing() or not self.check_mixed_gradients:
            return False
        return bool(st['grad16'].ne(0).any().item())

    def _entry_arrays(self, entries, ema):
        k = len(entries)
        if not k:
            return [None] * 9
        vp = ctypes.c_void_p

        def ptrs(i):
            return (vp * k)(*[(e[i].data_ptr() if e[i] is not None else None) for e in entries])
        arrs = ((ctypes.c_uint64 * k)(*[int(e[0]) for e in entries]), ptrs(1), ptrs(2), ptrs(3), ptrs(4), ptrs(5),
                (ctypes.c_int * k)(*[int(e[6]) for e in entries]), (ctypes.c_float * k)(*[float(e[7]) for e in entries]), ptrs(8) if ema else None)
        self._keep.append((arrs, entries))
        return [ctypes.cast(a, vp) if a is not None else None for a in arrs]

    def _launch(self, entries, phases, omd):
        cast = self._entry_arrays(entries, ema=omd > 0.0)
        capi.check(capi.lib.ngp_optim_adam_step_ex(len(entries), cast[0], cast[1], cast[2], cast[3], cast[4], cast[5], cast[6], cast[7], self.betas[0],
                                                   self.betas[1], self.eps, 1.0, self.growth_factor, self.backoff_factor, self.growth_interval,
                                                   self.scalars.data_ptr(), cast[8], float(omd), phases, capi.stream()))

    def _launch_small_commit(self, entries, flip, table_prefix=0):
        k, cast = len(entries), self._entry_arrays(entries, ema=False)
        ta = self._table_adam_struct() if table_prefix else None
        capi.check(capi.lib.ngp_optim_adam_small_commit(k, cast[0], cast[1], cast[2], cast[3], cast[4], cast[5], cast[6], cast[7], self.betas[0],
                                                        self.betas[1], self.eps, 1.0, self.growth_factor, self.backoff_factor, self.growth_interval,
                                                        self.scalars.data_ptr(), 1 if flip else 0,
                                                        None if ta is None else ctypes.cast(ctypes.pointer(ta), ctypes.c_void_p),
                                                        self.state[self.fused_table]['grad16'].data_ptr() if table_prefix else None,
                                                        int(table_prefix), capi.stream()))

    @torch.no_grad()
    def step(self, update_ema=None, gradients_checked=False):
        self._keep = []
        CHECK, UPDATE, COMMIT = capi.NGP_OPT_PHASE_CHECK, capi.NGP_OPT_PHASE_UPDATE, capi.NGP_OPT_PHASE_COMMIT
        if self.shard:
            if update_ema is not None:
                raise RuntimeError('NGPAdam(shard=True): fold-in EMA is not available; call gather_master() then ema.update() once per epoch')
            if any(p.grad is not None for p in self.flat_params):
                raise RuntimeError('NGPAdam(shard=True): gradients must be deposited by the fused path (found an autograd .grad)')
            self._refuse_stale_deposits('step')
            if not gradients_checked:
                self.pre_reduce_check()
            self.poison_shards()
            self.reduce_gradients()
            self.apply()
            self.gather_shadows()
            self.wait_shadows()
            return
        table_done = self.fused_table is not None and getattr(self.fused_table, '_ngp_table_adam_done', False)
        if table_done:
            self.fused_table._ngp_table_adam_done = False
            if update_ema is not None or not gradients_checked:
                raise RuntimeError('NGPAdam.step: a fused-table step needs gradients_checked=True (the producers raise found_inf) and no fold-in EMA')
            self.clean_deposits([p for p in self.flat_params if p is not self.fused_table and not getattr(p, '_ngp_deposit_overwritten', False)])
            entries = [(p.numel(), p, st['exp_avg'], st['exp_avg_sq'], grad, st.get('fp16'), is_half, lr, None)
                       for p, st, grad, is_half, lr in self._entries() if p is not self.fused_table]
            if len(entries) > _MAX or not all(e[6] & 1 for e in entries):
                raise RuntimeError('NGPAdam.step: a fused-table step serves at most 8 remaining tensors, all with deposited fp16 gradients')
            prefix = int(getattr(self.fused_table, '_ngp_table_adam_prefix', 0)) * int(self.fused_table.shape[1])
            self._launch_small_commit(entries, flip=True, table_prefix=prefix)
            return
        self.materialize()
        self.clean_deposits([p for p in self.flat_params if not getattr(p, '_ngp_deposit_overwritten', False)])
        omd = update_ema.begin_update() if update_ema is not None else 0.0
        entries = [(p.numel(), p, st['exp_avg'], st['exp_avg_sq'], grad, st.get('fp16'), is_half, lr,
                    update_ema.shadow_of(p) if update_ema is not None else None) for p, st, grad, is_half, lr in self._entries()]
        chunks = [entries[i:i + _MAX] for i in range(0, len(entries), _MAX)]
        checked = gradients_checked and all(e[6] & 1 for e in entries)
        if len(chunks) == 1:
            self._launch(chunks[0], (0 if checked else CHECK) | UPDATE | COMMIT, omd)
        else:
            for c in ([] if checked else chunks):
                self._launch(c, CHECK, 0.0)
            for c in chunks:
                self._launch(c, UPDATE, omd)
            self._launch([], COMMIT, 0.0)

    def load_torch_adam_state(self, adam_sd, scaler_sd=None):
        flat = [p for g in self.param_groups for p in g['params']]
        self.materialize()
        ids = [i for g in adam_sd['param_groups'] for i in g['params']]
        if len(ids) != len(flat):
            raise RuntimeError(f'NGPAdam: checkpoint has {len(ids)} parameters, the optimizer {len(flat)}')
        step = 0.0
        for p, i in zip(flat, ids):
            st = adam_sd['state'].get(i)
            if st is None:
                continue
            self._set_moments(p, st['exp_avg'], st['exp_avg_sq'])
            step = max(step, float(st['step']))
        self.scalars[3:4].fill_(step)
        factors = []
        for g, tg in zip(self.param_groups, adam_sd['param_groups']):
            base = float(tg.get('initial_lr', tg['lr']))
            g['lr'] = base
            factors.append(float(tg['lr']) / base if base != 0.0 else 1.0)
        if factors:
            if max(factors) - min(factors) > 1e-6 * max(1.0, max(factors)):
                for g, f in zip(self.param_groups, factors):
                    g['lr'] *= f
                self.set_lr_scale(1.0)
            else:
                self.set_lr_scale(factors[0])
        if scaler_sd:
            self.scalars[0:1].fill_(float(scaler_sd.get('scale', self.get_scale())))
            self.scalars[1:2].fill_(float(scaler_sd.get('_growth_tracker', 0)))
        self._sync_shadows(assume_complete=True)


# ... 136 lines not shown
```

Baseline: 625.3 million.

## Precompute MLP weight fragment images in global memory once per optimizer step

```diff
diff --git a/include/ngp_hip.h b/include/ngp_hip.h
--- a/include/ngp_hip.h
+++ b/include/ngp_hip.h
@@ -189,6 +189,7 @@
 #define NGP_FF_SINGLE_WAVE 8u
 #define NGP_FF_DEFER_REDUCE 16u
 #define NGP_FF_RECOMPUTE 32u
+#define NGP_FF_WEIGHT_IMAGES 64u
 int ngp_ffmlp_forward_ex(const void* inputs, const void* weights, uint32_t B, uint32_t input_dim, uint32_t output_dim,
                          uint32_t hidden_dim, uint32_t num_layers, uint32_t activation, uint32_t output_activation,
                          void* forward_buffer, void* outputs, uint32_t flags, ngp_stream_t stream);
@@ -200,6 +201,13 @@
                           uint32_t B, uint32_t input_dim, uint32_t output_dim, uint32_t hidden_dim, uint32_t num_layers,
                           uint32_t activation, uint32_t output_activation, int calc_grad_inputs, void* backward_buffer,
                           void* grad_inputs, void* grad_weights, uint32_t flags, ngp_stream_t stream);
+
+size_t ngp_ffmlp_forward_image_offset(uint32_t input_dim, uint32_t hidden_dim, uint32_t num_layers);
+size_t ngp_ffmlp_forward_image_bytes(uint32_t input_dim, uint32_t hidden_dim, uint32_t num_layers);
+size_t ngp_ffmlp_backward_image_offset(uint32_t input_dim, uint32_t hidden_dim, uint32_t num_layers);
+size_t ngp_ffmlp_backward_image_bytes(uint32_t input_dim, uint32_t hidden_dim, uint32_t num_layers);
+size_t ngp_ffmlp_weights_with_images_bytes(uint32_t input_dim, uint32_t hidden_dim, uint32_t num_layers);
+int ngp_ffmlp_build_weight_images(void* weights_and_images, uint32_t input_dim, uint32_t hidden_dim, uint32_t num_layers, ngp_stream_t stream);
 
 size_t ngp_ffmlp_backward_workspace_bytes(uint32_t B, uint32_t input_dim, uint32_t hidden_dim, uint32_t num_layers);
 int ngp_ffmlp_backward_ws(const void* grad, const void* inputs, const void* weights, const void* forward_buffer, uint32_t B,
@@ -339,6 +347,12 @@
                                 float beta2, float eps, float grad_mult, float growth_factor, float backoff_factor, float growth_interval,
                                 float* state, int flip_parity, const struct ngp_table_adam* table, const void* table_grad_fp16,
                                 uint64_t table_prefix_params, ngp_stream_t stream);
+int ngp_optim_adam_small_commit_images(int count, const uint64_t* n, float* const* params, float* const* exp_avg, float* const* exp_avg_sq,
+                                       void* const* grads, void* const* params_fp16, const int* grad_is_half, const float* lr, float beta1,
+                                       float beta2, float eps, float grad_mult, float growth_factor, float backoff_factor,
+                                       float growth_interval, float* state, int flip_parity, const struct ngp_table_adam* table,
+                                       const void* table_grad_fp16, uint64_t table_prefix_params, const uint32_t* image_shapes,
+                                       ngp_stream_t stream);
 int ngp_optim_poison_shards(void* flat_grad_fp16, uint32_t shards, uint64_t payload, const float* state, ngp_stream_t stream);
 int ngp_optim_shard_verdict(const void* shard_grad_fp16, float* state, void* flat_grad_fp16, uint32_t shards, uint64_t payload,
                             ngp_stream_t stream);
diff --git a/torch-ngp_amd/_ngp_capi.py b/torch-ngp_amd/_ngp_capi.py
--- a/torch-ngp_amd/_ngp_capi.py
+++ b/torch-ngp_amd/_ngp_capi.py
@@ -8,6 +8,7 @@
 
 NGP_F32, NGP_F16, NGP_F64 = 0, 1, 2
 NGP_FF_INPUT_PLANAR, NGP_FF_DX_PLANAR, NGP_FF_LAYERED, NGP_FF_SINGLE_WAVE, NGP_FF_DEFER_REDUCE, NGP_FF_RECOMPUTE = 1, 2, 4, 8, 16, 32
+NGP_FF_WEIGHT_IMAGES = 64
 NGP_MARCH_RESET_COUNTER, NGP_MARCH_ZERO_TAIL, NGP_MARCH_NOISE_FROM_SEED, NGP_MARCH_SCAN_LAUNCH = 1, 2, 4, 8
 NGP_OPT_PHASE_CHECK, NGP_OPT_PHASE_UPDATE, NGP_OPT_PHASE_COMMIT, NGP_OPT_PHASE_FLIP = 1, 2, 4, 8
 ABI_VERSION = 11
@@ -98,6 +99,9 @@
     'ngp_optim_adam_step_ex': [_i32, _vp, _vp, _vp, _vp, _vp, _vp, _vp, _vp, _f32, _f32, _f32, _f32, _f32, _f32, _f32, _vp, _vp, _f32, _u32, _vp],
     'ngp_optim_adam_small_commit': [_i32, _vp, _vp, _vp, _vp, _vp, _vp, _vp, _vp, _f32, _f32, _f32, _f32, _f32, _f32, _f32, _vp, _i32, _vp, _vp,
                                     ctypes.c_uint64, _vp],
+    'ngp_optim_adam_small_commit_images': [_i32, _vp, _vp, _vp, _vp, _vp, _vp, _vp, _vp, _f32, _f32, _f32, _f32, _f32, _f32, _f32, _vp, _i32, _vp, _vp,
+                                           ctypes.c_uint64, _vp, _vp],
+    'ngp_ffmlp_build_weight_images': [_vp, _u32, _u32, _u32, _vp],
     'ngp_optim_ema_update': [_i32, _vp, _vp, _vp, _f32, _vp],
     'ngp_optim_poison_shards': [_vp, _u32, ctypes.c_uint64, _vp, _vp],
     'ngp_optim_shard_verdict': [_vp, _vp, _vp, _u32, ctypes.c_uint64, _vp],
@@ -136,6 +140,11 @@
 lib.ngp_linear_stack_flat_size.argtypes = [_u32, _u32, _u32, _u32, _i32]
 lib.ngp_linear_stack_flat_size.restype = _u32
 lib.ngp_density_grid_update_workspace_bytes.restype = _sz
+_IMAGE_LAYOUT = ['ngp_ffmlp_forward_image_offset', 'ngp_ffmlp_forward_image_bytes', 'ngp_ffmlp_backward_image_offset', 'ngp_ffmlp_backward_image_bytes',
+                 'ngp_ffmlp_weights_with_images_bytes']
+for _name in _IMAGE_LAYOUT:
+    getattr(lib, _name).argtypes = [_u32, _u32, _u32]
+    getattr(lib, _name).restype = _sz
 
 if lib.ngp_abi_version() != ABI_VERSION:
     raise ImportError(f"{LIB_PATH}: ABI version {lib.ngp_abi_version()} != expected {ABI_VERSION}; rebuild the extension")
@@ -145,7 +154,7 @@
                                        'ngp_grid_backward_workspace_bytes', 'ngp_ffmlp_backward_workspace_bytes',
                                        'ngp_ffmlp_backward_slab_count', 'ngp_density_grid_update_workspace_bytes', 'ngp_grid_forward_work_lists', 'ngp_coarse_occupancy_bytes',
                                        'ngp_grid_table_adam_prefix', 'ngp_linear_stack_flat_size',
-                                       'ngp_grid_backward_backward_workspace_bytes'])
+                                       'ngp_grid_backward_backward_workspace_bytes'] + _IMAGE_LAYOUT)
 
 
 def check(rc):
@@ -173,6 +182,14 @@
 class TableAdam(ctypes.Structure):
     _fields_ = [('param', ctypes.c_void_p * 2), ('exp_avg', ctypes.c_void_p * 2), ('exp_avg_sq', ctypes.c_void_p * 2), ('param_fp16', ctypes.c_void_p * 2),
                 ('state', ctypes.c_void_p), ('lr', ctypes.c_float), ('beta1', ctypes.c_float), ('beta2', ctypes.c_float), ('eps', ctypes.c_float)]
+
+
+def weight_image_halves(shape):
+    return int(lib.ngp_ffmlp_weights_with_images_bytes(*[int(v) for v in shape])) // 2
+
+
+def build_weight_images(weights16, shape):
+    check(lib.ngp_ffmlp_build_weight_images(weights16.data_ptr(), int(shape[0]), int(shape[1]), int(shape[2]), stream()))
 
 
 def ptr(t):
diff --git a/torch-ngp_amd/csrc/ffmlp.hip b/torch-ngp_amd/csrc/ffmlp.hip
--- a/torch-ngp_amd/csrc/ffmlp.hip
+++ b/torch-ngp_amd/csrc/ffmlp.hip
@@ -1,4 +1,5 @@
 #include "common.h"
+#include "ffmlp_images.h"
 #include "sh_poly.inc"
 
 namespace ngp {
@@ -180,6 +181,31 @@
     }
 }
 
+template <int BATCH>
+__device__ __forceinline__ void copy_weight_images(half8_t* img, const half8_t* __restrict__ src_a, uint32_t n_a, const half8_t* __restrict__ src_b = nullptr,
+                                                   uint32_t n_b = 0u) {
+    const uint32_t total = n_a + n_b;
+    for (uint32_t e0 = threadIdx.x; e0 < total; e0 += BATCH * blockDim.x) {
+        half8_t v[BATCH];
+#pragma unroll
+        for (int b = 0; b < BATCH; b++) {
+            const uint32_t e = e0 + b * blockDim.x < total ? e0 + b * blockDim.x : e0;
+            v[b] = e < n_a ? src_a[e] : src_b[e - n_a];
+        }
+#pragma unroll
+        for (int b = 0; b < BATCH; b++) {
+            const uint32_t e = e0 + b * blockDim.x;
+            if (e < total) img[e] = v[b];
+        }
+    }
+}
+__device__ __forceinline__ const half8_t* forward_image_of(const half_t* weights, uint32_t in_dim, uint32_t hidden, uint32_t num_layers) {
+    return reinterpret_cast<const half8_t*>(reinterpret_cast<const unsigned char*>(weights) + ff_image_layout(in_dim, hidden, num_layers).fwd_off);
+}
+__device__ __forceinline__ const half8_t* backward_image_of(const half_t* weights, uint32_t in_dim, uint32_t hidden, uint32_t num_layers) {
+    return reinterpret_cast<const half8_t*>(reinterpret_cast<const unsigned char*>(weights) + ff_image_layout(in_dim, hidden, num_layers).bwd_off);
+}
+
 template <int WIDTH>
 __device__ __forceinline__ void pack_hidden(const float16_t (&acc)[Shape<WIDTH>::NIB], half8_t (&frag)[Shape<WIDTH>::NKB]) {
 #pragma unroll
@@ -229,11 +255,13 @@
 template <int WIDTH, bool TRAIN, bool PLAIN >
 __device__ __forceinline__ void ffmlp_forward_body(const half_t* __restrict__ inputs, const half_t* __restrict__ weights,
                                                    half_t* __restrict__ forward_buffer, half_t* __restrict__ outputs, uint32_t n_tiles,
-                                                   uint32_t in_dim, uint32_t num_layers, uint32_t act, uint32_t out_act, bool in_planar) {
+                                                   uint32_t in_dim, uint32_t num_layers, uint32_t act, uint32_t out_act, bool in_planar,
+                                                   bool images) {
     constexpr int NIB = Shape<WIDTH>::NIB, NKB = Shape<WIDTH>::NKB;
     extern __shared__ __attribute__((aligned(16))) unsigned char smem[];
     half8_t* img = reinterpret_cast<half8_t*>(smem);
-    build_forward_image<WIDTH>(img, weights, in_dim, num_layers);
+    if (images) copy_weight_images<4>(img, forward_image_of(weights, in_dim, WIDTH, num_layers), fwd_frag_count<WIDTH>(in_dim, num_layers) * 64u);
+    else build_forward_image<WIDTH>(img, weights, in_dim, num_layers);
     const size_t rows = (size_t)n_tiles * FF_TILE;
     __syncthreads();
 
@@ -300,14 +328,14 @@
 template <int WIDTH, bool TRAIN, bool PLAIN>
 __global__ __launch_bounds__(FF_THREADS) __attribute__((amdgpu_waves_per_eu(4, 4))) void k_ffmlp_forward(
     const half_t* __restrict__ inputs, const half_t* __restrict__ weights, half_t* __restrict__ forward_buffer, half_t* __restrict__ outputs,
-    uint32_t n_tiles, uint32_t in_dim, uint32_t num_layers, uint32_t act, uint32_t out_act, bool in_planar) {
-    ffmlp_forward_body<WIDTH, TRAIN, PLAIN>(inputs, weights, forward_buffer, outputs, n_tiles, in_dim, num_layers, act, out_act, in_planar);
+    uint32_t n_tiles, uint32_t in_dim, uint32_t num_layers, uint32_t act, uint32_t out_act, bool in_planar, bool images) {
+    ffmlp_forward_body<WIDTH, TRAIN, PLAIN>(inputs, weights, forward_buffer, outputs, n_tiles, in_dim, num_layers, act, out_act, in_planar, images);
 }
 template <int WIDTH, bool TRAIN, bool PLAIN>
 __global__ __launch_bounds__(FF_THREADS) __attribute__((amdgpu_waves_per_eu(2, 2))) void k_ffmlp_forward_wide(
     const half_t* __restrict__ inputs, const half_t* __restrict__ weights, half_t* __restrict__ forward_buffer, half_t* __restrict__ outputs,
-    uint32_t n_tiles, uint32_t in_dim, uint32_t num_layers, uint32_t act, uint32_t out_act, bool in_planar) {
-    ffmlp_forward_body<WIDTH, TRAIN, PLAIN>(inputs, weights, forward_buffer, outputs, n_tiles, in_dim, num_layers, act, out_act, in_planar);
+    uint32_t n_tiles, uint32_t in_dim, uint32_t num_layers, uint32_t act, uint32_t out_act, bool in_planar, bool images) {
+    ffmlp_forward_body<WIDTH, TRAIN, PLAIN>(inputs, weights, forward_buffer, outputs, n_tiles, in_dim, num_layers, act, out_act, in_planar, images);
 }
 
 
@@ -356,7 +384,7 @@
     const half_t* __restrict__ enc, bool enc_planar, const float* __restrict__ dirs, uint32_t M_valid, const half_t* __restrict__ w_sigma,
     const half_t* __restrict__ w_color, half_t* __restrict__ fb_s, half_t* __restrict__ h16, float* __restrict__ sigma,
     half_t* __restrict__ color_in, half_t* __restrict__ fb_c, float* __restrict__ rgb, uint32_t n_tiles_cap, uint32_t nl_s, uint32_t nl_c,
-    float density_scale, const uint32_t* __restrict__ rows_dev) {
+    float density_scale, const uint32_t* __restrict__ rows_dev, bool images) {
     constexpr int WIDTH = 64, NIB = 2, NKB = 4;
     constexpr uint32_t in_kb = 2;
     const uint32_t n_tiles = rows_dev ? min(n_tiles_cap, (rows_dev[0] + (uint32_t)FF_TILE - 1u) / (uint32_t)FF_TILE) : n_tiles_cap;
@@ -386,8 +414,13 @@
         }
     };
     request(blockIdx.x * WAVES + wid);
-    build_forward_image<WIDTH>(img_s, w_sigma, 32, nl_s);
-    build_forward_image<WIDTH>(img_c, w_color, 32, nl_c);
+    if (images) {
+        copy_weight_images<10>(img_s, forward_image_of(w_sigma, 32, WIDTH, nl_s), frags_s * 64u, forward_image_of(w_color, 32, WIDTH, nl_c),
+                               (NIB * in_kb + (nl_c - 1) * NIB * NKB + NKB) * 64u);
+    } else {
+        build_forward_image<WIDTH>(img_s, w_sigma, 32, nl_s);
+        build_forward_image<WIDTH>(img_c, w_color, 32, nl_c);
+    }
     __syncthreads();
 
     const size_t layer_stride = (size_t)n_tiles_cap * NKB * 64;
@@ -708,12 +741,14 @@
                                                                const half_t* __restrict__ weights, const half_t* __restrict__ forward_buffer,
                                                                uint32_t n_tiles, uint32_t in_dim, uint32_t num_layers, uint32_t act,
                                                                bool with_dx, half_t* __restrict__ grad_inputs, float* __restrict__ slabs,
-                                                               half_t* __restrict__ grad_weights_direct, bool in_planar, bool dx_planar, uint32_t pf_depth) {
+                                                               half_t* __restrict__ grad_weights_direct, bool in_planar, bool dx_planar, uint32_t pf_depth,
+                                                               bool images) {
     constexpr int NIB = Shape<WIDTH>::NIB, NKB = Shape<WIDTH>::NKB;
     extern __shared__ __attribute__((aligned(16))) unsigned char smem[];
     half8_t* img = reinterpret_cast<half8_t*>(smem);
     const uint32_t nfrag = bwd_frag_count<WIDTH>(in_dim, num_layers, with_dx);
-    build_backward_image<WIDTH>(img, weights, in_dim, num_layers, with_dx);
+    if (images) copy_weight_images<4>(img, backward_image_of(weights, in_dim, WIDTH, num_layers), nfrag * 64u);
+    else build_backward_image<WIDTH>(img, weights, in_dim, num_layers, with_dx);
     const int lane = threadIdx.x & 63, wid = threadIdx.x >> 6;
     const int n = lane & 31, h = lane >> 5;
     (void)nfrag;
@@ -949,7 +984,8 @@
 void k_ffmlp_backward_paired(const half_t* __restrict__ grad, const half_t* __restrict__ inputs, const half_t* __restrict__ weights,
                              const half_t* __restrict__ forward_buffer, uint32_t n_tiles, uint32_t in_dim, uint32_t num_layers, uint32_t act,
                              bool with_dx, half_t* __restrict__ grad_inputs, float* __restrict__ slabs,
-                             half_t* __restrict__ grad_weights_direct, bool in_planar, bool dx_planar, uint32_t pf_depth, MidEpilogue mid) {
+                             half_t* __restrict__ grad_weights_direct, bool in_planar, bool dx_planar, uint32_t pf_depth, MidEpilogue mid,
+                             bool images) {
     static_assert(NHM == 1 || NHM == 2, "the paired backward covers 2- and 3-layer networks");
     constexpr int NIB = Shape<WIDTH>::NIB, NKB = Shape<WIDTH>::NKB;
     extern __shared__ __attribute__((aligned(16))) unsigned char smem[];
@@ -981,8 +1017,12 @@
         for (uint32_t d = 0; d + 1 < (pf_depth > 1 ? pf_depth : 2u); d++)
             if (blockIdx.x * FP_PAIRS + d * base_step + pair < n_tiles) prefetch(d, blockIdx.x * FP_PAIRS + d * base_step + pair);
     }
-    build_backward_image<WIDTH>(img, weights, in_dim, num_layers, with_dx);
-    if (RECOMP) build_forward_image<WIDTH>(img + (size_t)nfrag * 64, weights, in_dim, num_layers, 0, ffrag);
+    if (images) copy_weight_images<3>(img, backward_image_of(weights, in_dim, WIDTH, num_layers), nfrag * 64u);
+    else build_backward_image<WIDTH>(img, weights, in_dim, num_layers, with_dx);
+    if constexpr (RECOMP) {
+        if (images) copy_weight_images<3>(img + (size_t)nfrag * 64, forward_image_of(weights, in_dim, WIDTH, num_layers), ffrag * 64u);
+        else build_forward_image<WIDTH>(img + (size_t)nfrag * 64, weights, in_dim, num_layers, 0, ffrag);
+    }
     const Selectors sel = make_selectors(n, h);
     __syncthreads();
 
@@ -1591,6 +1631,8 @@
     return NGP_OK;
 }
 
+static bool weight_images_readable(const void* weights) { return (reinterpret_cast<uintptr_t>(weights) & 15u) == 0; }
+
 static int raise_lds(const void* kern, size_t lds, const char* what) {
     if (lds > 64 * 1024) {
         hipError_t e = hipFuncSetAttribute(kern, hipFuncAttributeMaxDynamicSharedMemorySize, (int)lds);
@@ -1632,7 +1674,10 @@
                           uint32_t out_act, void* fwd, void* outputs, uint32_t flags, hipStream_t st) {
     const uint32_t n_tiles = B / FF_TILE;
     const size_t lds = forward_image_bytes<WIDTH>(in_dim, num_layers);
-    if (WIDTH > 128 || lds > 152 * 1024 || (flags & NGP_FF_LAYERED))
+    const bool layered = WIDTH > 128 || lds > 152 * 1024 || (flags & NGP_FF_LAYERED);
+    NGP_REQUIRE(!(flags & NGP_FF_WEIGHT_IMAGES) || (!layered && weight_images_readable(weights)), NGP_ERR_INVALID,
+                "ffmlp: NGP_FF_WEIGHT_IMAGES serves the register-resident kernels and needs 16-byte aligned weights");
+    if (layered)
         return launch_forward_layered<WIDTH, TRAIN>(inputs, weights, B, in_dim, num_layers, act, out_act, fwd, outputs, flags, st);
     if constexpr (WIDTH > 128) {
         return NGP_ERR_INVALID;
@@ -1653,8 +1698,8 @@
     half_t* a2 = (half_t*)fwd;
     half_t* a3 = (half_t*)outputs;
     uint32_t a4 = n_tiles, a5 = in_dim, a6 = num_layers, a7 = act, a8 = out_act;
-    bool a9 = (flags & NGP_FF_INPUT_PLANAR) != 0;
-    void* args[] = {&a0, &a1, &a2, &a3, &a4, &a5, &a6, &a7, &a8, &a9};
+    bool a9 = (flags & NGP_FF_INPUT_PLANAR) != 0, a10 = (flags & NGP_FF_WEIGHT_IMAGES) != 0;
+    void* args[] = {&a0, &a1, &a2, &a3, &a4, &a5, &a6, &a7, &a8, &a9, &a10};
     hipError_t e = hipLaunchKernel(kern, dim3(blocks), dim3(FF_THREADS), args, lds, st);
     NGP_REQUIRE(e == hipSuccess, NGP_ERR_LAUNCH, "ffmlp: kernel launch failed: %s", hipGetErrorString(e));
     return check_launch(TRAIN ? "ffmlp_forward" : "ffmlp_inference");
@@ -1733,7 +1778,8 @@
                            uint32_t num_layers, uint32_t act, bool with_dx, void* backward_buffer, void* grad_inputs,
                            void* grad_weights, uint32_t flags, hipStream_t st, const MidEpilogue* mid_in) {
     const bool in_planar = (flags & NGP_FF_INPUT_PLANAR) != 0, dx_planar = (flags & NGP_FF_DX_PLANAR) != 0;
-    const bool defer = (flags & NGP_FF_DEFER_REDUCE) != 0;
+    const bool defer = (flags & NGP_FF_DEFER_REDUCE) != 0, images = (flags & NGP_FF_WEIGHT_IMAGES) != 0;
+    NGP_REQUIRE(!images || weight_images_readable(weights), NGP_ERR_INVALID, "ffmlp_backward: NGP_FF_WEIGHT_IMAGES needs 16-byte aligned weights");
     const MidEpilogue mid = mid_in ? *mid_in : MidEpilogue{nullptr, nullptr, nullptr, 0.0f};
     constexpr int NIB = Shape<WIDTH>::NIB, NKB = Shape<WIDTH>::NKB;
     const uint32_t n_tiles = B / FF_TILE;
@@ -1763,7 +1809,7 @@
             hipLaunchKernelGGL(pk, dim3(direct ? 1 : blocks), dim3(FP_THREADS), lds_r, st, (const half_t*)grad, (const half_t*)inputs,
                                (const half_t*)weights, (const half_t*)nullptr, n_tiles, in_dim, num_layers, act, with_dx, (half_t*)grad_inputs,
                                direct ? (float*)nullptr : (float*)backward_buffer, direct ? (half_t*)grad_weights : (half_t*)nullptr, in_planar,
-                               dx_planar, depth, mid);
+                               dx_planar, depth, mid, images);
             int rc = check_launch("ffmlp_backward");
             if (rc || direct || defer) return rc;
             hipLaunchKernelGGL(k_ffmlp_reduce_slabs, dim3(cdiv(n_params, RS_PARAMS)), dim3(RS_PARAMS * RS_GROUPS), 0, st,
@@ -1784,7 +1830,7 @@
             hipLaunchKernelGGL(pk, dim3(direct ? 1 : blocks), dim3(FP_THREADS), lds, st, (const half_t*)grad, (const half_t*)inputs,
                                (const half_t*)weights, (const half_t*)fwd, n_tiles, in_dim, num_layers, act, with_dx, (half_t*)grad_inputs,
                                direct ? (float*)nullptr : (float*)backward_buffer, direct ? (half_t*)grad_weights : (half_t*)nullptr, in_planar,
-                               dx_planar, pf_depth, mid);
+                               dx_planar, pf_depth, mid, images);
             int rc = check_launch("ffmlp_backward");
             if (rc || direct || defer) return rc;
             hipLaunchKernelGGL(k_ffmlp_reduce_slabs, dim3(cdiv(n_params, RS_PARAMS)), dim3(RS_PARAMS * RS_GROUPS), 0, st,
@@ -1801,12 +1847,12 @@
     if (blocks <= 1) {
         hipLaunchKernelGGL(kern, dim3(1), dim3(FF_THREADS), lds, st, (const half_t*)grad, (const half_t*)inputs, (const half_t*)weights,
                            (const half_t*)fwd, n_tiles, in_dim, num_layers, act, with_dx, (half_t*)grad_inputs, (float*)nullptr,
-                           (half_t*)grad_weights, in_planar, dx_planar, pf_depth);
+                           (half_t*)grad_weights, in_planar, dx_planar, pf_depth, images);
         return check_launch("ffmlp_backward");
     }
     hipLaunchKernelGGL(kern, dim3(blocks), dim3(FF_THREADS), lds, st, (const half_t*)grad, (const half_t*)inputs, (const half_t*)weights,
                        (const half_t*)fwd, n_tiles, in_dim, num_layers, act, with_dx, (half_t*)grad_inputs, (float*)backward_buffer,
-                       (half_t*)nullptr, in_planar, dx_planar, pf_depth);
+                       (half_t*)nullptr, in_planar, dx_planar, pf_depth, images);
     int rc = check_launch("ffmlp_backward");
     if (rc) return rc;
     hipLaunchKernelGGL(k_ffmlp_reduce_slabs, dim3(cdiv(n_params, RS_PARAMS)), dim3(RS_PARAMS * RS_GROUPS), 0, st, (const float*)backward_buffer, blocks, n_params,
@@ -1825,9 +1871,59 @@
                                                        grad_inputs, grad_weights, flags, st, mid);
 }
 
+template <int WIDTH>
+__global__ __launch_bounds__(FF_THREADS) void k_ffmlp_build_weight_images(half_t* __restrict__ weights_and_images, uint32_t in_dim, uint32_t num_layers) {
+    const FFImageLayout lay = ff_image_layout(in_dim, WIDTH, num_layers);
+    unsigned char* base = reinterpret_cast<unsigned char*>(weights_and_images);
+    if (blockIdx.x == 0) build_forward_image<WIDTH>(reinterpret_cast<half8_t*>(base + lay.fwd_off), weights_and_images, in_dim, num_layers);
+    else build_backward_image<WIDTH>(reinterpret_cast<half8_t*>(base + lay.bwd_off), weights_and_images, in_dim, num_layers, true);
+}
+
+template <int WIDTH>
+static int launch_build_weight_images(void* weights_and_images, uint32_t in_dim, uint32_t num_layers, hipStream_t st) {
+    hipLaunchKernelGGL(k_ffmlp_build_weight_images<WIDTH>, dim3(2), dim3(FF_THREADS), 0, st, (half_t*)weights_and_images, in_dim, num_layers);
+    return check_launch("ffmlp_build_weight_images");
+}
+
+static bool weight_images_shape_ok(uint32_t in_dim, uint32_t hidden, uint32_t num_layers) {
+    return (hidden == 16 || hidden == 32 || hidden == 64 || hidden == 128) && in_dim > 0 && in_dim % 16 == 0 && num_layers >= 2;
+}
+
 }
 
 using namespace ngp;
+
+extern "C" size_t ngp_ffmlp_forward_image_offset(uint32_t input_dim, uint32_t hidden_dim, uint32_t num_layers) {
+    return weight_images_shape_ok(input_dim, hidden_dim, num_layers) ? ff_image_layout(input_dim, hidden_dim, num_layers).fwd_off : 0;
+}
+extern "C" size_t ngp_ffmlp_forward_image_bytes(uint32_t input_dim, uint32_t hidden_dim, uint32_t num_layers) {
+    return weight_images_shape_ok(input_dim, hidden_dim, num_layers) ? (size_t)ff_image_layout(input_dim, hidden_dim, num_layers).fwd_frags * 1024 : 0;
+}
+extern "C" size_t ngp_ffmlp_backward_image_offset(uint32_t input_dim, uint32_t hidden_dim, uint32_t num_layers) {
+    return weight_images_shape_ok(input_dim, hidden_dim, num_layers) ? ff_image_layout(input_dim, hidden_dim, num_layers).bwd_off : 0;
+}
+extern "C" size_t ngp_ffmlp_backward_image_bytes(uint32_t input_dim, uint32_t hidden_dim, uint32_t num_layers) {
+    return weight_images_shape_ok(input_dim, hidden_dim, num_layers) ? (size_t)ff_image_layout(input_dim, hidden_dim, num_layers).bwd_frags * 1024 : 0;
+}
+extern "C" size_t ngp_ffmlp_weights_with_images_bytes(uint32_t input_dim, uint32_t hidden_dim, uint32_t num_layers) {
+    return weight_images_shape_ok(input_dim, hidden_dim, num_layers) ? ff_image_layout(input_dim, hidden_dim, num_layers).total : 0;
+}
+
+extern "C" int ngp_ffmlp_build_weight_images(void* weights_and_images, uint32_t input_dim, uint32_t hidden_dim, uint32_t num_layers,
+                                             ngp_stream_t stream) {
+    NGP_REQUIRE(weight_images_shape_ok(input_dim, hidden_dim, num_layers), NGP_ERR_INVALID,
+                "ffmlp_build_weight_images: hidden_dim in [16, 32, 64, 128], input_dim 16 * m, num_layers >= 2 (got %u, %u, %u)", hidden_dim, input_dim,
+                num_layers);
+    NGP_REQUIRE(weights_and_images && (reinterpret_cast<uintptr_t>(weights_and_images) & 15u) == 0, NGP_ERR_INVALID,
+                "ffmlp_build_weight_images: NULL or not 16-byte aligned buffer");
+    hipStream_t st = as_stream(stream);
+    switch (hidden_dim) {
+        case 16: return launch_build_weight_images<16>(weights_and_images, input_dim, num_layers, st);
+        case 32: return launch_build_weight_images<32>(weights_and_images, input_dim, num_layers, st);
+        case 64: return launch_build_weight_images<64>(weights_and_images, input_dim, num_layers, st);
+        default: return launch_build_weight_images<128>(weights_and_images, input_dim, num_layers, st);
+    }
+}
 
 #define FF_WIDTHS(CALL)                  \
     switch (hidden_dim) {                \
@@ -1893,6 +1989,7 @@
     const bool fast = (hidden_dim == 32 || hidden_dim == 64) && num_layers <= 4 && input_dim <= 64 && !(flags & NGP_FF_LAYERED);
     NGP_REQUIRE(fast || !(flags & NGP_FF_RECOMPUTE), NGP_ERR_INVALID, "ffmlp_backward: NGP_FF_RECOMPUTE serves 64-wide ReLU networks with 32 inputs and 2 or 3 layers");
     NGP_REQUIRE(fast || !(flags & NGP_FF_DEFER_REDUCE), NGP_ERR_INVALID, "ffmlp_backward: NGP_FF_DEFER_REDUCE needs a 2- or 3-layer network of width 32 / 64");
+    NGP_REQUIRE(fast || !(flags & NGP_FF_WEIGHT_IMAGES), NGP_ERR_INVALID, "ffmlp_backward: NGP_FF_WEIGHT_IMAGES serves the register-resident kernels (width 32 / 64, <= 4 layers, <= 64 inputs)");
     if (!fast) {
 #define FF_LAY(W) launch_backward_layered<W>(grad, inputs, weights, forward_buffer, B, input_dim, num_layers, activation, dx, backward_buffer, grad_inputs, grad_weights, flags, workspace, workspace_bytes, st)
         FF_WIDTHS(FF_LAY)
@@ -1954,8 +2051,8 @@
                                           ngp_stream_t stream) {
     NGP_REQUIRE(num_layers_color == 2 || num_layers_color == 3, NGP_ERR_INVALID,
                 "network_backward_color: 2 or 3 layers (got %u); use ngp_ffmlp_backward_ex + ngp_pipeline_mid_backward", num_layers_color);
-    NGP_REQUIRE(!(flags & ~(NGP_FF_DEFER_REDUCE | NGP_FF_RECOMPUTE)), NGP_ERR_INVALID,
-                "network_backward_color: only NGP_FF_DEFER_REDUCE and NGP_FF_RECOMPUTE are accepted");
+    NGP_REQUIRE(!(flags & ~(NGP_FF_DEFER_REDUCE | NGP_FF_RECOMPUTE | NGP_FF_WEIGHT_IMAGES)), NGP_ERR_INVALID,
+                "network_backward_color: only NGP_FF_DEFER_REDUCE, NGP_FF_RECOMPUTE and NGP_FF_WEIGHT_IMAGES are accepted");
     int rc = check_ff_args("network_backward_color", M, 32, 16, 64, num_layers_color);
     if (rc) return rc;
     if (M == 0) return NGP_OK;
@@ -2018,15 +2115,17 @@
     const uint32_t need = cdiv(cdiv(n_tiles, nt), waves);
     if (blocks > need) blocks = need;
     hipStream_t st = as_stream(stream);
-    const bool planar = (flags & NGP_FF_INPUT_PLANAR) != 0;
+    const bool planar = (flags & NGP_FF_INPUT_PLANAR) != 0, images = (flags & NGP_FF_WEIGHT_IMAGES) != 0;
+    NGP_REQUIRE(!images || (weight_images_readable(w_sigma) && weight_images_readable(w_color)), NGP_ERR_INVALID,
+                "network_forward: NGP_FF_WEIGHT_IMAGES needs 16-byte aligned weights");
     if (training)
         hipLaunchKernelGGL((k_network_forward<true, TW, TT>), dim3(blocks), dim3(TW * 64), lds, st, (const half_t*)enc, planar, dirs, M_valid, (const half_t*)w_sigma,
                            (const half_t*)w_color, (half_t*)forward_buffer_sigma, (half_t*)h16, sigma, (half_t*)color_in, (half_t*)forward_buffer_color, rgb,
-                           n_tiles, num_layers_sigma, num_layers_color, density_scale, rows_dev);
+                           n_tiles, num_layers_sigma, num_layers_color, density_scale, rows_dev, images);
     else
         hipLaunchKernelGGL((k_network_forward<false, IW, IT>), dim3(blocks), dim3(IW * 64), lds, st, (const half_t*)enc, planar, dirs, M_valid, (const half_t*)w_sigma,
                            (const half_t*)w_color, (half_t*)nullptr, (half_t*)nullptr, sigma, (half_t*)nullptr, (half_t*)nullptr, rgb, n_tiles,
-                           num_layers_sigma, num_layers_color, density_scale, rows_dev);
+                           num_layers_sigma, num_layers_color, density_scale, rows_dev, images);
     return check_launch("network_forward");
 }
 
diff --git a/torch-ngp_amd/csrc/ffmlp_images.h b/torch-ngp_amd/csrc/ffmlp_images.h
--- /dev/null
+++ b/torch-ngp_amd/csrc/ffmlp_images.h
@@ -0,0 +1,67 @@
+#pragma once
+#include <stddef.h>
+#include <stdint.h>
+
+namespace ngp {
+
+struct FFImageLayout {
+    uint32_t in_dim, hidden, num_layers;
+    uint32_t nib, nkb, in_kb, in_jb;
+    uint32_t n_weights;
+    uint32_t fwd_frags, bwd_frags;
+    size_t fwd_off, bwd_off, total;
+};
+
+__host__ __device__ inline FFImageLayout ff_image_layout(uint32_t in_dim, uint32_t hidden, uint32_t num_layers) {
+    FFImageLayout L;
+    L.in_dim = in_dim; L.hidden = hidden; L.num_layers = num_layers;
+    L.nib = (hidden + 31u) / 32u;
+    L.nkb = (hidden + 15u) / 16u;
+    L.in_kb = in_dim / 16u;
+    L.in_jb = (in_dim + 31u) / 32u;
+    L.n_weights = hidden * (in_dim + hidden * (num_layers - 1u) + 16u);
+    L.fwd_frags = L.nib * L.in_kb + (num_layers - 1u) * L.nib * L.nkb + L.nkb;
+    L.bwd_frags = L.nib + (num_layers - 1u) * L.nib * L.nkb + L.in_jb * L.nkb;
+    L.fwd_off = ((size_t)L.n_weights * 2u + 1023u) / 1024u * 1024u;
+    L.bwd_off = L.fwd_off + (size_t)L.fwd_frags * 1024u;
+    L.total = L.bwd_off + (size_t)L.bwd_frags * 1024u;
+    return L;
+}
+
+__host__ __device__ inline uint32_t ff_image_half(uint32_t frag, uint32_t i, uint32_t h, uint32_t j) { return ((frag * 64u + h * 32u + i) * 8u) + j; }
+
+__host__ __device__ inline void ff_feature_slot(uint32_t f, uint32_t& kb, uint32_t& h, uint32_t& j) {
+    kb = f / 16u;
+    h = (f >> 2) & 1u;
+    j = ((f >> 3) & 1u) * 4u + (f & 3u);
+}
+
+__host__ __device__ inline void ff_weight_coords(const FFImageLayout& L, uint32_t idx, uint32_t& m, uint32_t& r, uint32_t& c) {
+    const uint32_t n_in = L.hidden * L.in_dim, n_hid = L.hidden * L.hidden;
+    if (idx < n_in) { m = 0u; r = idx / L.in_dim; c = idx % L.in_dim; return; }
+    idx -= n_in;
+    if (idx < (L.num_layers - 1u) * n_hid) { m = 1u + idx / n_hid; idx %= n_hid; }
+    else { m = L.num_layers; idx -= (L.num_layers - 1u) * n_hid; }
+    r = idx / L.hidden; c = idx % L.hidden;
+}
+
+__host__ __device__ inline uint32_t ff_forward_image_slot(const FFImageLayout& L, uint32_t idx) {
+    uint32_t m, r, c, kb, h, j;
+    ff_weight_coords(L, idx, m, r, c);
+    if (m == 0u) return ff_image_half((r / 32u) * L.in_kb + c / 16u, r % 32u, (c >> 3) & 1u, c & 7u);
+    ff_feature_slot(c, kb, h, j);
+    const uint32_t hid0 = L.nib * L.in_kb;
+    if (m < L.num_layers) return ff_image_half(hid0 + (m - 1u) * L.nib * L.nkb + (r / 32u) * L.nkb + kb, r % 32u, h, j);
+    return ff_image_half(hid0 + (L.num_layers - 1u) * L.nib * L.nkb + kb, r, h, j);
+}
+
+__host__ __device__ inline uint32_t ff_backward_image_slot(const FFImageLayout& L, uint32_t idx) {
+    uint32_t m, r, c, kb, h, j;
+    ff_weight_coords(L, idx, m, r, c);
+    if (m == L.num_layers) return ff_image_half(c / 32u, c % 32u, r / 8u, r & 7u);
+    ff_feature_slot(r, kb, h, j);
+    if (m >= 1u) return ff_image_half(L.nib + (L.num_layers - 1u - m) * L.nib * L.nkb + (c / 32u) * L.nkb + kb, c % 32u, h, j);
+    return ff_image_half(L.nib + (L.num_layers - 1u) * L.nib * L.nkb + (c / 32u) * L.nkb + kb, c % 32u, h, j);
+}
+
+}
diff --git a/torch-ngp_amd/csrc/optim.hip b/torch-ngp_amd/csrc/optim.hip
--- a/torch-ngp_amd/csrc/optim.hip
+++ b/torch-ngp_amd/csrc/optim.hip
@@ -1,4 +1,5 @@
 #include "common.h"
+#include "ffmlp_images.h"
 #include <math.h>
 #include <stdlib.h>
 
@@ -217,10 +218,14 @@
 }
 
 constexpr int OPT_SMALL_THREADS = 1024;
-__global__ __launch_bounds__(OPT_SMALL_THREADS) void k_adam_small_commit(OptTensors ts, float* __restrict__ state, float beta1, float beta2, float eps,
-                                                                        float grad_mult, float growth, float backoff, float growth_interval,
-                                                                        int flip_parity, TableAdam ta, const half_t* __restrict__ tgrad,
-                                                                        uint64_t tprefix, uint32_t prefix_blocks) {
+struct OptImageShapes {
+    uint32_t in_dim[OPT_MAX_TENSORS], hidden[OPT_MAX_TENSORS], num_layers[OPT_MAX_TENSORS];
+};
+template <bool IMAGES>
+__device__ __forceinline__ void adam_small_commit(const OptTensors& ts, float* __restrict__ state, float beta1, float beta2, float eps, float grad_mult,
+                                                  float growth, float backoff, float growth_interval, int flip_parity, const TableAdam& ta,
+                                                  const half_t* __restrict__ tgrad, uint64_t tprefix, uint32_t prefix_blocks,
+                                                  const OptImageShapes* shapes) {
     const AdamConsts ac = adam_consts(state, beta1, beta2, grad_mult);
     const float bc2_sqrt = ac.bc2_sqrt;
     const float beta1_s = beta1, beta2_s = beta2, eps_s = eps;
@@ -271,6 +276,12 @@
         const bool gh = (ts.g_is_half[k] & 1) != 0, keep = (ts.g_is_half[k] & 2) != 0;
         half_t* g16 = reinterpret_cast<half_t*>(ts.g[k]);
         float* g32 = reinterpret_cast<float*>(ts.g[k]);
+        bool with_images = false;
+        FFImageLayout lay = {};
+        if constexpr (IMAGES) {
+            with_images = p16 && shapes->hidden[k] != 0u;
+            if (with_images) lay = ff_image_layout(shapes->in_dim[k], shapes->hidden[k], shapes->num_layers[k]);
+        }
         for (uint64_t i = gtid; i < n; i += gstride) {
             float g = gh ? (float)g16[i] : g32[i];
             if (!keep) { if (gh) g16[i] = (half_t)0.0f; else g32[i] = 0.0f; }
@@ -280,6 +291,12 @@
             adam_element(g, nm, nv, np_, beta1_s, beta2_s, eps_s, step_size, bc2_sqrt);
             m[i] = nm; v[i] = nv; p[i] = np_;
             if (p16) p16[i] = (half_t)np_;
+            if constexpr (IMAGES) {
+                if (with_images) {
+                    p16[lay.fwd_off / 2 + ff_forward_image_slot(lay, (uint32_t)i)] = (half_t)np_;
+                    p16[lay.bwd_off / 2 + ff_backward_image_slot(lay, (uint32_t)i)] = (half_t)np_;
+                }
+            }
         }
     }
     __syncthreads();
@@ -290,6 +307,21 @@
             __hip_atomic_store(&state[6], 0.0f, __ATOMIC_RELAXED, __HIP_MEMORY_SCOPE_AGENT);
         }
     }
+}
+__global__ __launch_bounds__(OPT_SMALL_THREADS) void k_adam_small_commit(OptTensors ts, float* __restrict__ state, float beta1, float beta2, float eps,
+                                                                        float grad_mult, float growth, float backoff, float growth_interval,
+                                                                        int flip_parity, TableAdam ta, const half_t* __restrict__ tgrad,
+                                                                        uint64_t tprefix, uint32_t prefix_blocks) {
+    adam_small_commit<false>(ts, state, beta1, beta2, eps, grad_mult, growth, backoff, growth_interval, flip_parity, ta, tgrad, tprefix, prefix_blocks,
+                             nullptr);
+}
+__global__ __launch_bounds__(OPT_SMALL_THREADS) void k_adam_small_commit_images(OptTensors ts, float* __restrict__ state, float beta1, float beta2,
+                                                                               float eps, float grad_mult, float growth, float backoff,
+                                                                               float growth_interval, int flip_parity, TableAdam ta,
+                                                                               const half_t* __restrict__ tgrad, uint64_t tprefix,
+                                                                               uint32_t prefix_blocks, OptImageShapes shapes) {
+    adam_small_commit<true>(ts, state, beta1, beta2, eps, grad_mult, growth, backoff, growth_interval, flip_parity, ta, tgrad, tprefix, prefix_blocks,
+                            &shapes);
 }
 
 __global__ void k_poison_shards(half_t* __restrict__ grad, uint32_t shards, uint64_t payload, const float* __restrict__ state) {
@@ -394,6 +426,17 @@
                                            float beta2, float eps, float grad_mult, float growth_factor, float backoff_factor,
                                            float growth_interval, float* state, int flip_parity, const ngp_table_adam_t* table,
                                            const void* table_grad_fp16, uint64_t table_prefix_params, ngp_stream_t stream) {
+    return ngp_optim_adam_small_commit_images(count, n, params, exp_avg, exp_avg_sq, grads, params_fp16, grad_is_half, lr, beta1, beta2, eps, grad_mult,
+                                              growth_factor, backoff_factor, growth_interval, state, flip_parity, table, table_grad_fp16,
+                                              table_prefix_params, nullptr, stream);
+}
+
+extern "C" int ngp_optim_adam_small_commit_images(int count, const uint64_t* n, float* const* params, float* const* exp_avg, float* const* exp_avg_sq,
+                                                  void* const* grads, void* const* params_fp16, const int* grad_is_half, const float* lr,
+                                                  float beta1, float beta2, float eps, float grad_mult, float growth_factor, float backoff_factor,
+                                                  float growth_interval, float* state, int flip_parity, const ngp_table_adam_t* table,
+                                                  const void* table_grad_fp16, uint64_t table_prefix_params, const uint32_t* image_shapes,
+                                                  ngp_stream_t stream) {
     NGP_REQUIRE(state, NGP_ERR_INVALID, "optim_adam_small_commit: NULL state");
     NGP_REQUIRE((reinterpret_cast<uintptr_t>(state) & 15u) == 0, NGP_ERR_INVALID, "optim_adam_small_commit: state (8 floats) must be 16-byte aligned");
     NGP_REQUIRE(count >= 0 && count <= OPT_MAX_TENSORS, NGP_ERR_INVALID, "optim_adam_small_commit: at most %d tensors per call (got %d)", OPT_MAX_TENSORS,
@@ -415,6 +458,18 @@
         ts.lr[k] = lr[k];
         total += n[k];
     }
+    OptImageShapes shapes = {};
+    bool any_images = false;
+    for (int k = 0; image_shapes && k < count; k++) {
+        const uint32_t in_dim = image_shapes[3 * k], hidden = image_shapes[3 * k + 1], nl = image_shapes[3 * k + 2];
+        if (!hidden) continue;
+        NGP_REQUIRE((hidden == 16 || hidden == 32 || hidden == 64 || hidden == 128) && in_dim > 0 && in_dim % 16 == 0 && nl >= 2 &&
+                        ff_image_layout(in_dim, hidden, nl).n_weights == n[k] && ts.p16[k],
+                    NGP_ERR_INVALID, "optim_adam_small_commit_images: tensor %d is not an FFMLP weight tensor of shape (%u, %u, %u) with an fp16 copy", k,
+                    in_dim, hidden, nl);
+        shapes.in_dim[k] = in_dim; shapes.hidden[k] = hidden; shapes.num_layers[k] = nl;
+        any_images = true;
+    }
     TableAdam ta = {};
     if (table_prefix_params) {
         NGP_REQUIRE(table && table_grad_fp16 && table->state == state, NGP_ERR_INVALID,
@@ -436,9 +491,14 @@
     if (prefix_blocks > 192u) prefix_blocks = 192u;
     uint32_t small_blocks = (uint32_t)cdiv64(total - table_prefix_params, (uint64_t)OPT_SMALL_THREADS);
     small_blocks = small_blocks < 1u ? 1u : (small_blocks > 32u ? 32u : small_blocks);
-    hipLaunchKernelGGL(k_adam_small_commit, dim3(prefix_blocks + small_blocks), dim3(OPT_SMALL_THREADS), 0, as_stream(stream), ts, state, beta1, beta2, eps,
-                       grad_mult, growth_factor, backoff_factor, growth_interval, flip_parity, ta, reinterpret_cast<const half_t*>(table_grad_fp16),
-                       table_prefix_params, prefix_blocks);
+    if (any_images)
+        hipLaunchKernelGGL(k_adam_small_commit_images, dim3(prefix_blocks + small_blocks), dim3(OPT_SMALL_THREADS), 0, as_stream(stream), ts, state, beta1,
+                           beta2, eps, grad_mult, growth_factor, backoff_factor, growth_interval, flip_parity, ta,
+                           reinterpret_cast<const half_t*>(table_grad_fp16), table_prefix_params, prefix_blocks, shapes);
+    else
+        hipLaunchKernelGGL(k_adam_small_commit, dim3(prefix_blocks + small_blocks), dim3(OPT_SMALL_THREADS), 0, as_stream(stream), ts, state, beta1, beta2,
+                           eps, grad_mult, growth_factor, backoff_factor, growth_interval, flip_parity, ta,
+                           reinterpret_cast<const half_t*>(table_grad_fp16), table_prefix_params, prefix_blocks);
     return check_launch("optim_adam_small_commit");
 }
 
diff --git a/torch-ngp_amd/ffmlp/ffmlp.py b/torch-ngp_amd/ffmlp/ffmlp.py
--- a/torch-ngp_amd/ffmlp/ffmlp.py
+++ b/torch-ngp_amd/ffmlp/ffmlp.py
@@ -77,6 +77,7 @@
 
         self.num_parameters = hidden_dim * (input_dim + hidden_dim * (num_layers - 1) + self.padded_output_dim)
         self.weights = nn.Parameter(torch.zeros(self.num_parameters))
+        self.weights._ngp_ffmlp_shape = (self.input_dim, self.hidden_dim, self.num_layers)
         self.reset_parameters()
         _backend.allocate_splitk(self.num_layers + 1)
 
diff --git a/torch-ngp_amd/fused.py b/torch-ngp_amd/fused.py
--- a/torch-ngp_amd/fused.py
+++ b/torch-ngp_amd/fused.py
@@ -7,7 +7,7 @@
 from torch.autograd import Function
 
 import _ngp_capi as capi
-from optim import announce_overwrite, clean_deposits, resync_stale_shadows
+from optim import announce_overwrite, clean_deposits, image_shape, rebuild_weight_images, resync_stale_shadows
 
 _PLANAR_IN = capi.NGP_FF_INPUT_PLANAR
 _PLANAR_DX = capi.NGP_FF_DX_PLANAR
@@ -55,7 +55,7 @@
             fb_s = fb_c = None
         assert not cfg.training or density_scale == 1.0, 'the backward of _fused_ngp knows no density scale (the fused training render folds it itself)'
         _network_forward(enc, d, d_valid, bufs.ws16, bufs.wc16, cfg.nl_sigma, cfg.nl_color, float(density_scale), cfg.training, fb_s, h16, sigma,
-                         color_in, fb_c, out16, rgb, M, st)
+                         color_in, fb_c, out16, rgb, M, st, images=not cfg.training)
         if cfg.training:
             ctx.save_for_backward(x, offsets, enc, bufs.ws16, bufs.wc16, fb_s, fb_c, h16, color_in, rgb)
             ctx.cfg = cfg
@@ -97,11 +97,17 @@
 USE_FUSED_NETWORK = True
 
 
-def _network_forward(enc, dirs, d_valid, ws16, wc16, nl_sigma, nl_color, density_scale, training, fb_s, h16, sigma, color_in, fb_c, out16, rgb, M, st):
+def _images_flag(*weights16):
+    return capi.NGP_FF_WEIGHT_IMAGES if all(getattr(t, '_ngp_images', None) is not None for t in weights16) else 0
+
+
+def _network_forward(enc, dirs, d_valid, ws16, wc16, nl_sigma, nl_color, density_scale, training, fb_s, h16, sigma, color_in, fb_c, out16, rgb, M, st,
+                     images=False):
     if USE_FUSED_NETWORK:
         capi.check(capi.lib.ngp_network_forward(enc.data_ptr(), dirs.data_ptr(), M, d_valid, ws16.data_ptr(), wc16.data_ptr(), nl_sigma, nl_color,
                                                  float(density_scale), 1 if training else 0, capi.ptr(fb_s), capi.ptr(h16) if training else None,
-                                                 sigma.data_ptr(), capi.ptr(color_in) if training else None, capi.ptr(fb_c), rgb.data_ptr(), _PLANAR_IN, st))
+                                                 sigma.data_ptr(), capi.ptr(color_in) if training else None, capi.ptr(fb_c), rgb.data_ptr(),
+                                                 _PLANAR_IN | (_images_flag(ws16, wc16) if images else 0), st))
         return
     if training:
         capi.check(capi.lib.ngp_ffmlp_forward_ex(enc.data_ptr(), ws16.data_ptr(), M, 32, 16, 64, nl_sigma, 0, 6, fb_s.data_ptr(), h16.data_ptr(),
@@ -196,7 +202,7 @@
     return Marched(xyzs, dirs, deltas, rays, nears, fars, ws)
 
 
-def _render_train_network(marched, bufs, bg, offsets, cfg, rcfg, composite=True):
+def _render_train_network(marched, bufs, bg, offsets, cfg, rcfg, composite=True, images=False):
     xyzs, rays = marched.xyzs, marched.rays
     nl_sigma, nl_color = cfg.nl_sigma, cfg.nl_color
     N, M = rays.shape[0], rcfg.capacity
@@ -218,7 +224,7 @@
         fb_s = torch.empty(nl_sigma, M, 64, **half)
         fb_c = torch.empty(nl_color, M, 64, **half)
     _network_forward(enc, marched.dirs, M, bufs.ws16, bufs.wc16, nl_sigma, nl_color, float(rcfg.density_scale), True, fb_s, h16, sigma, color_in, fb_c,
-                     out16, rgb, M, st)
+                     out16, rgb, M, st, images)
     saved = Saved(xyzs, offsets, enc, bufs.ws16, bufs.wc16, fb_s, fb_c, h16, color_in, rgb, sigma, marched.deltas, rays, weights_sum=None,
                   image_raw=None, bg=bg, march_ws=marched.ws)
     if not composite:
@@ -236,7 +242,7 @@
     return image, depth, weights_sum, saved._replace(weights_sum=weights_sum, image_raw=image_raw)
 
 
-def _render_train_backward(saved, cfg, rcfg, grad_image, grad_ws, g_emb, g_ws, g_wc, found_inf=None, overwrite=False):
+def _render_train_backward(saved, cfg, rcfg, grad_image, grad_ws, g_emb, g_ws, g_wc, found_inf=None, overwrite=False, images=False):
     s = saved
     M, N = s.xyzs.shape[0], s.rays.shape[0]
     dev = s.xyzs.device
@@ -251,10 +257,11 @@
                                                               s.march_ws.data_ptr(), st))
     g_out16 = torch.empty(M, 16, device=dev, dtype=torch.half)
     capi.check(capi.lib.ngp_pipeline_rgb_backward(g_rgb.data_ptr(), s.rgb.data_ptr(), g_out16.data_ptr(), M, st))
-    _network_backward(saved, cfg, rcfg, g_sigma, g_out16, g_emb, g_ws, g_wc, found_inf, None, overwrite)
-
-
-def _network_backward(saved, cfg, rcfg, g_sigma, g_out16, g_emb, g_ws, g_wc, found_inf=None, loss_job=None, overwrite=False, table_adam=None):
+    _network_backward(saved, cfg, rcfg, g_sigma, g_out16, g_emb, g_ws, g_wc, found_inf, None, overwrite, images=images)
+
+
+def _network_backward(saved, cfg, rcfg, g_sigma, g_out16, g_emb, g_ws, g_wc, found_inf=None, loss_job=None, overwrite=False, table_adam=None,
+                      images=False):
     s = saved
     nl_sigma, nl_color, density_scale = cfg.nl_sigma, cfg.nl_color, rcfg.density_scale
     grid = (cfg.L, cfg.S, cfg.H, cfg.gridtype, cfg.align, cfg.interp, cfg.bound)
@@ -267,12 +274,13 @@
         scratch_s = torch.empty(nl_sigma, M, 64, **half)
         g_h16 = torch.empty(M, 16, **half)
         rc = capi.NGP_FF_RECOMPUTE if s.fb_c is None else 0
+        img_c, img_s = (_images_flag(s.wc16), _images_flag(s.ws16)) if images else (0, 0)
         capi.check(capi.lib.ngp_network_backward_color(g_out16.data_ptr(), s.color_in.data_ptr(), s.wc16.data_ptr(), capi.ptr(s.fb_c), M, nl_color,
                                                         scratch_c.data_ptr(), g_sigma.data_ptr(), s.h16.data_ptr(), float(density_scale),
-                                                        g_h16.data_ptr(), g_wc.data_ptr(), capi.NGP_FF_DEFER_REDUCE | rc, st))
+                                                        g_h16.data_ptr(), g_wc.data_ptr(), capi.NGP_FF_DEFER_REDUCE | rc | img_c, st))
         capi.check(capi.lib.ngp_ffmlp_backward_ex(g_h16.data_ptr(), s.enc.data_ptr(), s.ws16.data_ptr(), capi.ptr(s.fb_s), M, 32, 16, 64, nl_sigma,
                                                    0, 6, 1, scratch_s.data_ptr(), g_enc.data_ptr(), g_ws.data_ptr(),
-                                                   _PLANAR_IN | _PLANAR_DX | capi.NGP_FF_DEFER_REDUCE | rc, st))
+                                                   _PLANAR_IN | _PLANAR_DX | capi.NGP_FF_DEFER_REDUCE | rc | img_s, st))
         n_c, n_s = capi.lib.ngp_ffmlp_backward_slab_count(M, 32, 64, nl_color), capi.lib.ngp_ffmlp_backward_slab_count(M, 32, 64, nl_sigma)
         if USE_SLABS_IN_ACCUMULATE:
             err, loss = loss_job if loss_job is not None else (None, None)
@@ -291,14 +299,15 @@
             raise RuntimeError('fused: a deferred loss sum needs the carried reductions (_carries_reductions)')
         g_color_in = torch.empty(M, 32, **half)
         scratch = torch.empty(max(nl_color, nl_sigma), M, 64, **half)
+        img_c, img_s = (_images_flag(s.wc16), _images_flag(s.ws16)) if images else (0, 0)
         capi.check(capi.lib.ngp_ffmlp_backward_ex(g_out16.data_ptr(), s.color_in.data_ptr(), s.wc16.data_ptr(), s.fb_c.data_ptr(), M, 32, 16, 64,
-                                                   nl_color, 0, 6, 1, scratch.data_ptr(), g_color_in.data_ptr(), g_wc.data_ptr(), 0, st))
+                                                   nl_color, 0, 6, 1, scratch.data_ptr(), g_color_in.data_ptr(), g_wc.data_ptr(), img_c, st))
         g_h16 = g_out16
         capi.check(capi.lib.ngp_pipeline_mid_backward(g_sigma.data_ptr(), s.h16.data_ptr(), g_color_in.data_ptr(), g_h16.data_ptr(), M,
                                                        float(density_scale), st))
         capi.check(capi.lib.ngp_ffmlp_backward_ex(g_h16.data_ptr(), s.enc.data_ptr(), s.ws16.data_ptr(), s.fb_s.data_ptr(), M, 32, 16, 64, nl_sigma,
                                                    0, 6, 1, scratch[:nl_sigma].data_ptr(), g_enc.data_ptr(), g_ws.data_ptr(),
-                                                   _PLANAR_IN | _PLANAR_DX, st))
+                                                   _PLANAR_IN | _PLANAR_DX | img_s, st))
     _grid_backward(g_enc, s.xyzs, s.offsets, g_emb, M, *grid, st, found_inf, None, overwrite, table_adam)
 
 
@@ -381,6 +390,7 @@
 USE_OVERWRITE_TABLE = os.environ.get('NGP_FUSED_OVERWRITE_TABLE', '1') != '0'
 USE_SLABS_IN_ACCUMULATE = os.environ.get('NGP_FUSED_SLABS_IN_ACCUMULATE', '1') != '0'
 USE_RECOMPUTE = os.environ.get('NGP_FUSED_RECOMPUTE', '0') == '1'
+USE_WEIGHT_IMAGES = os.environ.get('NGP_FUSED_WEIGHT_IMAGES', '1') != '0'
 
 
 def _carries_reductions(nl_sigma, nl_color):
@@ -401,14 +411,14 @@
         raise RuntimeError('fused: table_adam needs the fused compositor, the in-kernel non-finite sweep (found_inf) and overwrite_table')
     g_emb, g_ws, g_wc = bufs.g_emb, bufs.g_ws.view(-1), bufs.g_wc.view(-1)
     if not USE_FUSED_COMPOSITE:
-        image, depth, weights_sum, saved = _render_train_network(marched, bufs, bg_t, offsets, cfg, rcfg)
+        image, depth, weights_sum, saved = _render_train_network(marched, bufs, bg_t, offsets, cfg, rcfg, images=USE_WEIGHT_IMAGES)
         loss = torch.empty(1, device=image.device, dtype=torch.float32)
         grad_image = torch.empty_like(image)
         capi.check(capi.lib.ngp_pipeline_mse_loss(image.data_ptr(), target.data_ptr(), image.numel(), capi.ptr(loss_scale), loss.data_ptr(),
                                                    grad_image.data_ptr(), capi.stream()))
-        _render_train_backward(saved, cfg, rcfg, grad_image, None, g_emb, g_ws, g_wc, found_inf, overwrite)
+        _render_train_backward(saved, cfg, rcfg, grad_image, None, g_emb, g_ws, g_wc, found_inf, overwrite, images=USE_WEIGHT_IMAGES)
         return loss, image, depth, weights_sum
-    s = _render_train_network(marched, bufs, bg_t, offsets, cfg, rcfg, composite=False)
+    s = _render_train_network(marched, bufs, bg_t, offsets, cfg, rcfg, composite=False, images=USE_WEIGHT_IMAGES)
     N, M, dev = s.rays.shape[0], s.xyzs.shape[0], s.xyzs.device
     f32 = dict(device=dev, dtype=torch.float32)
     weights_sum, image, depth = torch.empty(N, **f32), torch.empty(N, 3, **f32), torch.empty(N, **f32)
@@ -424,7 +434,7 @@
                                                            g_out16.data_ptr(), s.march_ws.data_ptr(),
                                                            s.march_ws.numel() * s.march_ws.element_size(), capi.stream()))
     _network_backward(s, cfg, rcfg, g_sigma, g_out16, g_emb, g_ws, g_wc, found_inf, loss_job=(ray_err, loss) if defer else None,
-                      overwrite=overwrite, table_adam=table_adam)
+                      overwrite=overwrite, table_adam=table_adam, images=USE_WEIGHT_IMAGES)
     return loss, image, depth, weights_sum
 
 
@@ -472,7 +482,7 @@
                   int(encoder.interp_id), bound, costs, st)
     h16 = torch.empty(M, 16, device=dev, dtype=torch.half)
     capi.check(capi.lib.ngp_ffmlp_inference_ex(enc.data_ptr(), w16.data_ptr(), M, 32, 16, 64, int(sigma_net.num_layers), 0, 6, None, h16.data_ptr(),
-                                                _PLANAR_IN, st))
+                                                _PLANAR_IN | _images_flag(w16), st))
     return torch.exp(h16[:, 0].float()), h16[:, 1:]
 
 
@@ -503,9 +513,15 @@
                     fn()
                 buf = getattr(p, '_ngp_fp16_pinbuf', None)
                 if buf is None or buf.shape != p.shape or buf.device != p.device:
-                    buf = torch.empty_like(p, dtype=torch.half)
+                    shape = image_shape(p)
+                    if shape is None:
+                        buf = torch.empty_like(p, dtype=torch.half)
+                    else:
+                        buf = torch.empty(capi.weight_image_halves(shape), device=p.device, dtype=torch.half)[:p.numel()].view_as(p)
+                        buf._ngp_images = shape
                     p._ngp_fp16_pinbuf = buf
                 buf.copy_(p.detach())
+                rebuild_weight_images(buf)
                 p._ngp_fp16_pin = buf
         return self
 
diff --git a/torch-ngp_amd/optim.py b/torch-ngp_amd/optim.py
--- a/torch-ngp_amd/optim.py
+++ b/torch-ngp_amd/optim.py
@@ -45,8 +45,23 @@
             p._ngp_grad16_stale = False
 
 
+def image_shape(p):
+    shape = getattr(p, '_ngp_ffmlp_shape', None)
+    if shape is None or not p.is_cuda:
+        return None
+    shape = tuple(int(v) for v in shape)
+    return shape if capi.weight_image_halves(shape) > 0 and shape[1] * (shape[0] + shape[1] * (shape[2] - 1) + 16) == p.numel() else None
+
+
+def rebuild_weight_images(t16):
+    shape = getattr(t16, '_ngp_images', None)
+    if shape is not None:
+        capi.build_weight_images(t16, shape)
+
+
 def refresh_shadow(p):
     p._ngp_fp16.copy_(p.detach())
+    rebuild_weight_images(p._ngp_fp16)
     p._ngp_version = p._version
 
 
@@ -89,10 +104,11 @@
                 raise RuntimeError('NGPAdam: parameters must be contiguous float32 CUDA tensors')
             dev = p.device
         self.flat_params = flat_params
+        images = {p: image_shape(p) for p in flat_params} if deposit and not self.shard else {}
         self.offsets, total = [], 0
         for p in flat_params:
             self.offsets.append(total)
-            total += (p.numel() + 7) // 8 * 8
+            total += ((capi.weight_image_halves(images[p]) if images.get(p) else p.numel()) + 7) // 8 * 8
         self.payload = total
         if self.shard:
             self.payload = ((total + self.world_size - 1) // self.world_size + 7) // 8 * 8
@@ -119,6 +135,9 @@
             if deposit:
                 st['fp16'] = self.flat_p16[off:off + n].view_as(p)
                 st['fp16'].copy_(p.detach())
+                if images.get(p):
+                    st['fp16']._ngp_images = images[p]
+                    rebuild_weight_images(st['fp16'])
                 st['grad16'] = self.flat_grad16[off:off + n].view_as(p)
                 p._ngp_fp16, p._ngp_grad16, p._ngp_version = st['fp16'], st['grad16'], p._version
             self.state[p] = st
@@ -408,12 +427,16 @@
     def _launch_small_commit(self, entries, flip, table_prefix=0):
         k, cast = len(entries), self._entry_arrays(entries, ema=False)
         ta = self._table_adam_struct() if table_prefix else None
-        capi.check(capi.lib.ngp_optim_adam_small_commit(k, cast[0], cast[1], cast[2], cast[3], cast[4], cast[5], cast[6], cast[7], self.betas[0],
-                                                        self.betas[1], self.eps, 1.0, self.growth_factor, self.backoff_factor, self.growth_interval,
-                                                        self.scalars.data_ptr(), 1 if flip else 0,
-                                                        None if ta is None else ctypes.cast(ctypes.pointer(ta), ctypes.c_void_p),
-                                                        self.state[self.fused_table]['grad16'].data_ptr() if table_prefix else None,
-                                                        int(table_prefix), capi.stream()))
+        shapes = [getattr(e[5], '_ngp_images', None) or (0, 0, 0) for e in entries]
+        shape_arr = (ctypes.c_uint32 * (3 * k))(*[int(v) for sh in shapes for v in sh]) if any(sh[1] for sh in shapes) else None
+        capi.check(capi.lib.ngp_optim_adam_small_commit_images(k, cast[0], cast[1], cast[2], cast[3], cast[4], cast[5], cast[6], cast[7],
+                                                               self.betas[0], self.betas[1], self.eps, 1.0, self.growth_factor,
+                                                               self.backoff_factor, self.growth_interval, self.scalars.data_ptr(),
+                                                               1 if flip else 0,
+                                                               None if ta is None else ctypes.cast(ctypes.pointer(ta), ctypes.c_void_p),
+                                                               self.state[self.fused_table]['grad16'].data_ptr() if table_prefix else None,
+                                                               int(table_prefix),
+                                                               None if shape_arr is None else ctypes.cast(shape_arr, ctypes.c_void_p), capi.stream()))
 
     @torch.no_grad()
     def step(self, update_ema=None, gradients_checked=False):
@@ -461,6 +484,8 @@
             for c in chunks:
                 self._launch(c, UPDATE, omd)
             self._launch([], COMMIT, 0.0)
+        for e in entries:
+            rebuild_weight_images(e[5])
 
     def load_torch_adam_state(self, adam_sd, scaler_sd=None):
         flat = [p for g in self.param_groups for p in g['params']]
```

Result: no change. 630.7 million, median of 6 (+0.9%).
